# scychon/openmm_drudeNose

Hardware: AMD Instinct MI355X
Metric: integrator steps/sec at 1M Drude pairs (higher is better)
Workload: dtype f64; 1 GPU; SWM4-NDP water box, 1000000 molecules = 5000000 particle slots, 1000000 Drude pairs, 1 temperature group (+ molecular-COM and Drude thermostats), TGNH mode, mixed precision, numNHChains=1, hard wall 0.02 nm, harness force call-out inside the timed region (harness_force: lattice); harness_force=lattice, precision=mixed, variant=resident, hipgraph=False, parallelism=particle-sharded x1 (whole molecules), one KE all-reduce per step, slots_per_gpu=5000000

## Files before the change

### include/drude_tgnh.h

```cpp
#ifndef DRUDE_TGNH_H_
#define DRUDE_TGNH_H_

#include <stdint.h>

#ifdef __cplusplus
extern "C" {
#endif

#define TGNH_ABI_VERSION 1

typedef int tgnh_status;
enum {
    TGNH_OK = 0,
    TGNH_ERR_ARG = -1,
    TGNH_ERR_GROUP_MISMATCH = -2,
    TGNH_ERR_HARDWALL = -3,
    TGNH_ERR_UNSUPPORTED = -4,
    TGNH_ERR_HIP = -5,
    TGNH_ERR_STATE = -6
};

enum { TGNH_MODE_DUALNH = 0,
       TGNH_MODE_TGNH = 1 };

// ... 8 lines not shown
enum { TGNH_FLAG_TRUST_STATE_CHANGED = 16 };

enum { TGNH_FLAG_GATHER = 32 };

typedef struct tgnh_desc {
    uint32_t struct_size;
    int32_t mode;
    int32_t precision;
    int32_t flags;
    int32_t device;
    int32_t num_particles;
    int32_t padded_num_particles;
    int32_t num_pairs;
    int32_t num_groups;
    int32_t num_residues;
    int32_t num_constraints;
    int32_t has_cm_motion_remover;
    const double* mass;
    const int32_t* pair_drude;
    const int32_t* pair_parent;
    const int32_t* group;
    const int32_t* resid;
    const int32_t* constraint_i;
    const int32_t* constraint_j;
    double kB;
    double temperature, coupling_time;
    double drude_temperature, drude_coupling_time;
    double step_size;
    int32_t drude_steps_per_real_step;
    int32_t num_nh_chains;
    int32_t use_drude_nh_chains;
    int32_t use_com_temp_group;
    double max_drude_distance;
} tgnh_desc;

typedef struct tgnh_context* tgnh_handle;


typedef int (*tgnh_allreduce_fn)(void* buf, int count, void* stream, void* user);

const char* tgnh_last_error(void);
int tgnh_abi_version(void);

tgnh_status tgnh_create(const tgnh_desc* desc, tgnh_handle* out);
tgnh_status tgnh_destroy(tgnh_handle h);

tgnh_status tgnh_bind_buffers(tgnh_handle h, void* posq, void* posq_correction, void* velm,
                              const void* force, void* pos_delta);

tgnh_status tgnh_set_step_size(tgnh_handle h, double dt);
tgnh_status tgnh_set_drude_steps_per_real_step(tgnh_handle h, int n);
tgnh_status tgnh_set_max_drude_distance(tgnh_handle h, double d);

tgnh_status tgnh_get_local_dof_terms(tgnh_handle h, double* terms, int* count);
tgnh_status tgnh_set_global_dof_terms(tgnh_handle h, const double* terms, int count);
tgnh_status tgnh_set_allreduce(tgnh_handle h, tgnh_allreduce_fn fn, void* user);

#define TGNH_RCCL_ID_BYTES 128
tgnh_status tgnh_rccl_unique_id(void* id_out);
tgnh_status tgnh_rccl_init(tgnh_handle h, int world, int rank, const void* id);
tgnh_status tgnh_set_rccl_comm(tgnh_handle h, void* nccl_comm);
tgnh_status tgnh_rccl_shutdown(tgnh_handle h);
tgnh_status tgnh_set_resident_share(tgnh_handle h, int share);
tgnh_status tgnh_get_resident_work_groups(tgnh_handle h, int* per_compute_unit);
tgnh_status tgnh_get_step_path(tgnh_handle h, int* gather, const char** reason);
tgnh_status tgnh_get_resident_kernel(tgnh_handle h, int* which);

#define TGNH_XCHG_HANDLE_BYTES 64
tgnh_status tgnh_exchange_create(tgnh_handle h, int world, int rank, void* ipc_handle_out, void** mailbox_out);
tgnh_status tgnh_exchange_attach(tgnh_handle h, const void* ipc_handles);
tgnh_status tgnh_exchange_attach_pointers(tgnh_handle h, void* const* mailboxes);
tgnh_status tgnh_exchange_detach(tgnh_handle h);
tgnh_status tgnh_exchange_wait_stats(tgnh_handle h, void* stream, double* mean_us, double* max_us, int64_t* exchanges);

tgnh_status tgnh_step_begin(tgnh_handle h, void* stream);
tgnh_status tgnh_step_end(tgnh_handle h, void* stream);
tgnh_status tgnh_step_begin_kick(tgnh_handle h, void* stream);
tgnh_status tgnh_step_begin_move(tgnh_handle h, void* stream);
tgnh_status tgnh_step_end_kick(tgnh_handle h, void* stream);
tgnh_status tgnh_step_end_thermo(tgnh_handle h, void* stream);
tgnh_status tgnh_flush(tgnh_handle h, void* stream);
tgnh_status tgnh_note_replayed_steps(tgnh_handle h, int nsteps);
tgnh_status tgnh_get_pending_state(tgnh_handle h, uint32_t* bits);
tgnh_status tgnh_set_time(tgnh_handle h, double time, int64_t step_count);
tgnh_status tgnh_state_changed(tgnh_handle h);

tgnh_status tgnh_set_velocities_to_temperature(tgnh_handle h, double temperature, double drude_temperature,
                                               uint64_t seed, int64_t first_particle, void* stream);

typedef struct tgnh_momentum {
    uint32_t struct_size;
    int32_t  reserved;
    int64_t  massive;
    double   mass;
    double   momentum[3];
} tgnh_momentum;
tgnh_status tgnh_get_momentum(tgnh_handle h, void* stream, tgnh_momentum* out);
tgnh_status tgnh_shift_velocities(tgnh_handle h, const double dv[3], void* stream);
tgnh_status tgnh_remove_cm_motion(tgnh_handle h, void* stream);
tgnh_status tgnh_set_cm_motion_removal(tgnh_handle h, int every);

tgnh_status tgnh_set_molecules(tgnh_handle h, const int32_t* molecule );
tgnh_status tgnh_get_num_molecules(tgnh_handle h, int* count);
tgnh_status tgnh_get_molecules(tgnh_handle h, int32_t* molecule_out );
tgnh_status tgnh_scale_positions(tgnh_handle h, const double scale[3], int save, void* stream);
tgnh_status tgnh_restore_positions(tgnh_handle h, void* stream);

enum { TGNH_MIN_DRUDE_ONLY = 1 };
typedef struct tgnh_minimize_desc {
    double tolerance;
    double dt_start, dt_max;
    double max_step;
    double f_inc, f_dec, alpha_start, f_alpha;
    int32_t n_min;
    int32_t flags;
    const uint8_t* moving;
} tgnh_minimize_desc;
typedef struct tgnh_minimize_state {
    int64_t iterations, uphill, since_uphill, moving;
    int32_t converged;
    int32_t reserved;
    double dt, alpha, power, ff, vv, rms_force;
} tgnh_minimize_state;
tgnh_status tgnh_minimize_begin(tgnh_handle h, const tgnh_minimize_desc* desc, double* work , void* stream);
tgnh_status tgnh_minimize_iterate(tgnh_handle h, void* stream);
tgnh_status tgnh_get_minimize_state(tgnh_handle h, void* stream, tgnh_minimize_state* out);
tgnh_status tgnh_minimize_end(tgnh_handle h);
tgnh_status tgnh_run_harness_minimize(tgnh_handle h, const void* x0, double k_drude, double k_tether, int iterations, void* stream);

tgnh_status tgnh_set_periodic_box(tgnh_handle h, const double a[3], const double b[3], const double c[3]);
tgnh_status tgnh_get_periodic_box(tgnh_handle h, double a[3], double b[3], double c[3]);
tgnh_status tgnh_wrap_molecules(tgnh_handle h, void* stream);
enum { TGNH_FRAME_WRAP = 1, TGNH_FRAME_SKIP_DRUDE = 2, TGNH_FRAME_INTERLEAVED = 4 };
typedef struct tgnh_frame_desc {
    uint32_t struct_size;
    int32_t  flags;
    double   unit;
    int64_t  stride;
    int64_t  capacity;
} tgnh_frame_desc;
tgnh_status tgnh_get_frame_count(tgnh_handle h, int32_t flags, int64_t* count);
tgnh_status tgnh_write_frame(tgnh_handle h, const tgnh_frame_desc* desc, float* out , void* stream);

tgnh_status tgnh_scale_velocities(tgnh_handle h, const double* factors, int count, void* stream);
tgnh_status tgnh_rescale_to_temperature(tgnh_handle h, double temperature, double drude_temperature, void* stream);
tgnh_status tgnh_get_rescale_factors(tgnh_handle h, void* stream, double* factors);
tgnh_status tgnh_set_velocity_rescaling(tgnh_handle h, int every, double temperature, double drude_temperature);

tgnh_status tgnh_set_temperatures(tgnh_handle h, double temperature, double drude_temperature, void* stream);

tgnh_status tgnh_get_kinetic_energy(tgnh_handle h, int ke_sum_valid, void* stream, double* out);
tgnh_status tgnh_get_num_thermostats(tgnh_handle h, int* count);
tgnh_status tgnh_get_last_kinetic_energies(tgnh_handle h, void* stream, double* ke);
tgnh_status tgnh_get_last_scale_factors(tgnh_handle h, void* stream, double* scale);
tgnh_status tgnh_get_status_flags(tgnh_handle h, void* stream, uint32_t* flags);
tgnh_status tgnh_get_time(tgnh_handle h, double* time, int64_t* step_count);
tgnh_status tgnh_get_dof(tgnh_handle h, double* dof, double* nkt);

#define TGNH_DRUDE_HIST_BINS 32
typedef struct tgnh_drude_stats {
    uint32_t struct_size;
    int32_t  worst_particle;
    int64_t  pairs;
    int64_t  over;
    double   max_distance;
    double   sum_d2;
// ... 58 lines not shown
```

### openmm_drudenose_amd/_lib.py

```python
import ctypes as C
import os

HERE = os.path.dirname(os.path.abspath(__file__))
LIB_PATH = os.environ.get("TGNH_LIB") or os.path.join(HERE, "libdrudetgnh_hip.so")

TGNH_OK = 0
ERR_ARG, ERR_GROUP_MISMATCH, ERR_HARDWALL, ERR_UNSUPPORTED, ERR_HIP, ERR_STATE = -1, -2, -3, -4, -5, -6
MODE_DUALNH, MODE_TGNH = 0, 1
PREC_SINGLE, PREC_MIXED, PREC_DOUBLE = 0, 1, 2
FLAG_DEFER_SCALE, FLAG_RESIDENT_STEP, FLAG_WAVE_TILES, FLAG_TRUST_STATE_CHANGED, FLAG_GATHER = 2, 4, 8, 16, 32
KID_SKD, KID_KICK_KE, KID_SCALE, KID_KE, KID_CHAIN, KID_FORCE, KID_OTHER, KID_STEP = range(8)
KERNEL_NAMES = {KID_SKD: "scale+kick+drift", KID_KICK_KE: "kick+KE", KID_SCALE: "rescale", KID_KE: "KE",
                KID_CHAIN: "chain", KID_FORCE: "harness force", KID_OTHER: "other", KID_STEP: "resident step"}

c_i32p = C.POINTER(C.c_int32)
c_f64p = C.POINTER(C.c_double)


class TgnhDesc(C.Structure):
    _fields_ = [
        ("struct_size", C.c_uint32), ("mode", C.c_int32), ("precision", C.c_int32), ("flags", C.c_int32),
        ("device", C.c_int32), ("num_particles", C.c_int32), ("padded_num_particles", C.c_int32),
        ("num_pairs", C.c_int32), ("num_groups", C.c_int32), ("num_residues", C.c_int32),
        ("num_constraints", C.c_int32), ("has_cm_motion_remover", C.c_int32),
        ("mass", c_f64p), ("pair_drude", c_i32p), ("pair_parent", c_i32p), ("group", c_i32p), ("resid", c_i32p),
        ("constraint_i", c_i32p), ("constraint_j", c_i32p),
        ("kB", C.c_double), ("temperature", C.c_double), ("coupling_time", C.c_double),
        ("drude_temperature", C.c_double), ("drude_coupling_time", C.c_double), ("step_size", C.c_double),
        ("drude_steps_per_real_step", C.c_int32), ("num_nh_chains", C.c_int32),
        ("use_drude_nh_chains", C.c_int32), ("use_com_temp_group", C.c_int32),
        ("max_drude_distance", C.c_double),
    ]


DRUDE_HIST_BINS = 32


class TgnhDrudeStats(C.Structure):
    _fields_ = [
        ("struct_size", C.c_uint32), ("worst_particle", C.c_int32), ("pairs", C.c_int64), ("over", C.c_int64),
        ("max_distance", C.c_double), ("sum_d2", C.c_double), ("dipole", C.c_double * 3),
        ("hist", C.c_int64 * (DRUDE_HIST_BINS + 1)),
    ]


class TgnhMomentum(C.Structure):
    _fields_ = [
        ("struct_size", C.c_uint32), ("reserved", C.c_int32), ("massive", C.c_int64), ("mass", C.c_double),
        ("momentum", C.c_double * 3),
    ]


FRAME_WRAP, FRAME_SKIP_DRUDE, FRAME_INTERLEAVED = 1, 2, 4


class TgnhFrameDesc(C.Structure):
    _fields_ = [
        ("struct_size", C.c_uint32), ("flags", C.c_int32), ("unit", C.c_double), ("stride", C.c_int64), ("capacity", C.c_int64),
    ]


MIN_DRUDE_ONLY = 1
SITE_TWO_AVERAGE, SITE_THREE_AVERAGE, SITE_OUT_OF_PLANE, SITE_LOCAL_COORDINATES = range(4)
SITE_PARAMS = 12


class TgnhMinimizeDesc(C.Structure):
    _fields_ = [
        ("tolerance", C.c_double), ("dt_start", C.c_double), ("dt_max", C.c_double), ("max_step", C.c_double),
        ("f_inc", C.c_double), ("f_dec", C.c_double), ("alpha_start", C.c_double), ("f_alpha", C.c_double),
        ("n_min", C.c_int32), ("flags", C.c_int32), ("moving", C.c_void_p),
    ]


class TgnhMinimizeState(C.Structure):
    _fields_ = [
        ("iterations", C.c_int64), ("uphill", C.c_int64), ("since_uphill", C.c_int64), ("moving", C.c_int64),
        ("converged", C.c_int32), ("reserved", C.c_int32),
        ("dt", C.c_double), ("alpha", C.c_double), ("power", C.c_double), ("ff", C.c_double), ("vv", C.c_double),
        ("rms_force", C.c_double),
    ]


ALLREDUCE_FN = C.CFUNCTYPE(C.c_int, C.c_void_p, C.c_int, C.c_void_p, C.c_void_p)

SIGNATURES = {
    "tgnh_last_error": (C.c_char_p, []),
    "tgnh_abi_version": (C.c_int, []),
    "tgnh_create": (C.c_int, [C.POINTER(TgnhDesc), C.POINTER(C.c_void_p)]),
    "tgnh_destroy": (C.c_int, [C.c_void_p]),
    "tgnh_bind_buffers": (C.c_int, [C.c_void_p] * 6),
    "tgnh_set_step_size": (C.c_int, [C.c_void_p, C.c_double]),
    "tgnh_set_drude_steps_per_real_step": (C.c_int, [C.c_void_p, C.c_int]),
    "tgnh_set_max_drude_distance": (C.c_int, [C.c_void_p, C.c_double]),
    "tgnh_get_local_dof_terms": (C.c_int, [C.c_void_p, c_f64p, C.POINTER(C.c_int)]),
    "tgnh_set_global_dof_terms": (C.c_int, [C.c_void_p, c_f64p, C.c_int]),
    "tgnh_set_allreduce": (C.c_int, [C.c_void_p, ALLREDUCE_FN, C.c_void_p]),
    "tgnh_rccl_unique_id": (C.c_int, [C.c_void_p]),
    "tgnh_rccl_init": (C.c_int, [C.c_void_p, C.c_int, C.c_int, C.c_void_p]),
    "tgnh_set_rccl_comm": (C.c_int, [C.c_void_p, C.c_void_p]),
    "tgnh_rccl_shutdown": (C.c_int, [C.c_void_p]),
    "tgnh_exchange_wait_stats": (C.c_int, [C.c_void_p, C.c_void_p, c_f64p, c_f64p, C.POINTER(C.c_int64)]),
    "tgnh_get_pending_state": (C.c_int, [C.c_void_p, C.POINTER(C.c_uint32)]),
    "tgnh_set_resident_share": (C.c_int, [C.c_void_p, C.c_int]),
    "tgnh_get_resident_work_groups": (C.c_int, [C.c_void_p, C.POINTER(C.c_int)]),
    "tgnh_get_resident_kernel": (C.c_int, [C.c_void_p, C.POINTER(C.c_int)]),
    "tgnh_get_step_path": (C.c_int, [C.c_void_p, C.POINTER(C.c_int), C.POINTER(C.c_char_p)]),
    "tgnh_exchange_create": (C.c_int, [C.c_void_p, C.c_int, C.c_int, C.c_void_p, C.POINTER(C.c_void_p)]),
    "tgnh_exchange_attach": (C.c_int, [C.c_void_p, C.c_char_p]),
    "tgnh_exchange_attach_pointers": (C.c_int, [C.c_void_p, C.POINTER(C.c_void_p)]),
    "tgnh_exchange_detach": (C.c_int, [C.c_void_p]),
    "tgnh_step_begin": (C.c_int, [C.c_void_p, C.c_void_p]),
    "tgnh_step_end": (C.c_int, [C.c_void_p, C.c_void_p]),
    "tgnh_step_begin_kick": (C.c_int, [C.c_void_p, C.c_void_p]),
    "tgnh_step_begin_move": (C.c_int, [C.c_void_p, C.c_void_p]),
    "tgnh_step_end_kick": (C.c_int, [C.c_void_p, C.c_void_p]),
    "tgnh_step_end_thermo": (C.c_int, [C.c_void_p, C.c_void_p]),
    "tgnh_flush": (C.c_int, [C.c_void_p, C.c_void_p]),
    "tgnh_state_changed": (C.c_int, [C.c_void_p]),
    "tgnh_set_velocities_to_temperature": (C.c_int, [C.c_void_p, C.c_double, C.c_double, C.c_int64, C.c_int64, C.c_void_p]),
    "tgnh_get_momentum": (C.c_int, [C.c_void_p, C.c_void_p, C.c_void_p]),
    "tgnh_shift_velocities": (C.c_int, [C.c_void_p, c_f64p, C.c_void_p]),
    "tgnh_remove_cm_motion": (C.c_int, [C.c_void_p, C.c_void_p]),
    "tgnh_set_cm_motion_removal": (C.c_int, [C.c_void_p, C.c_int]),
    "tgnh_scale_velocities": (C.c_int, [C.c_void_p, c_f64p, C.c_int, C.c_void_p]),
    "tgnh_rescale_to_temperature": (C.c_int, [C.c_void_p, C.c_double, C.c_double, C.c_void_p]),
    "tgnh_get_rescale_factors": (C.c_int, [C.c_void_p, C.c_void_p, c_f64p]),
    "tgnh_set_velocity_rescaling": (C.c_int, [C.c_void_p, C.c_int, C.c_double, C.c_double]),
    "tgnh_set_molecules": (C.c_int, [C.c_void_p, c_i32p]),
    "tgnh_get_num_molecules": (C.c_int, [C.c_void_p, C.POINTER(C.c_int)]),
    "tgnh_get_molecules": (C.c_int, [C.c_void_p, c_i32p]),
    "tgnh_scale_positions": (C.c_int, [C.c_void_p, c_f64p, C.c_int, C.c_void_p]),
    "tgnh_restore_positions": (C.c_int, [C.c_void_p, C.c_void_p]),
    "tgnh_minimize_begin": (C.c_int, [C.c_void_p, C.c_void_p, C.c_void_p, C.c_void_p]),
    "tgnh_minimize_iterate": (C.c_int, [C.c_void_p, C.c_void_p]),
    "tgnh_get_minimize_state": (C.c_int, [C.c_void_p, C.c_void_p, C.c_void_p]),
    "tgnh_minimize_end": (C.c_int, [C.c_void_p]),
    "tgnh_run_harness_minimize": (C.c_int, [C.c_void_p, C.c_void_p, C.c_double, C.c_double, C.c_int, C.c_void_p]),
    "tgnh_set_periodic_box": (C.c_int, [C.c_void_p, c_f64p, c_f64p, c_f64p]),
    "tgnh_get_periodic_box": (C.c_int, [C.c_void_p, c_f64p, c_f64p, c_f64p]),
    "tgnh_wrap_molecules": (C.c_int, [C.c_void_p, C.c_void_p]),
    "tgnh_get_frame_count": (C.c_int, [C.c_void_p, C.c_int32, C.POINTER(C.c_int64)]),
    "tgnh_write_frame": (C.c_int, [C.c_void_p, C.c_void_p, C.c_void_p, C.c_void_p]),
    "tgnh_set_temperatures": (C.c_int, [C.c_void_p, C.c_double, C.c_double, C.c_void_p]),
    "tgnh_note_replayed_steps": (C.c_int, [C.c_void_p, C.c_int]),
    "tgnh_set_time": (C.c_int, [C.c_void_p, C.c_double, C.c_int64]),
    "tgnh_get_kinetic_energy": (C.c_int, [C.c_void_p, C.c_int, C.c_void_p, c_f64p]),
    "tgnh_get_num_thermostats": (C.c_int, [C.c_void_p, C.POINTER(C.c_int)]),
    "tgnh_get_last_kinetic_energies": (C.c_int, [C.c_void_p, C.c_void_p, c_f64p]),
    "tgnh_get_last_scale_factors": (C.c_int, [C.c_void_p, C.c_void_p, c_f64p]),
    "tgnh_get_status_flags": (C.c_int, [C.c_void_p, C.c_void_p, C.POINTER(C.c_uint32)]),
    "tgnh_get_time": (C.c_int, [C.c_void_p, c_f64p, C.POINTER(C.c_int64)]),
    "tgnh_get_dof": (C.c_int, [C.c_void_p, c_f64p, c_f64p]),
    "tgnh_get_drude_statistics": (C.c_int, [C.c_void_p, C.c_double, C.c_double, C.c_void_p, C.c_void_p]),
    "tgnh_get_thermostat_len": (C.c_int, [C.c_void_p, C.c_int, C.POINTER(C.c_int)]),
    "tgnh_get_thermostat_state": (C.c_int, [C.c_void_p, C.c_int, C.c_void_p, c_f64p]),
    "tgnh_set_thermostat_state": (C.c_int, [C.c_void_p, C.c_int, C.c_void_p, c_f64p]),
    "tgnh_get_topology_len": (C.c_int, [C.c_void_p, C.c_int, C.POINTER(C.c_int)]),
    "tgnh_get_topology": (C.c_int, [C.c_void_p, C.c_int, c_i32p]),
    "tgnh_get_launch_bounds": (C.c_int, [C.c_void_p, c_i32p]),
    "tgnh_compute_kinetic_energies": (C.c_int, [C.c_void_p, C.c_void_p]),
    "tgnh_half_kick": (C.c_int, [C.c_void_p, C.c_void_p]),
    "tgnh_harness_force": (C.c_int, [C.c_void_p, C.c_void_p, C.c_double, C.c_double, C.c_void_p, C.c_void_p]),
    "tgnh_harness_pack_sites": (C.c_int, [C.c_void_p, C.c_void_p]),
    "tgnh_harness_lattice_hint": (C.c_int, [C.c_void_p, C.c_int, C.c_int, C.c_double, c_f64p, C.c_int]),
    "tgnh_harness_sites_kind": (C.c_int, [C.c_void_p, C.POINTER(C.c_int)]),
    "tgnh_run_harness": (C.c_int, [C.c_void_p, C.c_void_p, C.c_double, C.c_double, C.c_int, C.c_void_p]),
    "tgnh_run_steps": (C.c_int, [C.c_void_p, C.c_int, C.c_void_p]),
    "tgnh_harness_set_clusters": (C.c_int, [C.c_void_p, C.c_int, c_i32p, c_f64p]),
    "tgnh_harness_shake_positions": (C.c_int, [C.c_void_p, C.c_double, C.c_void_p]),
    "tgnh_harness_shake_velocities": (C.c_int, [C.c_void_p, C.c_double, C.c_void_p]),
    "tgnh_harness_set_virtual_sites": (C.c_int, [C.c_void_p, C.c_int, c_i32p, c_f64p]),
    "tgnh_harness_virtual_sites": (C.c_int, [C.c_void_p, C.c_void_p]),
    "tgnh_run_harness_constrained": (C.c_int, [C.c_void_p, C.c_void_p, C.c_double, C.c_double, C.c_double, C.c_int, C.c_void_p]),
    "tgnh_set_constraint_clusters": (C.c_int, [C.c_void_p, C.c_int, c_i32p, c_f64p]),
    "tgnh_get_num_constraint_clusters": (C.c_int, [C.c_void_p, C.POINTER(C.c_int)]),
    "tgnh_apply_constraints": (C.c_int, [C.c_void_p, C.c_double, C.c_void_p]),
    "tgnh_apply_velocity_constraints": (C.c_int, [C.c_void_p, C.c_double, C.c_void_p]),
    "tgnh_set_virtual_sites": (C.c_int, [C.c_void_p, C.c_int, c_i32p, c_i32p, c_f64p]),
    "tgnh_get_num_virtual_sites": (C.c_int, [C.c_void_p, C.POINTER(C.c_int)]),
    "tgnh_compute_virtual_sites": (C.c_int, [C.c_void_p, C.c_void_p]),
    "tgnh_distribute_virtual_site_forces": (C.c_int, [C.c_void_p, C.c_void_p, C.c_void_p]),
    "tgnh_harness_water_force": (C.c_int, [C.c_void_p, C.c_double, C.c_double, C.c_void_p, C.c_void_p]),
    "tgnh_harness_remove_cm_motion": (C.c_int, [C.c_void_p, C.c_void_p]),
    "tgnh_timing_enable": (C.c_int, [C.c_void_p, C.c_int]),
    "tgnh_timing_read": (C.c_int, [C.c_void_p, C.c_int, c_f64p, C.POINTER(C.c_int64)]),
# ... 28 lines not shown
```

### openmm_drudenose_amd/build.py

```python
import os
import subprocess
import sys

HERE = os.path.dirname(os.path.abspath(__file__))
CSRC = os.path.join(HERE, "csrc")
LIB = os.path.join(HERE, "libdrudetgnh_hip.so")
SOURCES = ["tgnh_topology.cpp", "tgnh_lifecycle.cpp", "tgnh_exchange.cpp", "tgnh_step.cpp", "tgnh_velocities.cpp", "tgnh_queries.cpp", "tgnh_harness_host.cpp", "tgnh_positions.cpp",
           "tgnh_frames.cpp", "tgnh_minimize.cpp", "tgnh_constraints.cpp", "tgnh_virtual_sites.cpp",
           "tgnh_kernels.hip", "tgnh_gather.hip", "tgnh_harness.hip", "tgnh_velinit.hip", "tgnh_drude_stats.hip", "tgnh_cm_motion.hip",
           "tgnh_rescale.hip", "tgnh_scale_positions.hip", "tgnh_wrap.hip", "tgnh_minimize.hip", "tgnh_constraints.hip",
           "tgnh_virtual_sites.hip"]
HEADERS = sorted(n for n in os.listdir(CSRC) if n.endswith(".h")) + [os.path.join("..", "..", "include", "drude_tgnh.h")]
ARCH = "gfx950"


def source_sha():
    import hashlib
    h = hashlib.sha1()
    for name in sorted(os.listdir(CSRC)):
        path = os.path.join(CSRC, name)
        if os.path.isfile(path) and name.endswith((".cpp", ".hip", ".h")):
            h.update(name.encode())
            h.update(open(path, "rb").read())
    h.update(open(os.path.join(HERE, "..", "include", "drude_tgnh.h"), "rb").read())
    return h.hexdigest()[:16]


def _stale():
    if not os.path.exists(LIB):
        return True
    t = os.path.getmtime(LIB)
    deps = [os.path.join(CSRC, s) for s in SOURCES + HEADERS] + [os.path.abspath(__file__)]
    return any(os.path.getmtime(d) > t for d in deps)


def _object_key(src, flags):
    import hashlib
    h = hashlib.sha1(" ".join(flags).encode())
    for path in [os.path.join(CSRC, src)] + [os.path.join(CSRC, x) for x in HEADERS]:
        h.update(open(path, "rb").read())
    return h.hexdigest()[:16]


def build(force=False, verbose=False):
    if not force and not _stale():
        return LIB
    from concurrent.futures import ThreadPoolExecutor
    hipcc = os.environ.get("HIPCC", "/opt/rocm/bin/hipcc")
    flags = [hipcc, "--offload-arch=" + ARCH, "-O3", "-std=c++17", "-fPIC", "-Wall", "-Wno-unused-function", "-x", "hip"]
    objdir = os.path.join(HERE, "build")
    os.makedirs(objdir, exist_ok=True)

    def compile_one(src):
        obj = os.path.join(objdir, f"{os.path.splitext(src)[0]}.{_object_key(src, flags)}.o")
        if force or not os.path.exists(obj):
            cmd = flags + ["-c", os.path.join(CSRC, src), "-o", obj + ".tmp"]
            if verbose:
                print(" ".join(cmd), file=sys.stderr)
            subprocess.run(cmd, check=True)
            os.replace(obj + ".tmp", obj)
        return obj

    with ThreadPoolExecutor(len(SOURCES)) as pool:
        objs = list(pool.map(compile_one, SOURCES))
    for name in os.listdir(objdir):
        if name.endswith(".o") and os.path.join(objdir, name) not in objs:
            os.remove(os.path.join(objdir, name))
    cmd = [hipcc, "--offload-arch=" + ARCH, "-shared", "-fPIC"] + objs + ["-ldl", "-o", LIB]
    if verbose:
        print(" ".join(cmd), file=sys.stderr)
    subprocess.run(cmd, check=True)
    return LIB


if __name__ == "__main__":
    print(build(force="--force" in sys.argv, verbose=True))
```

### openmm_drudenose_amd/csrc/tgnh_constraints.cpp

```cpp
#include <numeric>

#include "tgnh_host.h"
#include "tgnh_constraints.h"

static const int CN_PA[6] = {0, 0, 0, 1, 1, 2}, CN_PB[6] = {1, 2, 3, 2, 3, 3};

static tgnh_status clusters_check(const tgnh_context* c, int n, const int32_t* atoms, const double* dist) {
    const int N = c->d.num_particles;
    std::vector<int> owner((size_t)N, -1);
    for (int k = 0; k < n; k++) {
        const int32_t* at = atoms + 4 * (size_t)k;
        const double* d = dist + 6 * (size_t)k;
        const std::string who = "tgnh_set_constraint_clusters: cluster " + std::to_string(k);
        for (int m = 0; m < 4; m++) {
            if (at[m] < -1 || at[m] >= N) return fail(TGNH_ERR_ARG, who + ": atom index " + std::to_string(at[m]) + " out of range");
            if (at[m] < 0) continue;
            if (owner[at[m]] == k) return fail(TGNH_ERR_ARG, who + " lists atom " + std::to_string(at[m]) + " twice");
            if (owner[at[m]] >= 0)
                return fail(TGNH_ERR_ARG, who + " and cluster " + std::to_string(owner[at[m]]) + " share atom " + std::to_string(at[m]) + ": two lanes would write one slot");
            owner[at[m]] = k;
        }
        int K = 0;
        for (int p = 0; p < 6; p++) {
            if (!std::isfinite(d[p]) || d[p] < 0.0) return fail(TGNH_ERR_ARG, who + ": a distance is negative or not finite");
// ... 21 lines not shown
    return TGNH_OK;
}

extern "C" tgnh_status tgnh_set_constraint_clusters(tgnh_handle h, int n, const int32_t* atoms, const double* dist) {
    CHECK_H(h);
    if (n < 0 || (n > 0 && (!atoms || !dist))) return fail(TGNH_ERR_ARG, "tgnh_set_constraint_clusters: bad cluster arrays");
    tgnh_status rc = clusters_check(h, n, atoms, dist); if (rc) return rc;
    if (h->host_only) { h->cons.count = n; return TGNH_OK; }
    HIP_OK(hipSetDevice(h->device));
    h->cons.drop();
    if (n == 0) return TGNH_OK;
    std::vector<int> order((size_t)n), first((size_t)n);
    for (int k = 0; k < n; k++) {
        int lo = h->d.num_particles;
        for (int m = 0; m < 4; m++) if (atoms[4 * (size_t)k + m] >= 0) lo = std::min(lo, (int)atoms[4 * (size_t)k + m]);
        first[k] = lo;
    }
    std::iota(order.begin(), order.end(), 0);
    std::stable_sort(order.begin(), order.end(), [&](int x, int y) { return first[x] < first[y]; });
    std::vector<int4> r_atoms((size_t)n);
    std::vector<double4> r_w((size_t)n);
    std::vector<double> r_d2(3 * (size_t)n, 0.0);
    std::vector<uint32_t> r_pairs((size_t)n);
    for (int row = 0; row < n; row++) {
        const int32_t* at = atoms + 4 * (size_t)order[row];
        const double* d = dist + 6 * (size_t)order[row];
        r_atoms[row] = make_int4(at[0], at[1], at[2], at[3]);
        double w[4];
        for (int m = 0; m < 4; m++) w[m] = at[m] >= 0 && h->topo.mass[at[m]] != 0.0 ? 1.0 / h->topo.mass[at[m]] : 0.0;
        r_w[row] = make_double4(w[0], w[1], w[2], w[3]);
        uint32_t pairs = 0, K = 0;
        for (int p = 0; p < 6; p++) {
            if (d[p] == 0.0) continue;
            r_d2[K * (size_t)n + row] = d[p] * d[p];
            pairs |= ((uint32_t)CN_PA[p] | (uint32_t)CN_PB[p] << 2) << (4 * K);
            K++;
        }
        r_pairs[row] = pairs | K << 12;
    }
    HIP_OK(h->cons.d_atoms.upload(r_atoms));
    HIP_OK(h->cons.d_invmass.upload(r_w));
    HIP_OK(h->cons.d_d2.upload(r_d2));
    HIP_OK(h->cons.d_pairs.upload(r_pairs));
    h->cons.count = n;
    return TGNH_OK;
}

extern "C" tgnh_status tgnh_get_num_constraint_clusters(tgnh_handle h, int* count) {
    CHECK_H(h);
    if (!count) return fail(TGNH_ERR_ARG, "null count");
    *count = h->cons.count;
    return TGNH_OK;
}

static tgnh_status constraints_ready(tgnh_handle h, const char* what) {
    CHECK_H(h);
    if (h->host_only) return fail(TGNH_ERR_STATE, std::string(what) + ": host-only handle (device -1): no GPU work can be launched on it");
    if (!h->bound.velm) return fail(TGNH_ERR_STATE, std::string(what) + ": tgnh_bind_buffers has not been called");
    return TGNH_OK;
}

static ConstraintArgs constraint_args(tgnh_handle h, double tol) {
    ConstraintArgs a{};
    a.atoms = h->cons.d_atoms; a.invmass = h->cons.d_invmass; a.d2 = h->cons.d_d2; a.pairs = h->cons.d_pairs; a.n = h->cons.count;
    a.posq = h->bound.posq; a.posq_corr = h->bound.posq_corr; a.velm = h->bound.velm; a.pos_delta = h->bound.pos_delta;
    a.tol = tol; a.status = h->status.d_word;
    return a;
}

extern "C" tgnh_status tgnh_apply_constraints(tgnh_handle h, double tol, void* stream) {
    tgnh_status rc = constraints_ready(h, "tgnh_apply_constraints"); if (rc) return rc;
    if (!h->bound.pos_delta) return fail(TGNH_ERR_STATE, "tgnh_apply_constraints: posDelta buffer not bound");
    if (h->cons.count == 0) return TGNH_OK;
    HIP_OK(hipSetDevice(h->device));
    HIP_OK(launch_constrain_positions(h->d.precision, constraint_args(h, tol), (hipStream_t)stream));
    return TGNH_OK;
}

extern "C" tgnh_status tgnh_apply_velocity_constraints(tgnh_handle h, double tol, void* stream) {
    tgnh_status rc = constraints_ready(h, "tgnh_apply_velocity_constraints"); if (rc) return rc;
    h->owed.ke_carry = false;
    if (h->cons.count == 0) return TGNH_OK;
    HIP_OK(hipSetDevice(h->device));
    HIP_OK(launch_constrain_velocities(h->d.precision, constraint_args(h, tol), (hipStream_t)stream));
    return TGNH_OK;
}
```

### openmm_drudenose_amd/csrc/tgnh_context.h

```cpp
#ifndef TGNH_CONTEXT_H_
#define TGNH_CONTEXT_H_

#include <map>
#include <string>
#include <vector>

#include "tgnh_internal.h"
#include "tgnh_by_index.h"
#include "tgnh_minimize.h"

void tgnh_set_error(const std::string& msg);

namespace tgnh {
template <typename T> class DeviceBuf {
    T* p_ = nullptr;
    bool pinned_ = false;
public:
    DeviceBuf() = default;
    DeviceBuf(DeviceBuf&& o) noexcept : p_(o.p_), pinned_(o.pinned_) { o.p_ = nullptr; }
    ~DeviceBuf() { reset(); }
    void reset() { if (p_) (void)(pinned_ ? hipHostFree(p_) : hipFree(p_)); p_ = nullptr; }
    hipError_t alloc(size_t n, bool zero = false, unsigned ext_flags = 0) {
        reset(); pinned_ = false;
        void* p = nullptr;
        hipError_t e = ext_flags ? hipExtMallocWithFlags(&p, sizeof(T) * n, ext_flags) : hipMalloc(&p, sizeof(T) * n);
        if (e != hipSuccess) return e;
        p_ = static_cast<T*>(p);
        return zero ? hipMemset(p_, 0, sizeof(T) * n) : hipSuccess;
    }
    hipError_t alloc_pinned(size_t n) { reset(); pinned_ = true; return hipHostMalloc(reinterpret_cast<void**>(&p_), sizeof(T) * n, hipHostMallocDefault); }
    hipError_t upload(const T* src, size_t n) {
        hipError_t e = alloc(n ? n : 1);
        return e != hipSuccess || !n ? e : hipMemcpy(p_, src, sizeof(T) * n, hipMemcpyHostToDevice);
    }
    hipError_t upload(const std::vector<T>& v) { return upload(v.data(), v.size()); }
    T* get() const { return p_; }
    operator T*() const { return p_; }
};
typedef DeviceBuf<unsigned char> DeviceBytes;

template <typename Row> struct __attribute__((visibility("hidden"))) RowScratch {
    DeviceBuf<Row> d_rows;
    int rows_allocated = 0;
    Row h_row{};
    tgnh_status ensure(int grid, bool zero, const char* too_small);
};
}

struct tgnh_context {
    tgnh_desc d;
    int device = 0;
    bool host_only = false;
    struct Topology {
        std::vector<double> mass;
        std::vector<int> pair_drude, pair_parent, group, resid, normal;
        std::vector<int> res_count, res_first;
        std::vector<int> tile_start, tile_res;
        std::vector<int2> res_entries;
        std::vector<int> big_first, big_count;
        int num_big = 0, num_tiles = 0;
        std::vector<uint32_t> meta;
        std::vector<int2> wave_tile;
        std::vector<uint32_t> wmeta;
        std::vector<uint32_t> tile_pat, wtile_pat;
        std::vector<uint32_t> pattern, wpattern;
        int num_wtiles = 0;
        tgnh::DeviceBuf<uint32_t> d_meta, d_wmeta, d_tile_pat, d_pattern, d_wpattern;
        tgnh::DeviceBuf<int> d_tile_start, d_tile_res;
        tgnh::DeviceBuf<int2> d_res_table, d_wave_tile, d_big_table;
        tgnh::DeviceBytes d_big_com;
    } topo;
    struct Gather {
        bool generic = false;
        bool chain = false;
        std::string reason;
        std::vector<int2> res_table;
        std::vector<int> resid, partner;
        int com_lanes = 64;
        tgnh::DeviceBuf<int> d_group, d_resid, d_partner;
        tgnh::DeviceBuf<int2> d_res_table;
        tgnh::DeviceBytes d_com;
        tgnh::DeviceBuf<double> d_scratch;
    } gather;
    struct ByIndex {
        tgnh::DeviceBuf<int> d_partner;
    } by_index;
    tgnh::RowScratch<tgnh::DrudeStatsRow> dstats;
    struct CmMotion : tgnh::RowScratch<tgnh::CmRow> {
        int every = 0;
    } cmm;
    struct Rescale {
        tgnh::DeviceBuf<double> d_buf;
        bool applied = false;
        int every = 0;
        double temperature = 0, drude_temperature = 0;
    } resc;
    struct Molecules {
        struct Table {
            std::vector<int> mol_of;
            int count = 0;
            std::vector<int> mem_start, members;
            bool spans = false;
            std::vector<int> span_first;
            std::vector<unsigned long long> span_heads;
            std::vector<int> span_out;
            std::vector<unsigned long long> span_drude;
        } t;
        bool set = false;
        bool on_device = false;
        tgnh::DeviceBuf<int> d_span_first, d_mol_of, d_mem_start, d_members;
        tgnh::DeviceBuf<unsigned long long> d_span_heads;
        tgnh::DeviceBuf<int> d_span_out;
        tgnh::DeviceBuf<unsigned long long> d_span_drude;
        tgnh::DeviceBuf<double> d_shift;
        void drop_device() { on_device = false; d_span_first.reset(); d_mol_of.reset(); d_mem_start.reset(); d_members.reset(); d_span_heads.reset(); d_shift.reset(); d_span_out.reset(); d_span_drude.reset(); }
    } mol;
    struct PeriodicBox {
        bool set = false;
        double a[3] = {0, 0, 0}, b[3] = {0, 0, 0}, c[3] = {0, 0, 0};
    } box;
    struct Frames {
        std::vector<int> out_index;
        int kept = -1;
        tgnh::DeviceBuf<int> d_out_index;
    } frames;
    struct PositionSnapshot {
        tgnh::DeviceBytes d_posq, d_corr;
        bool taken = false;
        bool valid = false;
        const void *of_posq = nullptr, *of_corr = nullptr;
    } snap;
    struct Minimize {
        bool active = false;
        double* work = nullptr;
        int64_t moving = 0;
        tgnh::DeviceBuf<unsigned char> d_mask;
        tgnh::DeviceBuf<double> d_rows;
        tgnh::DeviceBuf<tgnh::MinState> d_state;
        tgnh::MinState h_state{};
        void drop() { active = false; work = nullptr; moving = 0; d_mask.reset(); d_rows.reset(); d_state.reset(); }
    } minim;
    struct Constraints {
        int count = 0;
        tgnh::DeviceBuf<int4> d_atoms;
        tgnh::DeviceBuf<double4> d_invmass;
        tgnh::DeviceBuf<double> d_d2;
        tgnh::DeviceBuf<uint32_t> d_pairs;
        void drop() { count = 0; d_atoms.reset(); d_invmass.reset(); d_d2.reset(); d_pairs.reset(); }
    } cons;
    struct VirtualSites {
        int count = 0;
        int receivers = 0;
        tgnh::DeviceBuf<int4> d_atoms;
        tgnh::DeviceBuf<int> d_kind;
        tgnh::DeviceBuf<double> d_params;
        tgnh::DeviceBuf<int> d_recv_slot, d_recv_start, d_recv_row;
        tgnh::DeviceBuf<unsigned char> d_recv_role;
        void drop() { count = receivers = 0; d_atoms.reset(); d_kind.reset(); d_params.reset(); d_recv_slot.reset(); d_recv_start.reset(); d_recv_row.reset(); d_recv_role.reset(); }
    } vsites;
    struct Thermostat {
        std::vector<double> h_state;
        std::vector<double> local_terms, global_terms;
        std::vector<double> dof, nkbt;
        double realkbT = 0, drudekbT = 0;
        tgnh::ChainLayout L{};
        tgnh::DeviceBuf<double> d_partials;
        tgnh::DeviceBuf<double> d_state;
        tgnh::DeviceBuf<double> d_stage;
        tgnh::DeviceBuf<double> d_scalar;
    } thermo;
    struct LaunchConfig {
        int grid = 0, gb = 1;
        int num_cus = 256, grid_override = 0;
        std::map<int, int> grid_cache;
        bool alternate_sweeps = true;
        int inline_sum_rows = tgnh::CHAIN_INLINE_SUM_ROWS;
        bool inline_sum_all = false;
        bool carry_ok = false;
        bool inline_chain = false;
        bool wave_ke = false;
        int resident_grid[5][2] = {{0, 0}, {0, 0}, {0, 0}, {0, 0}, {0, 0}};
        int resident_share = 1;
        int wresident_per_cu = 0, wresident_grid = 0;
        int resident_per_cu = 0;
    } cfg;
    struct Owed {
        bool end_pending = false;
        bool scale_pending = false;
        bool kick_pending = false;
        bool first_half_done = false;
        bool chain_pending = false;
        bool sum_pending = false;
        bool xwait_pending = false;
        bool stage_pending = false;
        bool ke_carry = false;
        bool chain_pending_twice = false;
        bool carry_pending = false;
        bool tail_summed = false;
        bool end_folded = false;
        bool g_com_fresh = false;
        enum : uint32_t { BIT_SWEEP_REVERSE = 1u << 8 };
        uint32_t bits() const {
            return end_pending | scale_pending << 1 | kick_pending << 2 | first_half_done << 3 | chain_pending << 4 | sum_pending << 5 |
                   xwait_pending << 6 | stage_pending << 7 | ke_carry << 9;
        }
        void chain_owed(bool twice) { chain_pending = true; chain_pending_twice = twice; }
        void chain_ran() { chain_pending = sum_pending = xwait_pending = carry_pending = false; }
        void velocities_current() { scale_pending = kick_pending = false; }
        void end_half_deferred(bool kick) { scale_pending = first_half_done = true; kick_pending = kick; }
        void resident_settled() { end_pending = first_half_done = false; velocities_current(); chain_pending = sum_pending = xwait_pending = false; }
        void thermostat_reset() { end_pending = first_half_done = false; velocities_current(); chain_pending = stage_pending = carry_pending = ke_carry = false; }
    } owed;
    struct Run {
        double time = 0;
        int64_t step_count = 0;
        int sweep_reverse = 0;
        int ke_parts = 0;
    } run;
    struct Bound {
        void *posq = nullptr, *posq_corr = nullptr, *velm = nullptr, *pos_delta = nullptr;
        const void* force = nullptr;
    } bound;
    struct Status {
        tgnh::DeviceBuf<uint32_t> d_word;
        tgnh::DeviceBuf<uint32_t> h_seen;
        int failed_code = 0;
        std::string failed;
    } status;
    struct Meeting {
        tgnh::DeviceBuf<unsigned int> d_sync;
        tgnh::DeviceBuf<unsigned long long> d_rows;
        tgnh::DeviceBuf<unsigned long long> self_box;
        tgnh::DeviceBuf<unsigned long long> d_self_misc;
        tgnh::XchgArgs self_x{};
    } meet;
    struct Exchange {
        tgnh_allreduce_fn allreduce = nullptr;
        void* allreduce_user = nullptr;
        void* rccl_comm = nullptr;
        bool rccl_owned = false;
        tgnh::XchgArgs args{};
        bool on = false;
        int world = 0, rank = 0;
        tgnh::DeviceBuf<unsigned long long> mailbox;
        tgnh::DeviceBuf<unsigned long long*> d_peers;
        std::vector<void*> opened;
        tgnh::DeviceBuf<unsigned long long> d_seq;
        tgnh::DeviceBuf<unsigned int> d_dead;
        tgnh::DeviceBuf<unsigned long long> d_stat;
        void close_peers() { for (void* p : opened) (void)hipIpcCloseMemHandle(p); opened.clear(); }
        ~Exchange() { close_peers(); }
    } xchg;
    struct Harness {
        tgnh::DeviceBuf<int4> d_cl_atoms, d_vs_atoms;
        tgnh::DeviceBuf<double> d_cl_dist, d_vs_w;
        int num_clusters = 0, num_sites = 0;
        tgnh::DeviceBuf<uint8_t> d_sflag;
        tgnh::DeviceBuf<uint32_t> d_sbase;
        tgnh::DeviceBytes d_sites;
        int lat_k = 0, lat_side = 0, lat_mol0 = 0;
        double lat_spacing = 0;
        std::vector<double> lat_geom;
        bool lat_on = false;
        tgnh::DeviceBuf<unsigned char> d_lat_tab;
        tgnh::DeviceBytes d_g_x0;
    } harness;
    struct Timing {
        bool on = false;
        int only = -1;
        struct Ev { hipEvent_t a, b; int kid; };
        std::vector<Ev> ev_pool;
        size_t ev_used = 0;
        double t_total[tgnh::KID_COUNT] = {0};
        int64_t t_count[tgnh::KID_COUNT] = {0};
        ~Timing() { for (auto& e : ev_pool) { (void)hipEventDestroy(e.a); (void)hipEventDestroy(e.b); } }
    } timing;
};

#endif
```

### openmm_drudenose_amd/csrc/tgnh_harness.hip

```cpp
#include "tgnh_context.h"
#include "tgnh_device_math.h"

namespace tgnh {

template <int PREC>
__global__ __launch_bounds__(BLOCK) void force_kernel(const ForceArgs a) {
    typedef typename Prec<PREC>::real4 real4;
    typedef typename Prec<PREC>::mixed mixed;
    const real4* __restrict__ posq = reinterpret_cast<const real4*>(a.posq);
    const float4* __restrict__ pcorr = reinterpret_cast<const float4*>(a.posq_corr);
    const real4* __restrict__ x0 = reinterpret_cast<const real4*>(a.x0);
    const mixed kd = (mixed)a.k_drude, kt = (mixed)a.k_tether;
    const int lane = threadIdx.x & 63;
    const int nround = (a.n + gridDim.x * BLOCK - 1) / (gridDim.x * BLOCK);
    for (int rr = 0; rr < nround; rr++) {
        const int r = a.reverse ? nround - 1 - rr : rr;
        const int blk = a.reverse ? (int)gridDim.x - 1 - (int)blockIdx.x : (int)blockIdx.x;
        const int i = (r * gridDim.x + blk) * BLOCK + threadIdx.x;
        const bool in = i < a.n;
        uint32_t m = 0;
        mixed x = 0, y = 0, z = 0;
        if (in) {
            m = a.meta[i];
            const real4 p = posq[i];
// ... 347 lines not shown
    const int ma = blockIdx.x;
    double xa[5][3], f[5][3];
#pragma unroll
    for (int i = 0; i < 5; i++) { site(5 * ma + i, xa[i]); f[i][0] = f[i][1] = f[i][2] = 0.0; }
    for (int mb = threadIdx.x; mb < a.n_mol; mb += BLOCK) {
        if (mb == ma) continue;
#pragma unroll
        for (int j = 0; j < 5; j++) {
            double xb[3];
            site(5 * mb + j, xb);
#pragma unroll
            for (int i = 0; i < 5; i++) {
                double d[3];
#pragma unroll
                for (int k = 0; k < 3; k++) { d[k] = xa[i][k] - xb[k]; d[k] -= a.box * floor(d[k] * inv_box + 0.5); }
                const double r2 = d[0] * d[0] + d[1] * d[1] + d[2] * d[2];
                if (r2 >= c2) continue;
                const double r = sqrt(r2), inv_r = 1.0 / r;
                double dEdr = ONE_4PI_EPS0 * Q[i] * Q[j] * (-inv_r * inv_r + 2.0 * krf * r);
                if (i == 0 && j == 0) {
                    const double s2 = sigma * sigma / r2, s6 = s2 * s2 * s2;
                    dEdr += 4.0 * eps * (-12.0 * s6 * s6 + 6.0 * s6) * inv_r;
                }
                const double c = -dEdr * inv_r;
                f[i][0] += c * d[0]; f[i][1] += c * d[1]; f[i][2] += c * d[2];
            }
        }
    }
    const int lane = threadIdx.x & 63, wv = threadIdx.x >> 6;
#pragma unroll
    for (int i = 0; i < 5; i++)
#pragma unroll
        for (int k = 0; k < 3; k++) {
            const double t = h_wave_sum(f[i][k]);
            if (lane == 0) sred[wv][3 * i + k] = t;
        }
    __syncthreads();
    if (threadIdx.x < 3) {
        const int k = threadIdx.x;
        double fs[5];
#pragma unroll
        for (int i = 0; i < 5; i++) { fs[i] = 0.0; for (int w = 0; w < BLOCK / 64; w++) fs[i] += sred[w][3 * i + k]; }
        const double sp = kd * (xa[1][k] - xa[0][k]);
        fs[1] -= sp; fs[0] += sp;
        fs[0] += W[0] * fs[4]; fs[2] += W[1] * fs[4]; fs[3] += W[2] * fs[4]; fs[4] = 0.0;
#pragma unroll
        for (int i = 0; i < 5; i++) a.force[(size_t)k * a.padded + 5 * ma + i] = (long long)(fs[i] * 4294967296.0);
    }
}

template <int PREC>
__global__ __launch_bounds__(BLOCK) void cmm_kernel(void* velm_, int n) {
    typedef typename Prec<PREC>::mixed mixed;
    typedef typename Prec<PREC>::mixed4 mixed4;
    mixed4* __restrict__ velm = reinterpret_cast<mixed4*>(velm_);
    __shared__ double sred[BLOCK / 64][4];
    __shared__ double vcm[3];
    double px = 0, py = 0, pz = 0, pm = 0;
    for (int i = threadIdx.x; i < n; i += BLOCK) {
        const mixed4 v = velm[i];
        if (v.w != 0) { const double m = 1.0 / (double)v.w; px += m * v.x; py += m * v.y; pz += m * v.z; pm += m; }
    }
    px = h_wave_sum(px); py = h_wave_sum(py); pz = h_wave_sum(pz); pm = h_wave_sum(pm);
    if ((threadIdx.x & 63) == 0) { double* r = sred[threadIdx.x >> 6]; r[0] = px; r[1] = py; r[2] = pz; r[3] = pm; }
    __syncthreads();
    if (threadIdx.x == 0) {
        double t[4] = {0, 0, 0, 0};
        for (int w = 0; w < BLOCK / 64; w++) for (int k = 0; k < 4; k++) t[k] += sred[w][k];
        for (int k = 0; k < 3; k++) vcm[k] = t[k] / t[3];
    }
    __syncthreads();
    for (int i = threadIdx.x; i < n; i += BLOCK) {
        mixed4 v = velm[i];
        if (v.w != 0) { v.x -= (mixed)vcm[0]; v.y -= (mixed)vcm[1]; v.z -= (mixed)vcm[2]; velm[i] = v; }
    }
}

}
using namespace tgnh;

#define H_FAIL(code, msg) do { tgnh_set_error(msg); return code; } while (0)
#define H_HIP(expr) do { hipError_t e_ = (expr); if (e_ != hipSuccess) { tgnh_set_error(std::string(#expr) + ": " + hipGetErrorString(e_)); return TGNH_ERR_HIP; } } while (0)

static tgnh_status harness_ready(tgnh_handle h) {
    if (!h) H_FAIL(TGNH_ERR_ARG, "null handle");
    if (h->host_only) H_FAIL(TGNH_ERR_STATE, "host-only handle (device -1): no GPU work can be launched on it");
    if (!h->bound.velm) H_FAIL(TGNH_ERR_STATE, "tgnh_bind_buffers has not been called");
    return TGNH_OK;
}

extern "C" tgnh_status tgnh_harness_set_clusters(tgnh_handle h, int n, const int32_t* atoms, const double* dist) {
    if (!h) H_FAIL(TGNH_ERR_ARG, "null handle");
    if (h->host_only) H_FAIL(TGNH_ERR_STATE, "host-only handle");
    if (n < 0 || (n > 0 && (!atoms || !dist))) H_FAIL(TGNH_ERR_ARG, "bad cluster arrays");
    for (long long i = 0; i < 4LL * n; i++)
        if (atoms[i] < -1 || atoms[i] >= h->d.num_particles) H_FAIL(TGNH_ERR_ARG, "cluster atom index out of range");
    H_HIP(hipSetDevice(h->device));
    h->harness.d_cl_atoms.reset(); h->harness.d_cl_dist.reset();
    h->harness.num_clusters = n;
    if (n == 0) return TGNH_OK;
    H_HIP(h->harness.d_cl_atoms.upload(reinterpret_cast<const int4*>(atoms), n));
    H_HIP(h->harness.d_cl_dist.upload(dist, 6 * (size_t)n));
    return TGNH_OK;
}

static ClusterArgs cluster_args(tgnh_handle h, double tol) {
    ClusterArgs a{};
    a.atoms = h->harness.d_cl_atoms; a.dist = h->harness.d_cl_dist; a.n = h->harness.num_clusters;
    a.posq = h->bound.posq; a.posq_corr = h->bound.posq_corr; a.velm = h->bound.velm; a.pos_delta = h->bound.pos_delta;
    a.tol = tol; a.status = h->status.d_word;
    return a;
}

extern "C" tgnh_status tgnh_harness_shake_positions(tgnh_handle h, double tol, void* stream) {
    tgnh_status rc = harness_ready(h); if (rc) return rc;
    if (!h->bound.pos_delta) H_FAIL(TGNH_ERR_STATE, "posDelta buffer not bound");
    if (h->harness.num_clusters == 0) return TGNH_OK;
    H_HIP(hipSetDevice(h->device));
    H_HIP(launch_shake<false>(h->d.precision, cluster_args(h, tol), (hipStream_t)stream));
    return TGNH_OK;
}

extern "C" tgnh_status tgnh_harness_shake_velocities(tgnh_handle h, double tol, void* stream) {
    tgnh_status rc = harness_ready(h); if (rc) return rc;
    h->owed.ke_carry = false;
    if (h->harness.num_clusters == 0) return TGNH_OK;
    H_HIP(hipSetDevice(h->device));
    H_HIP(launch_shake<true>(h->d.precision, cluster_args(h, tol), (hipStream_t)stream));
    return TGNH_OK;
}

extern "C" tgnh_status tgnh_harness_set_virtual_sites(tgnh_handle h, int n, const int32_t* atoms, const double* weights) {
    if (!h) H_FAIL(TGNH_ERR_ARG, "null handle");
    if (h->host_only) H_FAIL(TGNH_ERR_STATE, "host-only handle");
    if (n < 0 || (n > 0 && (!atoms || !weights))) H_FAIL(TGNH_ERR_ARG, "bad virtual-site arrays");
    for (long long i = 0; i < 4LL * n; i++)
        if (atoms[i] < 0 || atoms[i] >= h->d.num_particles) H_FAIL(TGNH_ERR_ARG, "virtual-site atom index out of range");
    H_HIP(hipSetDevice(h->device));
    h->harness.d_vs_atoms.reset(); h->harness.d_vs_w.reset();
    h->harness.num_sites = n;
    if (n == 0) return TGNH_OK;
    H_HIP(h->harness.d_vs_atoms.upload(reinterpret_cast<const int4*>(atoms), n));
    H_HIP(h->harness.d_vs_w.upload(weights, 3 * (size_t)n));
    return TGNH_OK;
}

extern "C" tgnh_status tgnh_harness_virtual_sites(tgnh_handle h, void* stream) {
    tgnh_status rc = harness_ready(h); if (rc) return rc;
    if (h->harness.num_sites == 0) return TGNH_OK;
    H_HIP(hipSetDevice(h->device));
    SiteArgs a{};
    a.atoms = h->harness.d_vs_atoms; a.w = h->harness.d_vs_w; a.n = h->harness.num_sites; a.posq = h->bound.posq; a.posq_corr = h->bound.posq_corr;
    H_HIP(launch_sites(h->d.precision, a, (hipStream_t)stream));
    return TGNH_OK;
}

extern "C" tgnh_status tgnh_run_harness_constrained(tgnh_handle h, const void* x0, double k_drude, double k_tether,
                                                    double tol, int nsteps, void* stream) {
    tgnh_status rc = harness_ready(h); if (rc) return rc;
    for (int i = 0; i < nsteps; i++) {
        rc = tgnh_step_begin_kick(h, stream); if (rc) return rc;
        rc = tgnh_harness_shake_positions(h, tol, stream); if (rc) return rc;
        rc = tgnh_apply_constraints(h, tol, stream); if (rc) return rc;
        rc = tgnh_step_begin_move(h, stream); if (rc) return rc;
        rc = tgnh_harness_virtual_sites(h, stream); if (rc) return rc;
        rc = tgnh_compute_virtual_sites(h, stream); if (rc) return rc;
        rc = tgnh_harness_force(h, x0, k_drude, k_tether, const_cast<void*>(h->bound.force), stream); if (rc) return rc;
        rc = tgnh_step_end_kick(h, stream); if (rc) return rc;
        if (h->d.mode == TGNH_MODE_TGNH) {
            rc = tgnh_harness_shake_velocities(h, tol, stream); if (rc) return rc;
            rc = tgnh_apply_velocity_constraints(h, tol, stream); if (rc) return rc;
        }
        rc = tgnh_step_end_thermo(h, stream); if (rc) return rc;
    }
    return TGNH_OK;
}

extern "C" tgnh_status tgnh_harness_water_force(tgnh_handle h, double box, double cutoff, void* force_out, void* stream) {
    tgnh_status rc = harness_ready(h); if (rc) return rc;
    if (!force_out || !(box > 0) || !(cutoff > 0)) H_FAIL(TGNH_ERR_ARG, "bad box / cutoff / force buffer");
    if (h->d.num_particles % 5) H_FAIL(TGNH_ERR_ARG, "the testWater force field needs O, D, H1, H2, M per molecule");
    H_HIP(hipSetDevice(h->device));
    WaterArgs a{};
    a.posq = h->bound.posq; a.posq_corr = h->bound.posq_corr; a.force = reinterpret_cast<long long*>(force_out);
    a.n_mol = h->d.num_particles / 5; a.padded = h->d.padded_num_particles; a.box = box; a.cutoff = cutoff;
    hipStream_t s = (hipStream_t)stream;
    auto fn = with_precision(h->d.precision, [](auto P) { return &water_force_kernel<decltype(P)::value>; });
    if (!fn) H_FAIL(TGNH_ERR_ARG, "unknown precision");
    TGNH_LAUNCH(fn, dim3(a.n_mol), dim3(BLOCK), 0, s, a);
    H_HIP(hipGetLastError());
    return TGNH_OK;
}

extern "C" tgnh_status tgnh_harness_remove_cm_motion(tgnh_handle h, void* stream) {
    tgnh_status rc = harness_ready(h); if (rc) return rc;
    h->owed.ke_carry = false;
    H_HIP(hipSetDevice(h->device));
    hipStream_t s = (hipStream_t)stream;
    auto fn = with_precision(h->d.precision, [](auto P) { return &cmm_kernel<decltype(P)::value>; });
    if (!fn) H_FAIL(TGNH_ERR_ARG, "unknown precision");
    TGNH_LAUNCH(fn, dim3(1), dim3(BLOCK), 0, s, h->bound.velm, h->d.num_particles);
    H_HIP(hipGetLastError());
    return TGNH_OK;
}
```

### openmm_drudenose_amd/csrc/tgnh_host.h

```cpp
#ifndef TGNH_HOST_H_
#define TGNH_HOST_H_

#include <algorithm>
#include <cmath>
#include <cstdio>
#include <cstdlib>
#include <cstring>

#include "tgnh_context.h"
#include "tgnh_minimize.h"
#include "tgnh_rescale.h"
#include "tgnh_scale_positions.h"

using namespace tgnh;

#pragma GCC visibility push(hidden)
inline tgnh_status fail(tgnh_status code, const std::string& msg) {
    tgnh_set_error(msg);
    return code;
}
#define HIP_OK(expr) do { hipError_t e_ = (expr); if (e_ != hipSuccess) return fail(TGNH_ERR_HIP, std::string(#expr) + ": " + hipGetErrorString(e_)); } while (0)
#define CHECK_H(h) do { if (!(h)) return fail(TGNH_ERR_ARG, "null handle"); } while (0)

inline bool com_thermostat_on(const tgnh_desc& d) { return d.mode == TGNH_MODE_TGNH && d.use_com_temp_group; }
inline int pass_kind(const tgnh_desc& d) { return (d.flags & TGNH_FLAG_DEFER_SCALE) ? 0 : 1; }
void make_layout(tgnh_context* c);
tgnh_status build_topology(tgnh_context* c, const tgnh_desc* d);
void local_dof_terms(tgnh_context* c);
tgnh_status check_temperatures(double temperature, double drude_temperature);
void set_bath_temperatures(tgnh_context* c, double temperature, double drude_temperature);
std::vector<double> thermostat_nkt(const tgnh_context* c, double realkbT, double drudekbT);
void thermostat_targets(tgnh_context* c, std::vector<double>& st);
tgnh_status finalize_thermostat(tgnh_context* c);
std::vector<int> partner_table(const tgnh_context* c);
tgnh_status device_partner_table(tgnh_context* c, const int** out);
tgnh_status deferred_guard(tgnh_handle h, const char* what);
void note_status(tgnh_handle h, uint32_t flags);
tgnh_status entry(tgnh_handle h, bool need_bufs);
bool stream_capturing(hipStream_t s);
tgnh_status finish_query(tgnh_handle h, hipStream_t s);
tgnh_status allreduce_doubles(tgnh_handle h, double* device_ptr, int count, hipStream_t s);
bool resident_now(tgnh_handle h);
tgnh_status allreduce_hook(tgnh_handle h, hipStream_t s);
bool big_com_on(tgnh_handle h);
tgnh_status run_big_com(tgnh_handle h, bool kick, hipStream_t s);
tgnh_status run_tile(tgnh_handle h, int ops, int kid, hipStream_t s, const double* scale = nullptr);
GatherArgs gather_args(tgnh_handle h, const double* scale);
ChainArgs chain_args(tgnh_handle h);
tgnh_status run_chain_gather(tgnh_handle h, hipStream_t s, bool sum_only);
tgnh_status materialize_chain(tgnh_handle h, hipStream_t s);
tgnh_status settle_kick(tgnh_handle h, hipStream_t s);
tgnh_status settle_end(tgnh_handle h, hipStream_t s);
tgnh_status flush_impl(tgnh_handle h, hipStream_t s);
tgnh_status ke_query_launches(tgnh_handle h, hipStream_t s);
tgnh_status cm_removal_due(tgnh_handle h, hipStream_t s);
tgnh_status rescale_due(tgnh_handle h, hipStream_t s);
tgnh_status molecules_ensure(tgnh_context* c, const char* what);
tgnh_status molecules_launch_bounds(const tgnh_context* c);
tgnh_status molecules_device(tgnh_context* c, hipStream_t s);

struct Timed {
    tgnh_context* c; hipStream_t s; int kid; tgnh_context::Timing::Ev* ev = nullptr;
    Timed(tgnh_context* c_, hipStream_t s_, int kid_) : c(c_), s(s_), kid(kid_) {
        if (!c->timing.on) return;
        if (c->timing.only >= 0 && kid != c->timing.only) return;
        if (c->timing.ev_used == c->timing.ev_pool.size()) {
            tgnh_context::Timing::Ev e; e.kid = kid;
            if (hipEventCreate(&e.a) != hipSuccess || hipEventCreate(&e.b) != hipSuccess) return;
            c->timing.ev_pool.push_back(e);
        }
        ev = &c->timing.ev_pool[c->timing.ev_used++];
        ev->kid = kid;
        (void)hipEventRecord(ev->a, s);
    }
    ~Timed() { if (ev) (void)hipEventRecord(ev->b, s); }
};
template <typename Row> tgnh_status tgnh::RowScratch<Row>::ensure(int grid, bool zero, const char* too_small) {
    if (!d_rows) {
        HIP_OK(d_rows.alloc((size_t)grid + 1, zero));
        rows_allocated = grid + 1;
    }
    if (grid < 1 || grid > INDEX_GRID_CAP || grid + 1 > rows_allocated) return fail(TGNH_ERR_STATE, too_small);
    return TGNH_OK;
}
#pragma GCC visibility pop

#endif
```

### openmm_drudenose_amd/csrc/tgnh_internal.h

```cpp
#ifndef TGNH_INTERNAL_H_
#define TGNH_INTERNAL_H_

#include <hip/hip_runtime.h>
#include <stdint.h>
#include <type_traits>

#include "../../include/drude_tgnh.h"

namespace tgnh {

#ifndef TGNH_SPT
#define TGNH_SPT 2
#endif
#ifndef TGNH_TBLOCK
#define TGNH_TBLOCK 256
#endif
constexpr int BLOCK = 256;
constexpr int TBLOCK = TGNH_TBLOCK;
constexpr int SPT = TGNH_SPT;
constexpr int TILE_SLOTS = TBLOCK * SPT;
constexpr int TILE_RES = TILE_SLOTS / 2;
constexpr int GRID_CAP = 2048;
constexpr int MAX_GROUPS = 32;

// ... 54 lines not shown
constexpr size_t XCHG_REPLICA_U64 =
    ((sizeof(unsigned long long) * 2 * (size_t)XCHG_MAX_WORLD * XCHG_NT_PAD * XCHG_CELL_U64 + 4095) / 4096 * 4096 + 256) / sizeof(unsigned long long);
constexpr size_t XCHG_MAILBOX_BYTES(int ) { return sizeof(unsigned long long) * XCHG_REPLICA_U64 * XCHG_REPLICAS; }

struct XchgArgs {
    int on;
    int world, rank;
    unsigned long long* const* peers;
    unsigned long long* mine;
    unsigned long long* seq;
    unsigned int* dead;
    unsigned int* status;
    unsigned long long* stat;
};

constexpr int CHAIN_INLINE_SUM_NT = 10;
constexpr int CHAIN_INLINE_SUM_ROWS = 256;

struct ChainArgs {
    ChainLayout L;
    XchgArgs x;
    int x_send, x_wait;
    double* st;
    uint32_t* status;
    const double* partials;
    int nparts;
    int nbig;
    const double* stage;
    int commit;
    int do_sum;
    int do_chain;
    int chain_twice;
    int lanes;
    int ke_carry;
    double dt;
    int S;
    double dtc, inv_dtc;
    double realkbT, drudekbT;
};

struct TileArgs {
    void* posq;
    void* posq_corr;
    void* velm;
    const long long* force;
    void* pos_delta;
    const uint32_t* meta;
    const int* tile_start;
    const int* tile_res;
    const int2* res_table;
    const void* big_com;
    const double* scale;
    double* partials;
    uint32_t* status;
    unsigned int* sync;
    int census;
    unsigned long long* rows;
    const int2* wave_tile;
    const uint32_t* wmeta;
    const uint32_t* tile_pat;
    const uint32_t* pattern;
    const uint32_t* wpattern;
    int num_wtiles;
    int tail_sum;
    double* ke_red;
    int num_tiles;
    int reverse;
    int padded;
    int num_groups;
    int use_com;
    int hardwall;
    double dt;
    double max_dist;
    double hw_scale;
    int chain_on;
    int sum_rows;
    int commit_len, commit_skip, commit_skip_n;
    const double* commit_src;
    double* commit_dst;
    int x_wait;
    const double* st_in;
    double* st_out;
    ChainArgs chain;
};

struct BigComArgs {
    const int2* table;
    int n;
    const void* velm;
    const long long* force;
    int padded;
    int kick;
    double dt;
    void* big_com;
    double* partials;
    int NT, G;
};

struct ForceArgs {
    const void* posq;
    const void* posq_corr;
    const void* x0;
    const uint32_t* meta;
    long long* force;
    int n, padded;
    int reverse;
    double k_drude, k_tether;
    const uint8_t* sflag;
    const uint32_t* sbase;
    const void* sites;
    int lat_k, lat_side, lat_mol0;
    double lat_spacing, lat_inv_k, lat_inv_side, lat_inv_side2;
    const unsigned char* lat_tab;
};
constexpr size_t LAT_TAB_BYTES = 64 + 64 * 3 * sizeof(double);

constexpr int GATHER_KE_ROWS = 1024;
constexpr int GATHER_MAX_NT = 2048;
struct GatherArgs {
    void* posq; void* posq_corr; void* velm; const long long* force; void* pos_delta;
    const int* group;
    const int* resid;
    const int2* res_table;
    const int* partner;
    void* com;
    const double* scale;
    double* partials;
    uint32_t* status;
    int n, padded, n_res, G, NT, use_com, hardwall, ops, kick_com;
    int com_lanes;
    double dt, max_dist, hw_scale;
};

#define TGNH_LAUNCH(...) do { (void)hipGetLastError(); hipLaunchKernelGGL(__VA_ARGS__); } while (0)

template <typename F>
auto with_precision(const int precision, F&& f) -> decltype(f(std::integral_constant<int, TGNH_PREC_SINGLE>{})) {
    switch (precision) {
        case TGNH_PREC_SINGLE: return f(std::integral_constant<int, TGNH_PREC_SINGLE>{});
        case TGNH_PREC_MIXED: return f(std::integral_constant<int, TGNH_PREC_MIXED>{});
        case TGNH_PREC_DOUBLE: return f(std::integral_constant<int, TGNH_PREC_DOUBLE>{});
        default: return {};
    }
}
#define TGNH_LAUNCH_PREC(kernel, precision, grid, block, lds, s, ...) do {                                        \
        auto fn_ = tgnh::with_precision(precision, [](auto P) { return &kernel<decltype(P)::value>; });           \
        if (!fn_) return hipErrorInvalidValue;                                                                     \
        TGNH_LAUNCH(fn_, grid, block, lds, s, __VA_ARGS__);                                                        \
    } while (0)
template <typename FN> int blocks_per_cu(FN fn, const int threads, const size_t lds) {
    int n = 0;
    if (!fn || hipOccupancyMaxActiveBlocksPerMultiprocessor(&n, reinterpret_cast<const void*>(fn), threads, lds) != hipSuccess) return 0;
    return n;
}

typedef void (*tile_fn_t)(const TileArgs);
hipError_t launch_tile(int precision, int ops, int gb, const TileArgs& a, int grid, size_t lds, hipStream_t s);
int tile_blocks_per_cu(int precision, int ops, int gb, size_t lds, bool multi = false);
hipError_t launch_step(int precision, int gb, int kind, const TileArgs& a, int grid, size_t lds, hipStream_t s);
int step_blocks_per_cu(int precision, int gb, int kind, size_t lds);
int step_kind_ops2(int kind);
hipError_t launch_wstep(int precision, int gb, bool multi, const TileArgs& a, int grid, hipStream_t s);
int wstep_blocks_per_cu(int precision, int gb, bool multi);
hipError_t launch_wke(int precision, int ops, int gb, const TileArgs& a, int grid, hipStream_t s);
int wke_blocks_per_cu(int precision, int ops, int gb);
hipError_t launch_chain(const ChainArgs& a, hipStream_t s);
hipError_t launch_big_com(int precision, const BigComArgs& a, hipStream_t s);
hipError_t launch_force(int precision, const ForceArgs& a, hipStream_t s);
hipError_t launch_gather_com(int precision, const GatherArgs& a, hipStream_t s);
int gather_ke_grid(const GatherArgs& a);
hipError_t launch_gather_ke(int precision, const GatherArgs& a, int grid, hipStream_t s);
hipError_t launch_gather_rowsum(const double* partials, int nrows, int NT, double* ke_red, hipStream_t s);
hipError_t launch_gather_chain(const ChainArgs& a, double* scratch, hipStream_t s);
hipError_t launch_gather_update(int precision, const GatherArgs& a, hipStream_t s);
hipError_t launch_gather_force(int precision, const GatherArgs& a, const void* x0, long long* force, double k_drude, double k_tether, hipStream_t s);
constexpr int PLAIN_KE_PARTS = 2048;
hipError_t launch_plain_ke(int precision, const void* velm, const long long* force, int n, int padded,
                           double time_shift, double* out , hipStream_t s);
size_t tile_lds_bytes(int precision, int ops, bool hardwall, bool use_com);

}

#endif
```

### openmm_drudenose_amd/csrc/tgnh_lifecycle.cpp

```cpp
#include <memory>

#include "tgnh_host.h"
#ifndef TGNH_MEETING_MEM
#define TGNH_MEETING_MEM hipDeviceMallocFinegrained
#endif

static thread_local std::string g_err;
extern "C" const char* tgnh_last_error(void) { return g_err.c_str(); }
extern "C" int tgnh_abi_version(void) { return TGNH_ABI_VERSION; }

void tgnh_set_error(const std::string& msg) { g_err = msg; }

static tgnh_status validate_desc(const tgnh_desc* d, bool* long_chain) {
    if (d->struct_size != sizeof(tgnh_desc)) return fail(TGNH_ERR_ARG, "tgnh_desc size mismatch (ABI)");
    if (d->mode != TGNH_MODE_DUALNH && d->mode != TGNH_MODE_TGNH) return fail(TGNH_ERR_ARG, "bad mode");
    if (d->precision < TGNH_PREC_SINGLE || d->precision > TGNH_PREC_DOUBLE) return fail(TGNH_ERR_ARG, "bad precision");
    if (d->num_particles < 1 || d->num_pairs < 0 || !d->mass || (d->num_pairs && (!d->pair_drude || !d->pair_parent)))
        return fail(TGNH_ERR_ARG, "bad particle / pair arrays");
    if (d->padded_num_particles < d->num_particles) return fail(TGNH_ERR_ARG, "padded_num_particles < num_particles");
    if (d->num_constraints < 0) return fail(TGNH_ERR_ARG, "negative num_constraints");
    if (3LL * d->padded_num_particles > 2147483647LL)
        return fail(TGNH_ERR_UNSUPPORTED, "more than 715 827 882 padded particle slots: the index into the third force plane leaves 32 bits");
    if (d->num_nh_chains < 1 || d->drude_steps_per_real_step < 1) return fail(TGNH_ERR_ARG, "numNHChains and drudeStepsPerRealStep must be >= 1");
    if (d->mode == TGNH_MODE_TGNH && (d->num_groups < 1 || d->num_residues < 1 || !d->group || !d->resid))
// ... 45 lines not shown
    if (const char* e = getenv("TGNH_GRID")) { int g = atoi(e); if (g >= 1) c->cfg.grid_override = std::min(g, GRID_CAP); }
#endif
    {
        bool want = true;
        c->cfg.inline_sum_all = d->num_particles < 2000000;
#ifdef TGNH_TUNING
        if (const char* e = getenv("TGNH_INLINE_CHAIN")) want = e[0] != '0';
        if (const char* e4 = getenv("TGNH_INLINE_SUM_ROWS")) c->cfg.inline_sum_rows = atoi(e4);
        if (const char* e5 = getenv("TGNH_INLINE_SUM_ALL")) c->cfg.inline_sum_all = e5[0] != '0';
        if (const char* e3 = getenv("TGNH_ALTERNATE_SWEEPS")) c->cfg.alternate_sweeps = e3[0] != '0';
#endif
        int inline_multi_max = 2500000;
#ifdef TGNH_TUNING
        if (const char* e6 = getenv("TGNH_INLINE_MULTI_MAX")) inline_multi_max = atoi(e6);
#endif
        c->cfg.inline_chain = want && !c->gather.generic && (c->thermo.L.C == 1 || (c->thermo.L.C <= 4 && d->num_particles < inline_multi_max));
        if (c->thermo.L.total > 256 && c->thermo.L.C > 1) c->cfg.inline_chain = c->cfg.inline_chain && false;
    }
    return TGNH_OK;
}

static tgnh_status allocate(tgnh_context* c) {
    const size_t NT = c->thermo.L.NT;
    HIP_OK(c->thermo.d_partials.alloc((size_t)(c->cfg.grid + c->topo.num_big) * NT, true));
    HIP_OK(c->thermo.d_state.alloc(c->thermo.L.total));
    HIP_OK(c->thermo.d_stage.alloc(c->thermo.L.total));
    HIP_OK(c->status.d_word.alloc(1, true));
    HIP_OK(c->status.h_seen.alloc_pinned(1));
    *c->status.h_seen = 0;
    if (c->gather.chain && c->thermo.L.C > 4) HIP_OK(c->gather.d_scratch.alloc(NT * (4 * c->thermo.L.C + 1)));
    HIP_OK(c->thermo.d_scalar.alloc(1 + PLAIN_KE_PARTS));
    HIP_OK(c->meet.d_sync.alloc(4, true));
    const bool resident = (c->d.flags & TGNH_FLAG_RESIDENT_STEP) != 0;
    if (c->cfg.wave_ke || resident)
        HIP_OK(c->meet.d_rows.alloc(2 * (size_t)GRID_CAP * CHAIN_INLINE_SUM_NT, true, TGNH_MEETING_MEM));
    if (!resident) return TGNH_OK;
    HIP_OK(c->meet.self_box.alloc(XCHG_MAILBOX_BYTES(1) / sizeof(unsigned long long), true, TGNH_MEETING_MEM));
    HIP_OK(c->meet.d_self_misc.alloc(4, true));
    unsigned long long* const box = c->meet.self_box;
    HIP_OK(hipMemcpy(c->meet.d_self_misc + 2, &box, sizeof(box), hipMemcpyHostToDevice));
    c->meet.self_x = XchgArgs{};
    c->meet.self_x.on = 1; c->meet.self_x.world = 1; c->meet.self_x.rank = 0;
    c->meet.self_x.peers = reinterpret_cast<unsigned long long* const*>(c->meet.d_self_misc + 2);
    c->meet.self_x.mine = c->meet.self_box;
    c->meet.self_x.seq = c->meet.d_self_misc;
    c->meet.self_x.dead = reinterpret_cast<unsigned int*>(c->meet.d_self_misc + 1);
    c->meet.self_x.status = c->status.d_word;
    return TGNH_OK;
}

template <typename Launch> static tgnh_status census(tgnh_context* c, int per_cu_max, Launch&& launch, int* found) {
    for (int per_cu = std::min(per_cu_max, 8); per_cu >= 1 && !*found; per_cu--) {
        TileArgs a{};
        a.census = 1; a.sync = c->meet.d_sync;
        HIP_OK(hipMemset(c->meet.d_sync + 2, 0, 2 * sizeof(unsigned int)));
        const int grid = std::min(per_cu * c->cfg.num_cus, GRID_CAP);
        HIP_OK(launch(a, grid));
        unsigned int res[2] = {0, 1};
        HIP_OK(hipMemcpy(res, c->meet.d_sync + 2, sizeof(res), hipMemcpyDeviceToHost));
        if (res[0] == (unsigned)grid && res[1] == 0) *found = per_cu;
    }
    return TGNH_OK;
}

static tgnh_status resident_census(tgnh_context* c) {
    if (!(c->d.flags & TGNH_FLAG_RESIDENT_STEP) || c->cfg.gb == 0 || !c->cfg.inline_chain || c->thermo.L.NT > CHAIN_INLINE_SUM_NT) return TGNH_OK;
    const int kind = pass_kind(c->d);
    const size_t lds = tile_lds_bytes(c->d.precision, step_kind_ops2(kind), true, true);
    tgnh_status rc = census(c, c->thermo.L.C == 1 ? step_blocks_per_cu(c->d.precision, c->cfg.gb, kind, lds) : 0,
                            [&](const TileArgs& a, int grid) { return launch_step(c->d.precision, c->cfg.gb, kind, a, grid, lds, (hipStream_t)0); },
                            &c->cfg.resident_per_cu);
    if (rc) return rc;
    const bool multi = c->thermo.L.C > 1;
    bool want_w = c->cfg.wave_ke && (c->d.flags & TGNH_FLAG_DEFER_SCALE) && (c->cfg.resident_per_cu > 0 || multi);
    if (c->d.mode == TGNH_MODE_DUALNH && !c->thermo.L.use_drude_chains && multi) want_w = false;
#ifdef TGNH_TUNING
    if (const char* e = getenv("TGNH_WSTEP")) want_w = want_w && e[0] != '0';
#endif
    return census(c, want_w ? wstep_blocks_per_cu(c->d.precision, c->cfg.gb, multi) : 0,
                  [&](const TileArgs& a, int grid) { return launch_wstep(c->d.precision, c->cfg.gb, multi, a, grid, (hipStream_t)0); },
                  &c->cfg.wresident_per_cu);
}

extern "C" tgnh_status tgnh_create(const tgnh_desc* d, tgnh_handle* out) {
    if (!d || !out) return fail(TGNH_ERR_ARG, "null argument");
    bool long_chain = false;
    tgnh_status rc = validate_desc(d, &long_chain); if (rc) return rc;
    const bool host_only = d->device == -1;
    if (!host_only) {
        int ndev = 0;
        HIP_OK(hipGetDeviceCount(&ndev));
        if (d->device < 0 || d->device >= ndev) return fail(TGNH_ERR_HIP, "no such HIP device (the HIP path needs an MI355X; there is no CPU fallback)");
        HIP_OK(hipSetDevice(d->device));
    }

    std::unique_ptr<tgnh_context> owner(new tgnh_context());
    tgnh_context* c = owner.get();
    c->host_only = host_only;
    c->d = *d;
    c->device = d->device;
    set_bath_temperatures(c, d->temperature, d->drude_temperature);
    make_layout(c);
    c->cfg.gb = c->thermo.L.G <= 1 ? 1 : (c->thermo.L.G <= 4 ? 4 : (c->thermo.L.G <= 8 ? 8 : 0));
    if (long_chain) { c->gather.generic = true; c->gather.reason = "a chain too long for the LDS-resident form"; }
    else if (d->flags & TGNH_FLAG_GATHER) { c->gather.generic = true; c->gather.reason = "asked for (TGNH_FLAG_GATHER)"; }
    if (!host_only) {
        hipDeviceProp_t prop;
        if (hipGetDeviceProperties(&prop, d->device) == hipSuccess && prop.multiProcessorCount > 0) c->cfg.num_cus = prop.multiProcessorCount;
    }
    rc = build_topology(c, d); if (rc) return rc;
    rc = decide_policy(c, d, long_chain); if (rc) return rc;
    local_dof_terms(c);
    c->thermo.global_terms = c->thermo.local_terms;
    c->d.mass = nullptr; c->d.pair_drude = c->d.pair_parent = c->d.group = c->d.resid = nullptr;
    c->d.constraint_i = c->d.constraint_j = nullptr;

    if (!host_only) {
        rc = allocate(c); if (rc) return rc;
        rc = resident_census(c); if (rc) return rc;
    }
    rc = finalize_thermostat(c); if (rc) return rc;
    *out = owner.release();
    return TGNH_OK;
}

extern "C" tgnh_status tgnh_destroy(tgnh_handle h) {
    CHECK_H(h);
    if (h->xchg.rccl_comm) (void)tgnh_rccl_shutdown(h);
    if (!h->host_only) (void)hipSetDevice(h->device);
    delete h;
    return TGNH_OK;
}

extern "C" tgnh_status tgnh_bind_buffers(tgnh_handle h, void* posq, void* posq_correction, void* velm,
                                         const void* force, void* pos_delta) {
    CHECK_H(h);
    if (h->host_only) return fail(TGNH_ERR_STATE, "host-only handle (device -1): no GPU work can be launched on it");
    if (!posq || !velm || !force) return fail(TGNH_ERR_ARG, "posq, velm and force are required");
    if (h->d.precision == TGNH_PREC_MIXED && !posq_correction) return fail(TGNH_ERR_ARG, "mixed precision needs posqCorrection");
    if ((h->owed.kick_pending || h->owed.end_pending) && (velm != h->bound.velm || force != h->bound.force))
        return fail(TGNH_ERR_STATE, "tgnh_bind_buffers: velm / force may not be rebound while a deferred half kick is pending (tgnh_flush first)");
    if (posq == h->bound.posq && posq_correction == h->bound.posq_corr && velm == h->bound.velm && force == h->bound.force && pos_delta == h->bound.pos_delta)
        return TGNH_OK;
    {
        HIP_OK(hipSetDevice(h->device));
        const size_t N = (size_t)h->d.num_particles, P = (size_t)h->d.padded_num_particles;
        const size_t r4 = h->d.precision == TGNH_PREC_DOUBLE ? 32 : 16, m4 = h->d.precision == TGNH_PREC_SINGLE ? 16 : 32;
        struct { const void* p; size_t need; const char* name; } bufs[] = {
            {posq, N * r4, "posq"}, {posq_correction, N * 16, "posqCorrection"}, {velm, N * m4, "velm"},
            {force, 3 * P * sizeof(long long), "force"}, {pos_delta, N * m4, "posDelta"}};
        for (const auto& b : bufs) {
            if (!b.p) continue;
            hipDeviceptr_t base = nullptr; size_t size = 0;
            if (hipMemGetAddressRange(&base, &size, const_cast<void*>(b.p)) != hipSuccess) { (void)hipGetLastError(); continue; }
            const size_t left = size - (size_t)(static_cast<const char*>(b.p) - static_cast<const char*>(base));
            if (left < b.need)
                return fail(TGNH_ERR_ARG, std::string("tgnh_bind_buffers: ") + b.name + " has " + std::to_string(left) + " bytes behind the pointer, the launches touch " + std::to_string(b.need));
        }
    }
    h->owed.ke_carry = false;
    if (posq != h->bound.posq || posq_correction != h->bound.posq_corr) h->snap.valid = false;
    h->bound.posq = posq; h->bound.posq_corr = posq_correction; h->bound.velm = velm; h->bound.force = force; h->bound.pos_delta = pos_delta;
    return TGNH_OK;
}

tgnh_status deferred_guard(tgnh_handle h, const char* what) {
    if (h->owed.first_half_done || h->owed.end_pending)
        return fail(TGNH_ERR_STATE, std::string(what) + ": not allowed between steps with TGNH_FLAG_DEFER_SCALE (the next thermostat half step has already run)");
    return TGNH_OK;
}

extern "C" tgnh_status tgnh_set_step_size(tgnh_handle h, double dt) {
    CHECK_H(h);
    if (!(dt > 0) || !std::isfinite(dt)) return fail(TGNH_ERR_ARG, "step size must be positive");
    if (dt != h->d.step_size) { tgnh_status rc = deferred_guard(h, "tgnh_set_step_size"); if (rc) return rc; }
    h->d.step_size = dt;
    return TGNH_OK;
}
extern "C" tgnh_status tgnh_set_drude_steps_per_real_step(tgnh_handle h, int n) {
    CHECK_H(h);
    if (n < 1) return fail(TGNH_ERR_ARG, "drudeStepsPerRealStep must be >= 1");
    if (n != h->d.drude_steps_per_real_step) { tgnh_status rc = deferred_guard(h, "tgnh_set_drude_steps_per_real_step"); if (rc) return rc; }
    h->d.drude_steps_per_real_step = n;
    return TGNH_OK;
}
extern "C" tgnh_status tgnh_set_max_drude_distance(tgnh_handle h, double dist) {
    CHECK_H(h);
    if (!(dist >= 0)) return fail(TGNH_ERR_ARG, "setMaxDrudeDistance: Distance cannot be negative");
    h->d.max_drude_distance = dist;
    return TGNH_OK;
}

extern "C" tgnh_status tgnh_set_temperatures(tgnh_handle h, double temperature, double drude_temperature, void* stream) {
    CHECK_H(h);
    tgnh_status rc = check_temperatures(temperature, drude_temperature); if (rc) return rc;
    rc = deferred_guard(h, "tgnh_set_temperatures"); if (rc) return rc;
    const ChainLayout& L = h->thermo.L;
    hipStream_t s = (hipStream_t)stream;
    rc = entry(h, false); if (rc) return rc;
    if (!h->host_only) { rc = materialize_chain(h, s); if (rc) return rc; }
    h->owed.ke_carry = false;
    set_bath_temperatures(h, temperature, drude_temperature);
    std::vector<double> st(L.total, 0.0);
    thermostat_targets(h, st);
    const int sections[2][2] = {{L.off_etaMass, L.len_etaMass}, {L.off_nkbt, L.NT}};
    for (const auto& sec : sections) std::copy(st.begin() + sec[0], st.begin() + sec[0] + sec[1], h->thermo.h_state.begin() + sec[0]);
    if (h->host_only) return TGNH_OK;
    for (const auto& sec : sections) {
        HIP_OK(hipMemcpyAsync(h->thermo.d_state + sec[0], st.data() + sec[0], sizeof(double) * sec[1], hipMemcpyHostToDevice, s));
        HIP_OK(hipMemcpyAsync(h->thermo.d_stage + sec[0], st.data() + sec[0], sizeof(double) * sec[1], hipMemcpyHostToDevice, s));
    }
    HIP_OK(hipStreamSynchronize(s));
    return TGNH_OK;
}

extern "C" tgnh_status tgnh_get_local_dof_terms(tgnh_handle h, double* terms, int* count) {
    CHECK_H(h);
    if (count) *count = h->thermo.L.NT;
    if (terms) std::copy(h->thermo.local_terms.begin(), h->thermo.local_terms.end(), terms);
    return TGNH_OK;
}
extern "C" tgnh_status tgnh_set_global_dof_terms(tgnh_handle h, const double* terms, int count) {
    CHECK_H(h);
    if (!terms || count != h->thermo.L.NT) return fail(TGNH_ERR_ARG, "dof term count mismatch");
    if (h->run.step_count != 0) return fail(TGNH_ERR_STATE, "global dof must be set before the first step");
    if (!h->host_only) HIP_OK(hipSetDevice(h->device));
    h->thermo.global_terms.assign(terms, terms + count);
    return finalize_thermostat(h);
}
```

### openmm_drudenose_amd/csrc/tgnh_queries.cpp

```cpp
#include "tgnh_host.h"

static tgnh_status read_state(tgnh_handle h, int off, int n, hipStream_t s, double* out) {
    if (!out) return fail(TGNH_ERR_ARG, "null out");
    if (h->host_only) { std::copy(h->thermo.h_state.begin() + off, h->thermo.h_state.begin() + off + n, out); return TGNH_OK; }
    { tgnh_status rc = entry(h, false); if (rc) return rc; }
    { tgnh_status rc = materialize_chain(h, s); if (rc) return rc; }
    HIP_OK(hipMemcpyAsync(out, h->thermo.d_state + off, sizeof(double) * n, hipMemcpyDeviceToHost, s));
    return finish_query(h, s);
}

extern "C" tgnh_status tgnh_get_kinetic_energy(tgnh_handle h, int ke_sum_valid, void* stream, double* out) {
    CHECK_H(h);
    if (!out) return fail(TGNH_ERR_ARG, "null out");
    hipStream_t s = (hipStream_t)stream;
    if (h->d.mode == TGNH_MODE_TGNH && ke_sum_valid)
        return read_state(h, h->thermo.L.off_kesum, 1, s, out);
    tgnh_status rc = entry(h, true); if (rc) return rc;
    rc = flush_impl(h, s); if (rc) return rc;
    const double ts = h->d.mode == TGNH_MODE_DUALNH ? 0.5 * h->d.step_size : 0.0;
    HIP_OK(launch_plain_ke(h->d.precision, h->bound.velm, reinterpret_cast<const long long*>(h->bound.force), h->d.num_particles,
                           h->d.padded_num_particles, ts, h->thermo.d_scalar, s));
    HIP_OK(hipMemcpyAsync(out, h->thermo.d_scalar, sizeof(double), hipMemcpyDeviceToHost, s));
    HIP_OK(hipStreamSynchronize(s));
    return TGNH_OK;
// ... 151 lines not shown
    if (!(threshold >= 0.0) || !std::isfinite(threshold)) return fail(TGNH_ERR_ARG, "tgnh_get_drude_statistics: threshold is negative or not finite");
    if (!(hist_max >= 0.0) || !std::isfinite(hist_max)) return fail(TGNH_ERR_ARG, "tgnh_get_drude_statistics: hist_max is negative or not finite");
    tgnh_status rc = entry(h, true); if (rc) return rc;
    hipStream_t s = (hipStream_t)stream;
    DrudeStatsRow& r = h->dstats.h_row;
    r = DrudeStatsRow{};
    r.worst = 0x7fffffff;
    if (h->d.num_pairs > 0) {
        const int grid = index_grid(h->d.num_particles);
        rc = h->dstats.ensure(grid, true, "internal: the Drude statistics' grid exceeds its rows"); if (rc) return rc;
        if (h->d.precision == TGNH_PREC_MIXED && !h->bound.posq_corr) return fail(TGNH_ERR_STATE, "internal: mixed precision without a position correction");
        const int* partner = nullptr;
        rc = device_partner_table(h, &partner); if (rc) return rc;
        {
            Timed t(h, s, KID_OTHER);
            HIP_OK(launch_drude_stats(h->d.precision, h->bound.posq, h->bound.posq_corr, partner, h->d.num_particles, threshold, hist_max,
                                      h->dstats.d_rows, grid, s));
        }
        HIP_OK(hipMemcpyAsync(&r, h->dstats.d_rows + grid, sizeof(r), hipMemcpyDeviceToHost, s));
    }
    rc = finish_query(h, s); if (rc) return rc;
    double max_d2;
    std::memcpy(&max_d2, &r.max_key, sizeof(max_d2));
    out->worst_particle = r.worst == 0x7fffffff ? -1 : r.worst;
    out->pairs = r.pairs; out->over = r.over;
    out->max_distance = r.worst == 0x7fffffff ? 0.0 : std::sqrt(max_d2);
    out->sum_d2 = r.sum_d2;
    std::copy(r.dipole, r.dipole + 3, out->dipole);
    std::copy(r.hist, r.hist + TGNH_DRUDE_HIST_BINS + 1, out->hist);
    return TGNH_OK;
}

static void drain_events(tgnh_handle h) {
    for (size_t i = 0; i < h->timing.ev_used; i++) {
        auto& e = h->timing.ev_pool[i];
        if (hipEventSynchronize(e.b) != hipSuccess) continue;
        float ms = 0;
        if (hipEventElapsedTime(&ms, e.a, e.b) == hipSuccess) { h->timing.t_total[e.kid] += ms; h->timing.t_count[e.kid] += 1; }
    }
    h->timing.ev_used = 0;
}
extern "C" tgnh_status tgnh_timing_enable(tgnh_handle h, int on) {
    CHECK_H(h);
    if (h->host_only) return fail(TGNH_ERR_STATE, "host-only handle");
    HIP_OK(hipSetDevice(h->device));
    if (!on) drain_events(h);
    else {
        for (int k = 0; k < KID_COUNT; k++) { h->timing.t_total[k] = 0; h->timing.t_count[k] = 0; }
        h->timing.ev_used = 0;
        while (h->timing.ev_pool.size() < 2048) {
            tgnh_context::Timing::Ev e; e.kid = 0;
            if (hipEventCreate(&e.a) != hipSuccess) break;
            if (hipEventCreate(&e.b) != hipSuccess) { (void)hipEventDestroy(e.a); break; }
            h->timing.ev_pool.push_back(e);
        }
    }
    h->timing.on = on != 0;
    h->timing.only = on >= 2 ? on - 2 : -1;
    return TGNH_OK;
}
extern "C" tgnh_status tgnh_timing_read(tgnh_handle h, int kernel, double* total_ms, int64_t* launches) {
    CHECK_H(h);
    if (kernel < 0 || kernel >= KID_COUNT) return fail(TGNH_ERR_ARG, "bad kernel id");
    if (!h->host_only) { HIP_OK(hipSetDevice(h->device)); drain_events(h); }
    if (total_ms) *total_ms = h->timing.t_total[kernel];
    if (launches) *launches = h->timing.t_count[kernel];
    return TGNH_OK;
}
extern "C" tgnh_status tgnh_algorithmic_bytes(tgnh_handle h, int kernel, double* bytes) {
    CHECK_H(h);
    if (!bytes) return fail(TGNH_ERR_ARG, "null out");
    const double N = h->d.num_particles;
    const double V = h->d.precision == TGNH_PREC_SINGLE ? 16 : 32;
    const double F = 24;
    const double X = h->d.precision == TGNH_PREC_SINGLE ? 16 : 32;
    double b = 0;
    switch (kernel) {
        case KID_SKD: b = N * (2 * V + F + 2 * X); break;
        case KID_KICK_KE: b = N * (V + F); break;
        case KID_SCALE: b = N * (2 * V + (h->owed.end_folded ? F : 0)); break;
        case KID_KE: b = N * V; break;
        case KID_FORCE: b = N * (X + F); break;
        case KID_STEP:
            b = (h->d.flags & TGNH_FLAG_DEFER_SCALE) ? N * (3 * V + 2 * F + 2 * X) : N * (6 * V + 3 * F + 2 * X) / 2; break;
        default: b = 0;
    }
    *bytes = b;
    return TGNH_OK;
}
```

### openmm_drudenose_amd/csrc/tgnh_step.cpp

```cpp
#include "tgnh_host.h"

constexpr int64_t STATUS_POLL_EVERY = 64;

void note_status(tgnh_handle h, uint32_t flags) {
    if (h->status.failed_code) return;
    if (flags & 8u) {
        h->status.failed_code = TGNH_ERR_STATE;
        h->status.failed = "resident step (noticed at step " + std::to_string((long long)h->run.step_count) + "): the launch's work-groups did "
                    "not all become resident within the time limit (TGNH_FLAG_RESIDENT_STEP needs the device to itself)";
        if (flags & 4u) h->status.failed += "; the waiting work-groups timed out in turn (status bits 2 and 3)";
    } else if (flags & 16u) {
        h->status.failed_code = TGNH_ERR_STATE;
        h->status.failed = "kinetic-energy pass (noticed at step " + std::to_string((long long)h->run.step_count) + "): work-group 0 did not "
                    "receive every work-group's row of sums within the time limit (the sums were left as NaN: nothing integrated "
                    "on with a partial sum); the device is shared with something that keeps this launch's work-groups from running "
                    "-- or a chain was handed a NaN kinetic energy: with an all-reduce attached, the rank on which that happened";
    } else if (flags & 4u) {
        h->status.failed_code = TGNH_ERR_STATE;
        h->status.failed = "mailbox exchange timed out (noticed at step " + std::to_string((long long)h->run.step_count) +
                    "): a peer did not send its kinetic-energy sums; the run cannot continue";
    } else if ((flags & 1u) && h->d.mode == TGNH_MODE_DUALNH) {
        h->status.failed_code = TGNH_ERR_HARDWALL;
        h->status.failed = "Drude particle moved too far beyond hard wall constraint";
    }
// ... 238 lines not shown
    ChainArgs a{};
    a.L = h->thermo.L; a.st = h->thermo.d_state; a.partials = h->thermo.d_partials; a.nparts = h->run.ke_parts;
    a.nbig = h->topo.num_big;
    a.dt = h->d.step_size; a.S = h->d.drude_steps_per_real_step;
    a.dtc = a.dt / a.S; a.inv_dtc = 1.0 / a.dtc;
    a.realkbT = h->thermo.realkbT; a.drudekbT = h->thermo.drudekbT;
#ifdef TGNH_TUNING
    if (const char* e = getenv("TGNH_CHAIN_LANES")) a.lanes = e[0] != '0';
#endif
    a.stage = h->thermo.d_stage;
    a.status = h->status.d_word;
    if (h->xchg.on) a.x = h->xchg.args;
    a.commit = h->owed.stage_pending ? 1 : 0;
    h->owed.stage_pending = false;
    return a;
}

static tgnh_status commit_stage(tgnh_handle h, hipStream_t s) {
    if (!h->owed.stage_pending) return TGNH_OK;
    ChainArgs a = chain_args(h);
    a.do_sum = 0; a.do_chain = 0;
    HIP_OK(launch_chain(a, s));
    return TGNH_OK;
}

static tgnh_status run_chain(tgnh_handle h, hipStream_t s, bool twice) {
    if (h->gather.chain) return run_chain_gather(h, s, false);
    const bool sum_next = rescale_sums_rows(h, h->run.ke_parts), sum_now = !sum_next && !h->owed.tail_summed;
    const bool mailbox = h->xchg.on, hook = !mailbox && h->xchg.allreduce;
    const bool chain_next = h->cfg.inline_chain;
    const bool chain_with_sum = !chain_next && !hook, chain_alone = !chain_next && hook;
    h->owed.tail_summed = false;
    tgnh_status rc;
    ChainArgs a = chain_args(h);
    a.chain_twice = twice ? 1 : 0;
    if (sum_now || chain_with_sum) {
        a.do_sum = sum_now ? 1 : 0; a.x_send = mailbox ? 1 : 0;
        a.do_chain = chain_with_sum ? 1 : 0; a.x_wait = mailbox && chain_with_sum ? 1 : 0;
        rc = timed_chain(h, a, s); if (rc) return rc;
    }
    if (hook) { rc = allreduce_hook(h, s); if (rc) return rc; }
    if (chain_alone) {
        a.do_sum = 0; a.do_chain = 1; a.commit = 0;
        rc = timed_chain(h, a, s); if (rc) return rc;
    }
    if (chain_next) { h->owed.chain_owed(twice); h->owed.sum_pending |= sum_next; h->owed.xwait_pending |= mailbox; }
    return TGNH_OK;
}

tgnh_status materialize_chain(tgnh_handle h, hipStream_t s) {
    { tgnh_status rc = settle_end(h, s); if (rc) return rc; }
    if (!h->owed.chain_pending) return commit_stage(h, s);
    ChainArgs a = chain_args(h);
    a.do_sum = h->owed.sum_pending ? 1 : 0; a.do_chain = 1; a.chain_twice = h->owed.chain_pending_twice ? 1 : 0;
    a.x_wait = h->owed.xwait_pending ? 1 : 0;
    a.ke_carry = h->owed.carry_pending ? 1 : 0;
    { tgnh_status rc = timed_chain(h, a, s); if (rc) return rc; }
    h->owed.chain_ran();
    return TGNH_OK;
}

static int resident_kernel(tgnh_handle h, int kind) {
    if (!((h->d.flags & TGNH_FLAG_RESIDENT_STEP) && h->cfg.inline_chain && h->cfg.gb != 0 && h->thermo.L.NT <= CHAIN_INLINE_SUM_NT &&
          (h->xchg.on || !h->xchg.allreduce))) return 0;
    if (kind == 0 && h->cfg.wresident_per_cu > 0) return 2;
    return h->cfg.resident_per_cu > 0 && h->thermo.L.C == 1 ? 1 : 0;
}
bool resident_now(tgnh_handle h) { return resident_kernel(h, pass_kind(h->d)) != 0; }

extern "C" tgnh_status tgnh_get_step_path(tgnh_handle h, int* gather, const char** reason) {
    CHECK_H(h);
    if (gather) *gather = h->gather.generic ? (h->gather.chain ? 2 : 1) : 0;
    if (reason) *reason = h->gather.reason.c_str();
    return TGNH_OK;
}

extern "C" tgnh_status tgnh_get_resident_kernel(tgnh_handle h, int* which) {
    CHECK_H(h);
    if (!which) return fail(TGNH_ERR_ARG, "null out");
    *which = resident_kernel(h, pass_kind(h->d));
    return TGNH_OK;
}

static tgnh_status run_resident(tgnh_handle h, hipStream_t s, int kind) {
    if (h->owed.stage_pending) { tgnh_status rc = commit_stage(h, s); if (rc) return rc; }
    TileArgs a = tile_args(h, nullptr);
    const int ops2 = step_kind_ops2(kind);
    if ((ops2 & OP_POSDELTA) && !h->bound.pos_delta) return fail(TGNH_ERR_STATE, "posDelta buffer not bound");
    const bool hw = a.hardwall != 0 && (ops2 & (OP_DRIFT | OP_MOVE));
    const size_t lds = tile_lds_bytes(h->d.precision, ops2, hw, a.use_com != 0);
    const bool wstep = resident_kernel(h, kind) == 2;
    int& grid = h->cfg.resident_grid[kind][hw ? 1 : 0];
    if (grid == 0 && !wstep) {
        int per_cu = std::min(h->cfg.resident_per_cu, step_blocks_per_cu(h->d.precision, h->cfg.gb, kind, lds));
        if (per_cu < 1) return fail(TGNH_ERR_HIP, "step_kernel: occupancy query failed");
        grid = std::max(1, std::min(std::min(h->topo.num_tiles, per_cu * h->cfg.num_cus / h->cfg.resident_share), GRID_CAP));
    }
    a.chain_on = 1;
    a.chain = chain_args(h);
    a.chain.chain_twice = kind == 0 ? 1 : 0;
    a.x_wait = 1;
    if (!h->xchg.on) a.chain.x = h->meet.self_x;
    a.st_in = h->thermo.d_state; a.st_out = h->thermo.d_state;
    a.sync = h->meet.d_sync; a.rows = h->meet.d_rows;
    if (big_com_on(h)) { tgnh_status rc = run_big_com(h, kind == 0 || kind == 2, s); if (rc) return rc; }
    if (wstep && h->cfg.wresident_grid == 0) {
        const int need = (h->topo.num_wtiles + WBLOCK / 64 - 1) / (WBLOCK / 64);
        h->cfg.wresident_grid = std::max(1, std::min(std::min(need, h->cfg.wresident_per_cu * h->cfg.num_cus / h->cfg.resident_share), GRID_CAP));
    }
    const int g = wstep ? h->cfg.wresident_grid : grid;
    a.chain.nparts = g;
    h->run.ke_parts = g;
    { tgnh_status rc = check_launch(h, a, g, wstep ? WBLOCK : TBLOCK, wstep, true); if (rc) return rc; }
    {
        Timed t(h, s, KID_STEP);
        if (wstep) HIP_OK(launch_wstep(h->d.precision, h->cfg.gb, h->thermo.L.C > 1, a, g, s));
        else HIP_OK(launch_step(h->d.precision, h->cfg.gb, kind, a, g, lds, s));
    }
    h->owed.resident_settled();
    return TGNH_OK;
}

static tgnh_status first_half(tgnh_handle h, hipStream_t s) {
    if (h->owed.first_half_done) return TGNH_OK;
    if (h->owed.ke_carry) {
        h->owed.ke_carry = false;
        if (big_com_on(h)) { tgnh_status rc = run_big_com(h, false, s); if (rc) return rc; }
        if (h->cfg.inline_chain) {
            h->owed.chain_owed(false); h->owed.sum_pending = false; h->owed.carry_pending = true;
            return TGNH_OK;
        }
        ChainArgs a = chain_args(h);
        a.do_sum = 0; a.do_chain = 1; a.ke_carry = 1;
        return timed_chain(h, a, s);
    }
    tgnh_status rc = run_tile(h, OP_KE, KID_KE, s); if (rc) return rc;
    return run_chain(h, s, false);
}

tgnh_status entry(tgnh_handle h, bool need_bufs) {
    if (!h) return fail(TGNH_ERR_ARG, "null handle");
    h->owed.g_com_fresh = false;
    if (need_bufs) { tgnh_status rc = need_buffers(h); if (rc) return rc; }
    if (!h->host_only) {
        HIP_OK(hipSetDevice(h->device));
        if (h->status.h_seen) note_status(h, *h->status.h_seen);
    }
    if (h->status.failed_code) return fail(h->status.failed_code, h->status.failed);
    return TGNH_OK;
}

static tgnh_status poll_status_async(tgnh_handle h, hipStream_t s) {
    if (!h->status.h_seen || h->run.step_count % STATUS_POLL_EVERY != 0) return TGNH_OK;
    if (stream_capturing(s)) return TGNH_OK;
    HIP_OK(hipMemcpyAsync(h->status.h_seen, h->status.d_word, sizeof(uint32_t), hipMemcpyDeviceToHost, s));
    return TGNH_OK;
}

static void start_of_step(tgnh_handle h) {
    if (h->cfg.alternate_sweeps) h->run.sweep_reverse = (int)(h->run.step_count & 1);
}
static tgnh_status advance_clock(tgnh_handle h, hipStream_t s) {
    h->run.time += h->d.step_size; h->run.step_count += 1;
    return poll_status_async(h, s);
}

extern "C" tgnh_status tgnh_step_begin(tgnh_handle h, void* stream) {
    tgnh_status rc = entry(h, true); if (rc) return rc;
    hipStream_t s = (hipStream_t)stream;
    rc = cm_removal_due(h, s); if (rc) return rc;
    rc = rescale_due(h, s); if (rc) return rc;
    start_of_step(h);
    if (h->owed.end_pending) {
        if (resident_now(h)) return run_resident(h, s, 0);
        rc = settle_end(h, s); if (rc) return rc;
    }
    if (!(h->d.flags & TGNH_FLAG_DEFER_SCALE) && resident_now(h) && !h->owed.ke_carry)
        return run_resident(h, s, 1);
    rc = first_half(h, s); if (rc) return rc;
    rc = run_tile(h, (h->owed.kick_pending ? OP_PREKICK : 0) | OP_SCALE | OP_KICK | OP_DRIFT, KID_SKD, s); if (rc) return rc;
    h->owed.velocities_current(); h->owed.first_half_done = false;
    return TGNH_OK;
}

static tgnh_status second_half(tgnh_handle h, hipStream_t s, int kick_ops) {
    tgnh_status rc;
    const bool defer = (h->d.flags & TGNH_FLAG_DEFER_SCALE) != 0;
    h->owed.ke_carry = false;
    if (h->owed.scale_pending || h->owed.kick_pending || h->owed.end_pending) { rc = flush_impl(h, s); if (rc) return rc; }
    if (!defer && resident_now(h)) {
        rc = run_resident(h, s, kick_ops ? 2 : 4); if (rc) return rc;
        h->owed.ke_carry = ke_carries(h);
    } else if (kick_ops && resident_now(h)) {
        h->owed.end_pending = true;
    } else {
        const bool fold = !defer && kick_ops != 0 && !h->gather.generic;
        const int nostore = kick_ops && !h->gather.generic ? OP_NOSTORE : 0;
        h->owed.end_folded = fold;
        rc = run_tile(h, kick_ops | OP_KE | nostore, kick_ops ? KID_KICK_KE : KID_KE, s); if (rc) return rc;
        rc = run_chain(h, s, defer); if (rc) return rc;
        if (defer) h->owed.end_half_deferred(nostore != 0);
        else {
            rc = run_tile(h, (fold ? OP_PREKICK : 0) | OP_SCALE, KID_SCALE, s); if (rc) return rc;
            h->owed.ke_carry = ke_carries(h);
        }
    }
    return advance_clock(h, s);
}

extern "C" tgnh_status tgnh_step_end(tgnh_handle h, void* stream) {
    tgnh_status rc = entry(h, true); if (rc) return rc;
    return second_half(h, (hipStream_t)stream, OP_KICK);
}

tgnh_status settle_kick(tgnh_handle h, hipStream_t s) {
    return (h->owed.kick_pending || h->owed.end_pending) ? flush_impl(h, s) : TGNH_OK;
}

tgnh_status settle_end(tgnh_handle h, hipStream_t s) {
    if (!h->owed.end_pending) return TGNH_OK;
    h->owed.end_pending = false;
    tgnh_status rc = run_tile(h, OP_KICK | OP_KE | OP_NOSTORE, KID_KICK_KE, s); if (rc) return rc;
    rc = run_chain(h, s, true); if (rc) return rc;
    h->owed.end_half_deferred(true);
    return TGNH_OK;
}

static tgnh_status split_entry(tgnh_handle h, hipStream_t s, bool fresh_ke) {
    tgnh_status rc = entry(h, true); if (rc) return rc;
    if (fresh_ke) h->owed.ke_carry = false;
    return settle_kick(h, s);
}

extern "C" tgnh_status tgnh_step_begin_kick(tgnh_handle h, void* stream) {
    hipStream_t s = (hipStream_t)stream;
    tgnh_status rc = split_entry(h, s, false); if (rc) return rc;
    rc = cm_removal_due(h, s); if (rc) return rc;
    rc = rescale_due(h, s); if (rc) return rc;
    start_of_step(h);
    if (!(h->d.flags & TGNH_FLAG_DEFER_SCALE) && resident_now(h) && !h->owed.ke_carry) return run_resident(h, s, 3);
    rc = first_half(h, s); if (rc) return rc;
    rc = run_tile(h, OP_SCALE | OP_KICK | OP_POSDELTA, KID_OTHER, s); if (rc) return rc;
    h->owed.scale_pending = false; h->owed.first_half_done = false;
    return TGNH_OK;
}
extern "C" tgnh_status tgnh_step_begin_move(tgnh_handle h, void* stream) {
    tgnh_status rc = split_entry(h, (hipStream_t)stream, true); if (rc) return rc;
    return run_tile(h, OP_MOVE, KID_OTHER, (hipStream_t)stream);
}
extern "C" tgnh_status tgnh_step_end_kick(tgnh_handle h, void* stream) {
    tgnh_status rc = split_entry(h, (hipStream_t)stream, true); if (rc) return rc;
    return run_tile(h, OP_KICK, KID_OTHER, (hipStream_t)stream);
}
extern "C" tgnh_status tgnh_step_end_thermo(tgnh_handle h, void* stream) {
    tgnh_status rc = entry(h, true); if (rc) return rc;
    return second_half(h, (hipStream_t)stream, 0);
}
extern "C" tgnh_status tgnh_half_kick(tgnh_handle h, void* stream) { return tgnh_step_end_kick(h, stream); }

tgnh_status flush_impl(tgnh_handle h, hipStream_t s) {
    tgnh_status rc = settle_end(h, s); if (rc) return rc;
    if (!h->owed.scale_pending && !h->owed.kick_pending) return TGNH_OK;
    rc = materialize_chain(h, s); if (rc) return rc;
    if (h->owed.scale_pending) {
        rc = run_tile(h, (h->owed.kick_pending ? OP_PREKICK : 0) | OP_SCALE, KID_SCALE, s, h->thermo.d_state + h->thermo.L.off_scale_a); if (rc) return rc;
        HIP_OK(hipMemcpyAsync(h->thermo.d_state + h->thermo.L.off_scale, h->thermo.d_state + h->thermo.L.off_scale_b, sizeof(double) * h->thermo.L.NT,
                              hipMemcpyDeviceToDevice, s));
    } else {
        rc = run_tile(h, OP_KICK, KID_OTHER, s); if (rc) return rc;
    }
    if (big_com_on(h)) { rc = run_big_com(h, false, s); if (rc) return rc; }
    h->owed.velocities_current();
    return TGNH_OK;
}

extern "C" tgnh_status tgnh_flush(tgnh_handle h, void* stream) {
    CHECK_H(h);
    if (!h->owed.scale_pending && !h->owed.kick_pending && !h->owed.end_pending) return TGNH_OK;
    tgnh_status rc = entry(h, true); if (rc) return rc;
    return flush_impl(h, (hipStream_t)stream);
}

extern "C" tgnh_status tgnh_note_replayed_steps(tgnh_handle h, int nsteps) {
    CHECK_H(h);
    if (nsteps < 0) return fail(TGNH_ERR_ARG, "negative step count");
    h->run.time += h->d.step_size * nsteps;
    h->run.step_count += nsteps;
    return TGNH_OK;
}

extern "C" tgnh_status tgnh_set_time(tgnh_handle h, double time, int64_t step_count) {
    CHECK_H(h);
    if (step_count < 0) return fail(TGNH_ERR_ARG, "negative step count");
    h->run.time = time;
    h->run.step_count = step_count;
    return TGNH_OK;
}

extern "C" tgnh_status tgnh_get_pending_state(tgnh_handle h, uint32_t* bits) {
    CHECK_H(h);
    if (!bits) return fail(TGNH_ERR_ARG, "null out");
    *bits = h->owed.bits() | (h->run.sweep_reverse ? (uint32_t)tgnh_context::Owed::BIT_SWEEP_REVERSE : 0u);
    return TGNH_OK;
}

extern "C" tgnh_status tgnh_state_changed(tgnh_handle h) {
    CHECK_H(h);
    tgnh_status rc = deferred_guard(h, "tgnh_state_changed");
    if (rc) return rc;
    h->owed.ke_carry = false;
    return TGNH_OK;
}
```

### openmm_drudenose_amd/csrc/tgnh_topology.cpp

```cpp
#include <map>

#include "tgnh_host.h"

std::vector<int> partner_table(const tgnh_context* c) {
    std::vector<int> t(c->d.num_particles, -1);
    for (size_t k = 0; k < c->topo.pair_drude.size(); k++) {
        const int p = c->topo.pair_drude[k], p1 = c->topo.pair_parent[k];
        t[p] = (int)((unsigned)p1 | 0x80000000u); t[p1] = p;
    }
    return t;
}
tgnh_status device_partner_table(tgnh_context* c, const int** out) {
    if (!c->gather.d_partner && !c->by_index.d_partner) HIP_OK(c->by_index.d_partner.upload(partner_table(c)));
    *out = c->gather.d_partner ? c->gather.d_partner : c->by_index.d_partner;
    return TGNH_OK;
}

static tgnh_status build_gather_topology(tgnh_context* c, const std::vector<int>& res_order) {
    const tgnh_desc& d = c->d;
    const int N = d.num_particles;
    const bool com = com_thermostat_on(d);
    c->topo.tile_start.assign(1, N); c->topo.tile_res.assign(1, 0); c->topo.num_tiles = 0;
    c->topo.res_entries.assign(1, make_int2(0, 0));
    c->topo.meta.clear(); c->topo.wave_tile.clear(); c->topo.wmeta.clear(); c->topo.num_wtiles = 0;
// ... 154 lines not shown
    while (start < N && !c->gather.generic) {
        int end = std::min(start + cap, N);
        auto ok = [&](int e) {
            if (e < N && forbid[e] > 0) return false;
            if (com && entries_in(start, e) > TILE_RES) return false;
            return true;
        };
        while (end > start && !ok(end)) end--;
        if (end == start) {
            c->gather.generic = true;
            c->gather.reason = "a Drude pair (or a chain of overlapping pairs) spans more than one 512-slot tile";
            break;
        }
        end = mol_cut(start, end, cap, ok);
        if (align > 1 && end < N) {
            for (int e = end; e > start && e > end - 64; e--)
                if (e % align == 0 && ok(e)) { end = e; break; }
        }
        c->topo.tile_start.push_back(start);
        start = end;
    }
    c->topo.tile_start.push_back(N);
    c->topo.num_tiles = (int)c->topo.tile_start.size() - 1;
    if (c->gather.generic) return build_gather_topology(c, res_order);

    std::vector<int2> entries;
    c->topo.tile_res.assign(c->topo.num_tiles + 1, 0);
    c->topo.meta.assign(N, 0);
    for (int t = 0; t < c->topo.num_tiles; t++) {
        c->topo.tile_res[t] = (int)entries.size();
        int prev_res = -1, local = -1;
        for (int i = c->topo.tile_start[t]; i < c->topo.tile_start[t + 1]; i++) {
            if (com && c->topo.resid[i] != prev_res) {
                prev_res = c->topo.resid[i];
                local++;
                entries.push_back(is_big[prev_res] ? make_int2(-(big_index[prev_res] + 1), 0)
                                                   : make_int2(c->topo.res_count[prev_res], c->topo.res_first[prev_res]));
            }
            int off = 0;
            if (partner[i] >= 0) {
                off = partner[i] - i;
                if (partner[i] < c->topo.tile_start[t] || partner[i] >= c->topo.tile_start[t + 1] || off < -1024 || off > 1023)
                    return fail(TGNH_ERR_STATE, "internal: Drude partner outside its tile");
            }
            c->topo.meta[i] = pack_meta((uint32_t)role[i], (uint32_t)c->topo.group[i], off, (uint32_t)(com ? local : 0));
        }
        if (com && local + 1 > TILE_RES) return fail(TGNH_ERR_STATE, "internal: too many molecules in a tile");
    }
    c->topo.tile_res[c->topo.num_tiles] = (int)entries.size();
    if (entries.empty()) entries.push_back(make_int2(0, 0));
    c->topo.res_entries = entries;
    c->topo.num_big = (int)c->topo.big_first.size();

    c->topo.wave_tile.clear(); c->topo.wmeta.clear(); c->topo.num_wtiles = 0;
    if (c->topo.num_big == 0) {
        std::vector<int2> wt;
        bool fits = true;
        for (int st = 0; st < N && fits;) {
            int end = std::min(st + WAVE_SLOTS, N);
            while (end > st && end < N && forbid[end] > 0) end--;
            if (end == st) { fits = false; break; }
            end = mol_cut(st, end, WAVE_SLOTS, [&](int e) { return forbid[e] == 0; });
            int maxn = 1;
            if (com) for (int i = st; i < end; i++) maxn = std::max(maxn, c->topo.res_count[c->topo.resid[i]]);
            wt.push_back(make_int2(st, maxn));
            st = end;
        }
        if (fits) {
            c->topo.num_wtiles = (int)wt.size();
            wt.push_back(make_int2(N, 0));
            c->topo.wmeta.assign(N, 0);
            for (int i = 0; i < N; i++) {
                int pos = 0, n = 1;
                if (com) { const int r = c->topo.resid[i]; pos = i - c->topo.res_first[r]; n = c->topo.res_count[r]; }
                const int off = partner[i] >= 0 ? partner[i] - i : 0;
                c->topo.wmeta[i] = pack_wmeta((uint32_t)role[i], (uint32_t)c->topo.group[i], off, (uint32_t)pos, (uint32_t)(n - 1));
            }
            c->topo.wave_tile = wt;
        }
    }
    {
        std::map<std::vector<uint32_t>, uint32_t> ids, wids;
        auto intern = [&](std::map<std::vector<uint32_t>, uint32_t>& m, std::vector<uint32_t>& store, const uint32_t* w, int P,
                          uint32_t limit, uint32_t* id) {
            std::vector<uint32_t> key(w, w + P);
            auto it = m.find(key);
            if (it == m.end()) {
                if (m.size() >= limit) return false;
                it = m.emplace(key, (uint32_t)m.size()).first;
                key.resize(PATTERN_WORDS, 0u);
                store.insert(store.end(), key.begin(), key.end());
            }
            *id = it->second;
            return true;
        };
        c->topo.tile_pat.assign(std::max(c->topo.num_tiles, 1), 0u); c->topo.pattern.clear();
        for (int t = 0; t < c->topo.num_tiles; t++) {
            const int ts = c->topo.tile_start[t], n = c->topo.tile_start[t + 1] - ts;
            for (int P = 1; P <= PATTERN_WORDS && P < n; P++) {
                const uint32_t mols = com ? (c->topo.meta[ts + P] >> 21) - (c->topo.meta[ts] >> 21) : 0u;
                if (mols > 255u) break;
                bool same = true;
                for (int k = 0; k < n && same; k++)
                    same = c->topo.meta[ts + k] == c->topo.meta[ts + k % P] + (((uint32_t)(k / P) * mols) << 21);
                if (!same) continue;
                uint32_t id;
                if (intern(ids, c->topo.pattern, c->topo.meta.data() + ts, P, 1u << 16, &id))
                    c->topo.tile_pat[t] = (uint32_t)P | (mols << 8) | (id << 16);
                break;
            }
        }
        c->topo.wtile_pat.assign(std::max(c->topo.num_wtiles, 1), 0u); c->topo.wpattern.clear();
        for (int t = 0; t < c->topo.num_wtiles; t++) {
            const int ws = c->topo.wave_tile[t].x, n = c->topo.wave_tile[t + 1].x - ws;
            for (int P = 1; P <= PATTERN_WORDS && P < n; P++) {
                bool same = true;
                for (int k = 0; k < n && same; k++) same = c->topo.wmeta[ws + k] == c->topo.wmeta[ws + k % P];
                if (!same) continue;
                uint32_t id;
                if (intern(wids, c->topo.wpattern, c->topo.wmeta.data() + ws, P, 1u << 16, &id))
                    c->topo.wtile_pat[t] = (uint32_t)P | (id << 8);
                break;
            }
        }
        if (c->topo.pattern.empty()) c->topo.pattern.assign(PATTERN_WORDS, 0u);
        if (c->topo.wpattern.empty()) c->topo.wpattern.assign(PATTERN_WORDS, 0u);
    }
    if (c->host_only) return TGNH_OK;
    HIP_OK(c->topo.d_tile_pat.upload(c->topo.tile_pat));
    HIP_OK(c->topo.d_pattern.upload(c->topo.pattern));
    HIP_OK(c->topo.d_wpattern.upload(c->topo.wpattern));
    HIP_OK(c->topo.d_meta.upload(c->topo.meta));
    HIP_OK(c->topo.d_tile_start.upload(c->topo.tile_start));
    HIP_OK(c->topo.d_tile_res.upload(c->topo.tile_res));
    HIP_OK(c->topo.d_res_table.upload(c->topo.res_entries));
    if (!c->topo.wave_tile.empty()) {
        std::vector<int2> packed = c->topo.wave_tile;
        for (int t = 0; t < c->topo.num_wtiles; t++) packed[t].y |= (int)(c->topo.wtile_pat[t] << 8);
        HIP_OK(c->topo.d_wave_tile.upload(packed));
        HIP_OK(c->topo.d_wmeta.upload(c->topo.wmeta));
    }
    if (c->topo.num_big) {
        std::vector<int2> bt(c->topo.num_big);
        for (int k = 0; k < c->topo.num_big; k++) bt[k] = make_int2(c->topo.big_count[k], c->topo.big_first[k]);
        HIP_OK(c->topo.d_big_table.upload(bt));
        HIP_OK(c->topo.d_big_com.alloc(32 * (size_t)c->topo.num_big, true));
    }
    return TGNH_OK;
}

void local_dof_terms(tgnh_context* c) {
    const tgnh_desc& d = c->d;
    const int N = d.num_particles, P = d.num_pairs;
    const int NT = c->thermo.L.NT;
    c->thermo.local_terms.assign(NT, 0.0);
    if (d.mode == TGNH_MODE_DUALNH) {
        double real = 0;
        for (int i = 0; i < N; i++) real += (c->topo.mass[i] == 0.0 ? 0 : 3);
        real -= 3.0 * P;
        real -= d.num_constraints;
        c->thermo.local_terms[0] = real;
        c->thermo.local_terms[2] = 3.0 * P;
        return;
    }
    const int G = d.num_groups, R = d.num_residues;
    std::vector<double> resInv(R, 0.0);
    {
        std::vector<double> rm(R, 0.0);
        for (int i = 0; i < N; i++) rm[c->topo.resid[i]] += c->topo.mass[i];
        for (int r = 0; r < R; r++) resInv[r] = 1.0 / rm[r];
    }
    std::vector<double> dof(G, 0.0), red(G, 0.0);
    for (int i = 0; i < N; i++) {
        if (c->topo.mass[i] != 0.0) {
            dof[c->topo.group[i]] += 3;
            if (d.use_com_temp_group) red[c->topo.group[i]] += 3 * c->topo.mass[i] * resInv[c->topo.resid[i]];
        }
    }
    for (int i = 0; i < P; i++) dof[c->topo.group[c->topo.pair_drude[i]]] -= 3;
    for (int i = 0; i < d.num_constraints; i++) {
        if (d.constraint_i) dof[c->topo.group[d.constraint_i[i]]] -= 1; else dof[0] -= 1;
    }
    for (int g = 0; g < G; g++) c->thermo.local_terms[g] = dof[g] - red[g];
    c->thermo.local_terms[G] = d.use_com_temp_group ? 3.0 * R : 0.0;
    c->thermo.local_terms[G + 1] = 3.0 * P;
}

tgnh_status check_temperatures(double temperature, double drude_temperature) {
    if (!(temperature >= 0) || !std::isfinite(temperature) || !(drude_temperature >= 0) || !std::isfinite(drude_temperature))
        return fail(TGNH_ERR_ARG, "a temperature must be finite and not negative");
    return TGNH_OK;
}
void set_bath_temperatures(tgnh_context* c, double temperature, double drude_temperature) {
    c->d.temperature = temperature; c->d.drude_temperature = drude_temperature;
    c->thermo.realkbT = c->d.kB * temperature;
    c->thermo.drudekbT = c->d.kB * drude_temperature;
}

std::vector<double> thermostat_nkt(const tgnh_context* c, double realkbT, double drudekbT) {
    const ChainLayout& L = c->thermo.L;
    std::vector<double> nkbt(L.NT, 0.0);
    if (c->d.mode == TGNH_MODE_DUALNH) {
        nkbt[0] = c->thermo.dof[0] * realkbT; nkbt[2] = c->thermo.dof[2] * drudekbT;
    } else {
        for (int i = 0; i < L.G + 1; i++) nkbt[i] = c->thermo.dof[i] * realkbT;
        nkbt[L.G + 1] = c->thermo.dof[L.G + 1] * drudekbT;
// ... 115 lines not shown
```

### openmm_drudenose_amd/csrc/tgnh_wave_device.h

```cpp
#ifndef TGNH_WAVE_DEVICE_H_
#define TGNH_WAVE_DEVICE_H_
#include "tgnh_tile_device.h"

namespace tgnh {

struct PatternWord {
    uint32_t pat = 0u, word = 0u;
    __device__ __forceinline__ bool of(const TileArgs& a, const uint32_t p, const int lane) {
        if ((p & 255u) == 0u) return false;
        if (p != pat) {
            const int period = (int)(p & 255u);
            const int q = (int)(((float)lane + 0.5f) * __builtin_amdgcn_rcpf((float)period));
            word = a.wpattern[(p >> 8) * PATTERN_WORDS + (uint32_t)(lane - q * period)];
            pat = p;
        }
        return true;
    }
};

template <int PREC> struct WaveIn {
    typename Prec<PREC>::mixed4 v;
    uint32_t meta;
    long long fx, fy, fz;
};

template <int PREC, int OPS>
__device__ __forceinline__ void wave_load(const TileArgs& a, const int ws, const int n, const bool patterned, const uint32_t pword, const int lane, WaveIn<PREC>& in) {
    typedef typename Prec<PREC>::mixed mixed;
    typedef typename Prec<PREC>::mixed4 mixed4;
    const mixed4* __restrict__ velm = reinterpret_cast<const mixed4*>(a.velm);
    const int idx = ws + lane;
    mixed4 v = mk4((mixed)0, (mixed)0, (mixed)0, (mixed)0);
    uint32_t meta = 64u << 10;
    long long fx = 0, fy = 0, fz = 0;
    if (lane < n) {
        v = velm[idx];
        if (!patterned) meta = a.wmeta[idx];
        if (OPS & OP_KICK) {
            fx = a.force[idx];
            fy = a.force[idx + a.padded];
            fz = a.force[idx + 2 * a.padded];
        }
    }
    if (patterned && lane < n) meta = pword;
    in.v = v; in.meta = meta; in.fx = fx; in.fy = fy; in.fz = fz;
}

template <int PREC> struct WStepIn {
    typename Prec<PREC>::mixed4 v;
    uint32_t meta;
    long long fx, fy, fz;
    typename Prec<PREC>::real4 p;
    float4 c;
    typename Prec<PREC>::mixed mass, cx, cy, cz;
};

struct WaveBounds { int ws, y, n; };

template <int PREC, int GB> struct WaveStep {
    typedef typename Prec<PREC>::real real;
    typedef typename Prec<PREC>::mixed mixed;
    typedef typename Prec<PREC>::real4 real4;
    typedef typename Prec<PREC>::mixed4 mixed4;
    const TileArgs& a;
    TileEnv<PREC, GB>* e;
    const double* s_scale;
    mixed *ix, *iy, *iz, *im, *jx, *jy, *jz;
    mixed4* __restrict__ velm; real4* __restrict__ posq; float4* __restrict__ pcorr;
    int lane, G, nw;
    bool use_com, hardwall;
    mixed dt, fscale;
    PatternWord pw;
    __device__ __forceinline__ WaveStep(const TileArgs& a_, TileEnv<PREC, GB>* e_, const double* s_scale_, mixed* img, const int lane_)
        : a(a_), e(e_), s_scale(s_scale_), ix(img), iy(img + WAVE_SLOTS), iz(img + 2 * WAVE_SLOTS), im(img + 3 * WAVE_SLOTS),
          jx(img + 4 * WAVE_SLOTS), jy(img + 5 * WAVE_SLOTS), jz(img + 6 * WAVE_SLOTS),
          velm(reinterpret_cast<mixed4*>(a_.velm)), posq(reinterpret_cast<real4*>(a_.posq)), pcorr(reinterpret_cast<float4*>(a_.posq_corr)),
          lane(lane_), G(a_.num_groups), nw(a_.num_wtiles), use_com(a_.use_com != 0), hardwall(a_.hardwall != 0),
          dt((mixed)a_.dt), fscale((mixed)(0.5 * a_.dt / 4294967296.0)) {}
    __device__ __forceinline__ static void wfence() {
        __builtin_amdgcn_fence(__ATOMIC_RELEASE, "wavefront");
        __builtin_amdgcn_wave_barrier();
        __builtin_amdgcn_fence(__ATOMIC_ACQUIRE, "wavefront");
    }
    __device__ __forceinline__ void bounds(const int ww, WaveBounds& b) const {
        const int2* t = a.wave_tile + (a.reverse ? nw - 1 - ww : ww);
        b.ws = t[0].x; b.y = t[0].y; b.n = t[1].x - b.ws;
    }
    __device__ __forceinline__ void load_vf(const WaveBounds& b, WStepIn<PREC>& in) {
        const int idx = b.ws + lane;
        const bool patterned = pw.of(a, (uint32_t)b.y >> 8, lane);
        mixed4 v = mk4((mixed)0, (mixed)0, (mixed)0, (mixed)0);
        uint32_t meta = 64u << 10;
        long long fx = 0, fy = 0, fz = 0;
        if (lane < b.n) {
            v = reinterpret_cast<const mixed4*>(a.velm)[idx];
            if (!patterned) meta = a.wmeta[idx];
            fx = a.force[idx]; fy = a.force[idx + a.padded]; fz = a.force[idx + 2 * a.padded];
        }
        if (patterned && lane < b.n) meta = pw.word;
        in.v = v; in.meta = meta; in.fx = fx; in.fy = fy; in.fz = fz;
    }
    __device__ __forceinline__ void load_x(const WaveBounds& b, WStepIn<PREC>& in) const {
        const int idx = b.ws + lane;
        if (lane < b.n) {
            in.p = reinterpret_cast<const real4*>(a.posq)[idx];
            if (PREC == TGNH_PREC_MIXED) in.c = reinterpret_cast<const float4*>(a.posq_corr)[idx];
        }
    }
    template <bool KICK = true>
    __device__ __forceinline__ void prepare(WStepIn<PREC>& t, const WaveBounds& bd, const bool ke) {
        mixed4& v = t.v;
        const uint32_t m = t.meta;
        t.mass = v.w != 0 ? rcp_(v.w) : (mixed)0;
        if (KICK) {
            const mixed c = fscale * v.w;
            v.x += c * force_as(t.fx, (mixed)0);
            v.y += c * force_as(t.fy, (mixed)0);
            v.z += c * force_as(t.fz, (mixed)0);
        }
        ix[lane] = v.x; iy[lane] = v.y; iz[lane] = v.z; im[lane] = t.mass;
        wfence();
        mixed cx = 0, cy = 0, cz = 0;
        if (use_com) {
            const int j = (int)((m >> 17) & 63u), n1 = (int)((m >> 23) & 63u);
            const int first = lane - j;
            mixed px = 0, py = 0, pz = 0, pm = 0;
            for (int k = 0; k < (bd.y & 255); k++) {
                if (k <= n1) {
                    const mixed um = im[first + k];
                    px += ix[first + k] * um; py += iy[first + k] * um; pz += iz[first + k] * um; pm += um;
                }
            }
            const mixed wq = rcp_(pm);
            cx = px * wq; cy = py * wq; cz = pz * wq;
            if (ke && j == 0 && lane < bd.n)
                e->ke_com += ((double)cx * cx + (double)cy * cy + (double)cz * cz) * (double)pm;
        }
        t.cx = cx; t.cy = cy; t.cz = cz;
        if (ke) {
            const uint32_t role = m & 3u, g = (m >> 2) & 255u;
            const double rx = v.x - cx, ry = v.y - cy, rz = v.z - cz;
            double val = v.w != 0 ? (rx * rx + ry * ry + rz * rz) * (double)t.mass : 0.0;
            if (role == ROLE_DRUDE) {
                const int pl = lane + (int)((m >> 10) & 127u) - 64;
                const double dx = ix[pl] - v.x, dy = iy[pl] - v.y, dz = iz[pl] - v.z;
                const double mass1 = t.mass, mass2 = im[pl];
                const double mu = mass1 * mass2 * rcp_(mass1 + mass2);
                const double d = (dx * dx + dy * dy + dz * dz) * mu;
                e->ke_drude += d;
                val -= d;
            }
#pragma unroll
            for (int b = 0; b < GB; b++) e->ke_g[b] += (g == (uint32_t)b) ? val : 0.0;
        }
    }
    __device__ __forceinline__ void finish(WStepIn<PREC>& t, const WaveBounds& bd) {
        mixed4 v = t.v;
        const uint32_t m = t.meta;
        const uint32_t role = m & 3u, g = (m >> 2) & 255u;
        const int pl = lane + (int)((m >> 10) & 127u) - 64;
        const mixed mass = t.mass, cx = t.cx, cy = t.cy, cz = t.cz;
        const mixed s_com = (mixed)s_scale[G], s_drude = (mixed)s_scale[G + 1], s_g = (mixed)s_scale[g];
        mixed px = t.p.x, py = t.p.y, pz = t.p.z;
        const real pq = t.p.w;
        if (PREC == TGNH_PREC_MIXED) { px += (mixed)t.c.x; py += (mixed)t.c.y; pz += (mixed)t.c.z; }
        if (role == ROLE_NORMAL) {
            if (v.w != 0) {
                const mixed rx = v.x - cx, ry = v.y - cy, rz = v.z - cz;
                v.x = s_g * rx + s_com * (v.x - rx);
                v.y = s_g * ry + s_com * (v.y - ry);
                v.z = s_g * rz + s_com * (v.z - rz);
            }
        } else {
            const mixed ux = ix[pl], uy = iy[pl], uz = iz[pl], um = im[pl];
            const mixed rsx = v.x - cx, rsy = v.y - cy, rsz = v.z - cz;
            const mixed rpx = ux - cx, rpy = uy - cy, rpz = uz - cz;
            const mixed invTot = rcp_(mass + um);
            const mixed msf = invTot * mass, mpf = invTot * um;
            const mixed sdp = s_drude * mpf;
            v.x = s_g * (rsx * msf + rpx * mpf) + sdp * (rsx - rpx) + s_com * (v.x - rsx);
            v.y = s_g * (rsy * msf + rpy * mpf) + sdp * (rsy - rpy) + s_com * (v.y - rsy);
            v.z = s_g * (rsz * msf + rpz * mpf) + sdp * (rsz - rpz) + s_com * (v.z - rsz);
        }
        if (v.w != 0) {
            const mixed c = fscale * v.w;
            v.x += c * force_as(t.fx, (mixed)0);
            v.y += c * force_as(t.fy, (mixed)0);
            v.z += c * force_as(t.fz, (mixed)0);
            px += dt * v.x; py += dt * v.y; pz += dt * v.z;
        }
        if (hardwall) {
            wfence();
            ix[lane] = v.x; iy[lane] = v.y; iz[lane] = v.z;
            jx[lane] = px; jy[lane] = py; jz[lane] = pz;
            wfence();
            if (role != ROLE_NORMAL) {
                const mixed maxd = (mixed)a.max_dist, hws = (mixed)a.hw_scale;
                const mixed sxd = px - jx[pl], syd = py - jy[pl], szd = pz - jz[pl];
                const mixed d2 = sxd * sxd + syd * syd + szd * szd;
                if (d2 > maxd * maxd) {
                    const mixed4 uv = mk4(ix[pl], iy[pl], iz[pl], im[pl]);
                    const bool is_d = role == ROLE_DRUDE;
                    const mixed4 vel1 = is_d ? v : uv, vel2 = is_d ? uv : v;
                    const mixed dx = is_d ? sxd : -sxd, dy = is_d ? syd : -syd, dz = is_d ? szd : -szd;
                    const mixed r = sqrt_(d2);
                    const mixed rInv = rcp_(r);
                    if (rInv * maxd < (mixed)0.5) atomicOr(a.status, 1u);
                    const mixed bx = dx * rInv, by = dy * rInv, bz = dz * rInv;
                    const mixed mass1 = is_d ? mass : uv.w, mass2 = is_d ? uv.w : mass;
                    const mixed deltaR = r - maxd;
                    mixed deltaT = dt;
                    mixed dotvr1 = vel1.x * bx + vel1.y * by + vel1.z * bz;
                    const mixed vp1x = vel1.x - bx * dotvr1, vp1y = vel1.y - by * dotvr1, vp1z = vel1.z - bz * dotvr1;
                    const mixed invTot = rcp_(mass1 + mass2);
                    mixed dotvr2 = vel2.x * bx + vel2.y * by + vel2.z * bz;
                    const mixed vp2x = vel2.x - bx * dotvr2, vp2y = vel2.y - by * dotvr2, vp2z = vel2.z - bz * dotvr2;
                    const mixed vbCMass = (mass1 * dotvr1 + mass2 * dotvr2) * invTot;
                    dotvr1 -= vbCMass;
                    dotvr2 -= vbCMass;
                    if (dotvr1 != dotvr2) deltaT = deltaR / abs_(dotvr1 - dotvr2);
                    if (deltaT > dt) deltaT = dt;
                    const mixed vBond = hws / sqrt_(mass1);
                    dotvr1 = -dotvr1 * vBond * mass2 * invTot / abs_(dotvr1);
                    dotvr2 = -dotvr2 * vBond * mass1 * invTot / abs_(dotvr2);
                    const mixed dr1 = -deltaR * mass2 * invTot + deltaT * dotvr1;
                    const mixed dr2 = deltaR * mass1 * invTot + deltaT * dotvr2;
                    dotvr1 += vbCMass;
                    dotvr2 += vbCMass;
                    if (is_d) {
                        px += bx * dr1; py += by * dr1; pz += bz * dr1;
                        v.x = vp1x + bx * dotvr1; v.y = vp1y + by * dotvr1; v.z = vp1z + bz * dotvr1;
                    } else {
                        px += bx * dr2; py += by * dr2; pz += bz * dr2;
                        v.x = vp2x + bx * dotvr2; v.y = vp2y + by * dotvr2; v.z = vp2z + bz * dotvr2;
                    }
                }
            }
        }
        wfence();
        if (lane < bd.n) {
            const int idx = bd.ws + lane;
            velm[idx] = v;
            store_position<PREC>(posq, pcorr, idx, px, py, pz, pq);
        }
    }
};

}
#endif
```

### openmm_drudenose_amd/csrc/tgnh_wave_kernels.h

```cpp
#ifndef TGNH_WAVE_KERNELS_H_
#define TGNH_WAVE_KERNELS_H_
#include "tgnh_wave_device.h"
#include "tgnh_meet_device.h"

namespace tgnh {

template <int PREC, int OPS, int GB>
__global__ __launch_bounds__(TBLOCK, TGNH_MINWAVES) void wke_kernel(const TileArgs a) {
    typedef typename Prec<PREC>::mixed mixed;
    typedef typename Prec<PREC>::mixed4 mixed4;
    constexpr bool DO_KICK = (OPS & OP_KICK) != 0, STORE = DO_KICK && !(OPS & OP_NOSTORE);
    static_assert(GB > 0, "register bins only");
    __shared__ double sred[TBLOCK / 64][GB + 2];
    __shared__ mixed s_img[TBLOCK / 64][4][WAVE_SLOTS];
    const int tid = threadIdx.x, lane = tid & 63;
    const int wv = __builtin_amdgcn_readfirstlane(tid >> 6);
    mixed* const ix = s_img[wv][0]; mixed* const iy = s_img[wv][1]; mixed* const iz = s_img[wv][2]; mixed* const im = s_img[wv][3];
    const int G = a.num_groups;
    const bool use_com = a.use_com != 0;
    const mixed fscale = (mixed)(0.5 * a.dt / 4294967296.0);
    mixed4* __restrict__ velm = reinterpret_cast<mixed4*>(a.velm);
    commit_staged(a, tid, TBLOCK);
    double ke_g[GB], ke_com = 0.0, ke_drude = 0.0;
#pragma unroll
// ... 45 lines not shown
            const double d = (dx * dx + dy * dy + dz * dz) * mu;
            ke_drude += d;
            val -= d;
        }
#pragma unroll
        for (int b = 0; b < GB; b++) ke_g[b] += (g == (uint32_t)b) ? val : 0.0;
        __builtin_amdgcn_fence(__ATOMIC_RELEASE, "wavefront");
        __builtin_amdgcn_wave_barrier();
        __builtin_amdgcn_fence(__ATOMIC_ACQUIRE, "wavefront");
    };

    int w = __builtin_amdgcn_readfirstlane((int)blockIdx.x * (TBLOCK / 64) + wv);
    Bounds b0{}, b1{}, b2{};
    WaveIn<PREC> A, B;
    PatternWord pw;
    auto load = [&](const Bounds& b, WaveIn<PREC>& in) {
        const bool patterned = pw.of(a, (uint32_t)b.y >> 8, lane);
        wave_load<PREC, OPS>(a, b.ws, b.n, patterned, pw.word, lane, in);
    };
    if (w < nw) { bounds(w, b0); load(b0, A); }
    if (w + stride < nw) bounds(w + stride, b1);
    while (w < nw) {
        if (w + 2 * stride < nw) bounds(w + 2 * stride, b2);
        if (w + stride < nw) load(b1, B);
        work(A, b0);
        w += stride;
        if (w >= nw) break;
        if (w + 2 * stride < nw) bounds(w + 2 * stride, b0);
        if (w + stride < nw) load(b2, A);
        work(B, b1);
        w += stride;
        b1 = b0; b0 = b2;
    }
#pragma unroll
    for (int b = 0; b < GB; b++) ke_g[b] = wave_sum(ke_g[b]);
    ke_com = wave_sum(ke_com);
    ke_drude = wave_sum(ke_drude);
    if (lane == 0) {
#pragma unroll
        for (int b = 0; b < GB; b++) sred[wv][b] = ke_g[b];
        sred[wv][GB] = ke_com;
        sred[wv][GB + 1] = ke_drude;
    }
    __syncthreads();
    if (tid < GB + 2) {
        double t = 0.0;
#pragma unroll
        for (int k = 0; k < TBLOCK / 64; k++) t += sred[k][tid];
        const int b = tid < GB ? tid : G + (tid - GB);
        if (tid >= GB || tid < G) {
            if (a.tail_sum) {
                unsigned long long* cell = a.rows + row_word((int)blockIdx.x, 2 * b);
                store_tagged(cell, cell + 64, (unsigned long long)(gen0 + 1u) << 32, t);
            } else a.partials[(size_t)blockIdx.x * (G + 2) + b] = t;
        }
    }
    if (a.tail_sum && blockIdx.x == 0) {
        __shared__ double s_tail[TBLOCK / 64][GB + 2];
        const int NT = G + 2;
        double acc[GB + 2];
#pragma unroll
        for (int b = 0; b < GB + 2; b++) acc[b] = 0.0;
        const bool ok = collect_rows<GB, false, TBLOCK>(a, tid, (int)gridDim.x, NT, (unsigned long long)(gen0 + 1u), acc);
        if (!ok) atomicOr(a.status, 16u);
#pragma unroll
        for (int b = 0; b < GB + 2; b++) {
            if (b < NT) {
                const double t = wave_sum(acc[b]);
                if (lane == 0) s_tail[wv][b] = t;
            }
        }
        const bool all_ok = __syncthreads_and(ok ? 1 : 0) != 0;
        if (tid < NT) {
            double t = 0.0;
#pragma unroll
            for (int k = 0; k < TBLOCK / 64; k++) t += s_tail[k][tid];
            a.ke_red[tid] = all_ok ? t : __longlong_as_double(0x7ff8000000000000ll);
        }
        if (tid == 0) a.sync[1] = gen0 + 1u;
    }
}


template <int PREC, int GB, bool MULTI = false>
__global__ __launch_bounds__(WBLOCK) void wstep_kernel(const TileArgs a) {
    typedef typename Prec<PREC>::mixed mixed;
    static_assert(GB > 0, "register bins only");
    __shared__ double s_scale[MAX_GROUPS + 2];
    __shared__ double s_part[WBLOCK / 64][CHAIN_INLINE_SUM_NT];
    __shared__ double s_x[64 + XCHG_MAX_WORLD * CHAIN_INLINE_SUM_NT];
    __shared__ int s_go;
    __shared__ unsigned s_gen;
    __shared__ unsigned long long s_seq1;
    __shared__ mixed s_img[WBLOCK / 64][7][WAVE_SLOTS];
    __shared__ double s_block[256];
    const int tid = threadIdx.x, lane = tid & 63, G = a.num_groups, NT = G + 2;
    const int wv = __builtin_amdgcn_readfirstlane(tid >> 6);
    const bool chain_wave = tid < 64;
    const int itg = tid & 63;
    if (a.census) { census(a); return; }
    TileEnv<PREC, GB> e;
    e.tid = tid; e.G = G; e.smem = nullptr; e.wbins0 = nullptr; e.s_scale = s_scale;
    e.clear_ke();
    WaveStep<PREC, GB> ws(a, &e, s_scale, &s_img[wv][0][0], lane);
    typedef WaveBounds Bounds;
    auto bounds = [&](const int ww, Bounds& b) { ws.bounds(ww, b); };
    auto load_vf = [&](const Bounds& b, WStepIn<PREC>& in) { ws.load_vf(b, in); };
    auto load_x = [&](const Bounds& b, WStepIn<PREC>& in) { ws.load_x(b, in); };
    auto prepare = [&](WStepIn<PREC>& t, const Bounds& bd, const bool ke) { ws.template prepare<true>(t, bd, ke); };
    auto finish = [&](WStepIn<PREC>& t, const Bounds& bd) { ws.finish(t, bd); };
    auto wfence = [] { WaveStep<PREC, GB>::wfence(); };

    unsigned gen0 = 0;
    unsigned long long seq0 = 0;
    Chain1Regs creg{};
    if (chain_wave) {
        gen0 = __hip_atomic_load(&a.sync[1], __ATOMIC_RELAXED, __HIP_MEMORY_SCOPE_AGENT);
        seq0 = __hip_atomic_load(a.chain.x.seq, __ATOMIC_RELAXED, __HIP_MEMORY_SCOPE_AGENT);
        if (itg < NT && !(MULTI && a.chain.L.C > 1)) creg = chain1_load(a.chain, a.st_in, itg);
    }
    if (MULTI && a.chain.L.C > 1 && tid < a.chain.L.total) s_block[tid] = a.st_in[tid];

    const int nw = a.num_wtiles, stride = (int)gridDim.x * (WBLOCK / 64);

    TRACE(0);
    const int w0 = __builtin_amdgcn_readfirstlane((int)blockIdx.x * (WBLOCK / 64) + wv);
    const bool have = w0 < nw;
    int w = w0;
    Bounds b0{}, b1{};
    WStepIn<PREC> cur;
    if (have) {
        bounds(w, b0);
        if (w + stride < nw) bounds(w + stride, b1);
        load_vf(b0, cur);
    }
    while (have) {
#ifdef TGNH_TRACE
        if (w == w0) { asm volatile("s_waitcnt vmcnt(0)" ::: "memory"); TRACE(3); }
#endif
        prepare(cur, b0, true);
#ifdef TGNH_TRACE
        if (w == w0) TRACE(4);
#endif
        if (w + stride >= nw) break;
        wfence();
        w += stride;
        b0 = b1;
        if (w + stride < nw) bounds(w + stride, b1);
        load_vf(b0, cur);
    }
    const int w_last = w;
    TRACE(1);
    MeetShared sh{s_scale, s_part, s_x, &s_go, &s_gen, &s_seq1, s_block};
    if (!step_meet<PREC, GB, true, WBLOCK, MULTI>(a, e, gen0, seq0, creg, sh, [&] {
            if (have) {
                load_x(b0, cur);
                if (w_last - stride >= 0) bounds(w_last - stride, b1);
            }
        })) return;

    TRACE(9);
    if (have) {
        w = w_last;
        finish(cur, b0);
        TRACE(5);
        while (w - stride >= 0) {
            w -= stride;
            b0 = b1;
            if (w - stride >= 0) bounds(w - stride, b1);
            load_vf(b0, cur); load_x(b0, cur);
            prepare(cur, b0, false);
            finish(cur, b0);
        }
    }
    TRACE(15);
}

template <int PREC, int OPS> static tile_fn_t wke_fn_gb(int gb) {
    if (gb <= 1) return wke_kernel<PREC, OPS, 1>;
    if (gb <= 4) return wke_kernel<PREC, OPS, 4>;
    return wke_kernel<PREC, OPS, 8>;
}
template <int PREC> static tile_fn_t wke_fn_ops(int ops, int gb) {
    switch (ops) {
        case OP_KE: return wke_fn_gb<PREC, OP_KE>(gb);
        case OP_KICK | OP_KE: return wke_fn_gb<PREC, OP_KICK | OP_KE>(gb);
        case OP_KICK | OP_KE | OP_NOSTORE: return wke_fn_gb<PREC, OP_KICK | OP_KE | OP_NOSTORE>(gb);
        default: return nullptr;
    }
}
static tile_fn_t wke_fn(int precision, int ops, int gb) {
    if (gb == 0) return nullptr;
    return with_precision(precision, [&](auto P) -> tile_fn_t { return wke_fn_ops<decltype(P)::value>(ops, gb); });
}
hipError_t launch_wke(int precision, int ops, int gb, const TileArgs& a, int grid, hipStream_t s) {
    tile_fn_t fn = wke_fn(precision, ops, gb);
    if (!fn) return hipErrorInvalidValue;
    TGNH_LAUNCH(fn, dim3(grid), dim3(TBLOCK), 0, s, a);
    return hipGetLastError();
}
int wke_blocks_per_cu(int precision, int ops, int gb) { return blocks_per_cu(wke_fn(precision, ops, gb), TBLOCK, 0); }

template <int PREC, bool MULTI> static tile_fn_t wstep_fn_gb(int gb) {
    return gb <= 1 ? wstep_kernel<PREC, 1, MULTI> : gb <= 4 ? wstep_kernel<PREC, 4, MULTI> : wstep_kernel<PREC, 8, MULTI>;
}
static tile_fn_t wstep_fn(int precision, int gb, bool multi) {
    if (gb == 0) return nullptr;
    return with_precision(precision, [&](auto P) -> tile_fn_t {
        return multi ? wstep_fn_gb<decltype(P)::value, true>(gb) : wstep_fn_gb<decltype(P)::value, false>(gb);
    });
}
hipError_t launch_wstep(int precision, int gb, bool multi, const TileArgs& a, int grid, hipStream_t s) {
    tile_fn_t fn = wstep_fn(precision, gb, multi);
    if (!fn) return hipErrorInvalidValue;
    TGNH_LAUNCH(fn, dim3(grid), dim3(WBLOCK), 0, s, a);
    return hipGetLastError();
}
int wstep_blocks_per_cu(int precision, int gb, bool multi) { return blocks_per_cu(wstep_fn(precision, gb, multi), WBLOCK, 0); }

}
#endif
```

### openmm_drudenose_amd/drudetgnhplugin.py

```python
import ctypes as C

import numpy as np

from . import _lib
from ._lib import (MODE_DUALNH, MODE_TGNH, PREC_SINGLE, PREC_MIXED, PREC_DOUBLE,
                   FLAG_DEFER_SCALE, FLAG_RESIDENT_STEP, FLAG_WAVE_TILES, FLAG_TRUST_STATE_CHANGED, FLAG_GATHER)
from .synth import KB

_PREC = {"single": PREC_SINGLE, "mixed": PREC_MIXED, "double": PREC_DOUBLE}
_MODE = {"dualNH": MODE_DUALNH, "TGNH": MODE_TGNH}


class TgnhError(RuntimeError):

    def __init__(self, status, message):
        super().__init__(message)
        self.status = status


def _check(rc):
    if rc != _lib.TGNH_OK:
        raise TgnhError(rc, _lib.load().tgnh_last_error().decode())


# ... 888 lines not shown
        self.force.view(3, self.padded)[:, :self.n] = (t * 4294967296.0).to(self.torch.int64).t()

    def compute_forces(self):
        if self.force_fn is not None:
            self.force_fn(self)
        else:
            _check(self.lib.tgnh_harness_force(self.h, self._x0_arg(), self.k_drude, self.k_tether,
                                               self.force.data_ptr(), self._stream()))
        if self.site_forces:
            self.distribute_site_forces()

    def step_begin(self):
        _check(self.lib.tgnh_step_begin(self.h, self._stream()))

    def step_end(self):
        _check(self.lib.tgnh_step_end(self.h, self._stream()))
        self.ke_sum_valid = True

    def step(self, steps):
        if self.force_fn is None and self.constrained:
            _check(self.lib.tgnh_run_harness_constrained(self.h, self._x0_arg(), self.k_drude, self.k_tether,
                                                         self.integrator.getConstraintTolerance(), int(steps), self._stream()))
            if steps > 0:
                self.ke_sum_valid = True
            return
        if self.force_fn is None:
            _check(self.lib.tgnh_run_harness(self.h, self._x0_arg(), self.k_drude, self.k_tether, int(steps), self._stream()))
            if steps > 0:
                self.ke_sum_valid = True
            return
        lib, h = self.lib, self.h
        for _ in range(steps):
            if self.state_hook is not None:
                self.state_hook(self)
            if not self.constrained:
                self.step_begin()
                self.compute_forces()
                self.step_end()
                continue
            tol = self.integrator.getConstraintTolerance()
            _check(lib.tgnh_step_begin_kick(h, self._stream()))
            _check(lib.tgnh_harness_shake_positions(h, tol, self._stream()))
            _check(lib.tgnh_apply_constraints(h, tol, self._stream()))
            _check(lib.tgnh_step_begin_move(h, self._stream()))
            self._place_sites()
            self.compute_forces()
            _check(lib.tgnh_step_end_kick(h, self._stream()))
            if self.mode == MODE_TGNH:
                _check(lib.tgnh_harness_shake_velocities(h, tol, self._stream()))
                _check(lib.tgnh_apply_velocity_constraints(h, tol, self._stream()))
            _check(lib.tgnh_step_end_thermo(h, self._stream()))
            self.ke_sum_valid = True

    def step_without_forces(self, steps):
        if self.constrained:
            raise TgnhError(_lib.ERR_STATE, "step_without_forces: unconstrained systems only")
        _check(self.lib.tgnh_run_steps(self.h, int(steps), self._stream()))
        if steps > 0:
            self.ke_sum_valid = True

    def capture_steps(self, steps, forces=True):
        torch = self.torch
        if self.force_fn is not None:
            raise TgnhError(_lib.ERR_STATE, "capture_steps supports the harness force call-out only")
        for what, every in (("centre-of-mass removal", self.cm_motion_removal), ("velocity rescaling", self.velocity_rescaling)):
            if every > 0 and (self.time()[1] % every or int(steps) % every):
                raise TgnhError(_lib.ERR_STATE, f"capture_steps: with {what} every {every} steps, the step count at the "
                                f"capture ({self.time()[1]}) and the steps captured ({int(steps)}) must both be multiples of it")
        torch.cuda.synchronize(self.dev)
        def record():
            g = torch.cuda.CUDAGraph()
            with torch.cuda.graph(g):
                if self.constrained and not forces:
                    raise TgnhError(_lib.ERR_STATE, "capture_steps(forces=False): unconstrained systems only")
                if self.constrained:
                    _check(self.lib.tgnh_run_harness_constrained(self.h, self._x0_arg(), self.k_drude, self.k_tether,
                                                                 self.integrator.getConstraintTolerance(), int(steps), self._stream()))
                elif not forces:
                    _check(self.lib.tgnh_run_steps(self.h, int(steps), self._stream()))
                else:
                    _check(self.lib.tgnh_run_harness(self.h, self._x0_arg(), self.k_drude, self.k_tether, int(steps), self._stream()))
            return g
        for _ in range(4):
            owed_before = self.pending_state() & 0x2ff
            first = record()
            if self.pending_state() & 0x2ff == owed_before:
                break
            first.replay()
            torch.cuda.synchronize(self.dev)
            self.ke_sum_valid = True
        else:
            raise TgnhError(_lib.ERR_STATE, "capture_steps: the handle does not reach a steady state of its step sequence")
        clock = self.time()
        graphs = [first, record()]
        if self.pending_state() & 0x2ff != owed_before:
            raise TgnhError(_lib.ERR_STATE, "capture_steps: the step sequence is not periodic")
        self.set_time(*clock)
        self._captured_not_run = int(steps)
        turn = [0]
        baths = self._bath_epoch

        def replay():
            if self._bath_epoch != baths:
                raise TgnhError(_lib.ERR_STATE, "capture_steps: the temperatures were changed after these steps were recorded "
                                "(their launches hold the old kT): capture them again")
            graphs[turn[0] & 1].replay()
            turn[0] += 1
            if self._captured_not_run:
                self._captured_not_run = 0
            else:
                _check(self.lib.tgnh_note_replayed_steps(self.h, int(steps)))
            self.ke_sum_valid = True
        replay.graph = graphs[0]
        replay.graphs = graphs
        return replay

    def pending_state(self):
        bits = C.c_uint32()
        _check(self.lib.tgnh_get_pending_state(self.h, C.byref(bits)))
        return bits.value

    def status_flags(self):
        flags = C.c_uint32()
        self.lib.tgnh_get_status_flags(self.h, self._stream(), C.byref(flags))
        return flags.value

    def check(self):
        flags = C.c_uint32()
        _check(self.lib.tgnh_get_status_flags(self.h, self._stream(), C.byref(flags)))
        return flags.value

    def _vec(self, fn, n):
        out = np.zeros(n)
        _check(fn(self.h, self._stream(), out.ctypes.data_as(_lib.c_f64p)))
        return out

    def last_kinetic_energies(self):
        return self._vec(self.lib.tgnh_get_last_kinetic_energies, self.num_thermostats())

    def last_scale_factors(self):
        return self._vec(self.lib.tgnh_get_last_scale_factors, self.num_thermostats())

    def compute_kinetic_energies(self):
        _check(self.lib.tgnh_compute_kinetic_energies(self.h, self._stream()))
        return self.last_kinetic_energies()

    def half_kick(self):
        _check(self.lib.tgnh_half_kick(self.h, self._stream()))

    def kinetic_energy(self):
        out = C.c_double()
        _check(self.lib.tgnh_get_kinetic_energy(self.h, int(self.ke_sum_valid), self._stream(), C.byref(out)))
        return out.value

    def drude_statistics(self, threshold=None, hist_max=0.0):
        if threshold is None:
            threshold = self.integrator.getMaxDrudeDistance()
        st = _lib.TgnhDrudeStats()
        st.struct_size = C.sizeof(st)
        _check(self.lib.tgnh_get_drude_statistics(self.h, float(threshold), float(hist_max), self._stream(), C.byref(st)))
        return DrudeStatistics(st, float(threshold), float(hist_max))

    def time(self):
        t, k = C.c_double(), C.c_int64()
        _check(self.lib.tgnh_get_time(self.h, C.byref(t), C.byref(k)))
        return t.value, k.value

    def set_time(self, time, step_count):
        _check(self.lib.tgnh_set_time(self.h, float(time), int(step_count)))

    def timing(self, on):
        _check(self.lib.tgnh_timing_enable(self.h, int(on)))

    def timing_read(self, kid):
        ms, n = C.c_double(), C.c_int64()
        _check(self.lib.tgnh_timing_read(self.h, kid, C.byref(ms), C.byref(n)))
        return ms.value, n.value

    def algorithmic_bytes(self, kid):
        b = C.c_double()
        _check(self.lib.tgnh_algorithmic_bytes(self.h, kid, C.byref(b)))
        return b.value
```

Baseline: 4158 steps/s.

## Keep velocities in SoA planes with per-pattern inverse mass during resident steps

While the resident wave-step kernel runs back-to-back steps, velocities move out of the interleaved velm (x,y,z,invmass) array into three planar arrays, and inverse mass is taken from a per-pattern table. This cuts velocity traffic to three words per particle instead of four. Entry happens after a streak of steady steps and a one-time device check that masses match the pattern table. Any path that reads velm converts the data back first, which adds state-tracking complexity, an extra conversion kernel, and a host sync on the first check.

```diff
diff --git a/include/drude_tgnh.h b/include/drude_tgnh.h
--- a/include/drude_tgnh.h
+++ b/include/drude_tgnh.h
@@ -114,6 +114,7 @@
 tgnh_status tgnh_flush(tgnh_handle h, void* stream);
 tgnh_status tgnh_note_replayed_steps(tgnh_handle h, int nsteps);
 tgnh_status tgnh_get_pending_state(tgnh_handle h, uint32_t* bits);
+tgnh_status tgnh_get_velocity_planes(tgnh_handle h, int32_t out[4]);
 tgnh_status tgnh_set_time(tgnh_handle h, double time, int64_t step_count);
 tgnh_status tgnh_state_changed(tgnh_handle h);
 
diff --git a/openmm_drudenose_amd/_lib.py b/openmm_drudenose_amd/_lib.py
--- a/openmm_drudenose_amd/_lib.py
+++ b/openmm_drudenose_amd/_lib.py
@@ -102,6 +102,7 @@
     "tgnh_rccl_shutdown": (C.c_int, [C.c_void_p]),
     "tgnh_exchange_wait_stats": (C.c_int, [C.c_void_p, C.c_void_p, c_f64p, c_f64p, C.POINTER(C.c_int64)]),
     "tgnh_get_pending_state": (C.c_int, [C.c_void_p, C.POINTER(C.c_uint32)]),
+    "tgnh_get_velocity_planes": (C.c_int, [C.c_void_p, C.POINTER(C.c_int32)]),
     "tgnh_set_resident_share": (C.c_int, [C.c_void_p, C.c_int]),
     "tgnh_get_resident_work_groups": (C.c_int, [C.c_void_p, C.POINTER(C.c_int)]),
     "tgnh_get_resident_kernel": (C.c_int, [C.c_void_p, C.POINTER(C.c_int)]),
diff --git a/openmm_drudenose_amd/build.py b/openmm_drudenose_amd/build.py
--- a/openmm_drudenose_amd/build.py
+++ b/openmm_drudenose_amd/build.py
@@ -9,7 +9,7 @@
            "tgnh_frames.cpp", "tgnh_minimize.cpp", "tgnh_constraints.cpp", "tgnh_virtual_sites.cpp",
            "tgnh_kernels.hip", "tgnh_gather.hip", "tgnh_harness.hip", "tgnh_velinit.hip", "tgnh_drude_stats.hip", "tgnh_cm_motion.hip",
            "tgnh_rescale.hip", "tgnh_scale_positions.hip", "tgnh_wrap.hip", "tgnh_minimize.hip", "tgnh_constraints.hip",
-           "tgnh_virtual_sites.hip"]
+           "tgnh_virtual_sites.hip", "tgnh_vplanes.hip"]
 HEADERS = sorted(n for n in os.listdir(CSRC) if n.endswith(".h")) + [os.path.join("..", "..", "include", "drude_tgnh.h")]
 ARCH = "gfx950"
 
diff --git a/openmm_drudenose_amd/csrc/tgnh_constraints.cpp b/openmm_drudenose_amd/csrc/tgnh_constraints.cpp
--- a/openmm_drudenose_amd/csrc/tgnh_constraints.cpp
+++ b/openmm_drudenose_amd/csrc/tgnh_constraints.cpp
@@ -127,6 +127,7 @@
     h->owed.ke_carry = false;
     if (h->cons.count == 0) return TGNH_OK;
     HIP_OK(hipSetDevice(h->device));
+    rc = velm_current(h, (hipStream_t)stream); if (rc) return rc;
     HIP_OK(launch_constrain_velocities(h->d.precision, constraint_args(h, tol), (hipStream_t)stream));
     return TGNH_OK;
 }
diff --git a/openmm_drudenose_amd/csrc/tgnh_context.h b/openmm_drudenose_amd/csrc/tgnh_context.h
--- a/openmm_drudenose_amd/csrc/tgnh_context.h
+++ b/openmm_drudenose_amd/csrc/tgnh_context.h
@@ -64,6 +64,8 @@
         std::vector<uint32_t> wmeta;
         std::vector<uint32_t> tile_pat, wtile_pat;
         std::vector<uint32_t> pattern, wpattern;
+        std::vector<double> wpat_mass;
+        bool wpat_all_uniform = false;
         int num_wtiles = 0;
         tgnh::DeviceBuf<uint32_t> d_meta, d_wmeta, d_tile_pat, d_pattern, d_wpattern;
         tgnh::DeviceBuf<int> d_tile_start, d_tile_res;
@@ -184,6 +186,16 @@
         int wresident_per_cu = 0, wresident_grid = 0;
         int resident_per_cu = 0;
     } cfg;
+    struct VelPlanes {
+        tgnh::DeviceBytes d_planes;
+        tgnh::DeviceBytes d_invm;
+        tgnh::DeviceBuf<uint32_t> d_mismatch;
+        int verdict = 0;
+        int streak = 0;
+        bool pinned = false;
+        hipStream_t stream = nullptr;
+        bool usable() const { return d_planes.get() != nullptr && verdict >= 0 && !pinned; }
+    } vp;
     struct Owed {
         bool end_pending = false;
         bool scale_pending = false;
@@ -194,6 +206,7 @@
         bool xwait_pending = false;
         bool stage_pending = false;
         bool ke_carry = false;
+        bool planes_live = false;
         bool chain_pending_twice = false;
         bool carry_pending = false;
         bool tail_summed = false;
@@ -202,7 +215,7 @@
         enum : uint32_t { BIT_SWEEP_REVERSE = 1u << 8 };
         uint32_t bits() const {
             return end_pending | scale_pending << 1 | kick_pending << 2 | first_half_done << 3 | chain_pending << 4 | sum_pending << 5 |
-                   xwait_pending << 6 | stage_pending << 7 | ke_carry << 9;
+                   xwait_pending << 6 | stage_pending << 7 | ke_carry << 9 | planes_live << 10;
         }
         void chain_owed(bool twice) { chain_pending = true; chain_pending_twice = twice; }
         void chain_ran() { chain_pending = sum_pending = xwait_pending = carry_pending = false; }
diff --git a/openmm_drudenose_amd/csrc/tgnh_harness.hip b/openmm_drudenose_amd/csrc/tgnh_harness.hip
--- a/openmm_drudenose_amd/csrc/tgnh_harness.hip
+++ b/openmm_drudenose_amd/csrc/tgnh_harness.hip
@@ -453,6 +453,8 @@
 #define H_FAIL(code, msg) do { tgnh_set_error(msg); return code; } while (0)
 #define H_HIP(expr) do { hipError_t e_ = (expr); if (e_ != hipSuccess) { tgnh_set_error(std::string(#expr) + ": " + hipGetErrorString(e_)); return TGNH_ERR_HIP; } } while (0)
 
+tgnh_status velm_current(tgnh_handle h, hipStream_t s) __attribute__((visibility("hidden")));
+
 static tgnh_status harness_ready(tgnh_handle h) {
     if (!h) H_FAIL(TGNH_ERR_ARG, "null handle");
     if (h->host_only) H_FAIL(TGNH_ERR_STATE, "host-only handle (device -1): no GPU work can be launched on it");
@@ -497,6 +499,7 @@
     h->owed.ke_carry = false;
     if (h->harness.num_clusters == 0) return TGNH_OK;
     H_HIP(hipSetDevice(h->device));
+    rc = velm_current(h, (hipStream_t)stream); if (rc) return rc;
     H_HIP(launch_shake<true>(h->d.precision, cluster_args(h, tol), (hipStream_t)stream));
     return TGNH_OK;
 }
@@ -568,6 +571,7 @@
     h->owed.ke_carry = false;
     H_HIP(hipSetDevice(h->device));
     hipStream_t s = (hipStream_t)stream;
+    rc = velm_current(h, s); if (rc) return rc;
     auto fn = with_precision(h->d.precision, [](auto P) { return &cmm_kernel<decltype(P)::value>; });
     if (!fn) H_FAIL(TGNH_ERR_ARG, "unknown precision");
     TGNH_LAUNCH(fn, dim3(1), dim3(BLOCK), 0, s, h->bound.velm, h->d.num_particles);
diff --git a/openmm_drudenose_amd/csrc/tgnh_host.h b/openmm_drudenose_amd/csrc/tgnh_host.h
--- a/openmm_drudenose_amd/csrc/tgnh_host.h
+++ b/openmm_drudenose_amd/csrc/tgnh_host.h
@@ -11,6 +11,7 @@
 #include "tgnh_minimize.h"
 #include "tgnh_rescale.h"
 #include "tgnh_scale_positions.h"
+#include "tgnh_vplanes.h"
 
 using namespace tgnh;
 
@@ -51,6 +52,7 @@
 tgnh_status materialize_chain(tgnh_handle h, hipStream_t s);
 tgnh_status settle_kick(tgnh_handle h, hipStream_t s);
 tgnh_status settle_end(tgnh_handle h, hipStream_t s);
+tgnh_status velm_current(tgnh_handle h, hipStream_t s);
 tgnh_status flush_impl(tgnh_handle h, hipStream_t s);
 tgnh_status ke_query_launches(tgnh_handle h, hipStream_t s);
 tgnh_status cm_removal_due(tgnh_handle h, hipStream_t s);
diff --git a/openmm_drudenose_amd/csrc/tgnh_internal.h b/openmm_drudenose_amd/csrc/tgnh_internal.h
--- a/openmm_drudenose_amd/csrc/tgnh_internal.h
+++ b/openmm_drudenose_amd/csrc/tgnh_internal.h
@@ -160,6 +160,8 @@
     const double* st_in;
     double* st_out;
     ChainArgs chain;
+    void* vplanes;
+    const void* wpat_invm;
 };
 
 struct BigComArgs {
@@ -239,7 +241,7 @@
 int step_blocks_per_cu(int precision, int gb, int kind, size_t lds);
 int step_kind_ops2(int kind);
 hipError_t launch_wstep(int precision, int gb, bool multi, const TileArgs& a, int grid, hipStream_t s);
-int wstep_blocks_per_cu(int precision, int gb, bool multi);
+int wstep_blocks_per_cu(int precision, int gb, bool multi, bool planes = false);
 hipError_t launch_wke(int precision, int ops, int gb, const TileArgs& a, int grid, hipStream_t s);
 int wke_blocks_per_cu(int precision, int ops, int gb);
 hipError_t launch_chain(const ChainArgs& a, hipStream_t s);
diff --git a/openmm_drudenose_amd/csrc/tgnh_lifecycle.cpp b/openmm_drudenose_amd/csrc/tgnh_lifecycle.cpp
--- a/openmm_drudenose_amd/csrc/tgnh_lifecycle.cpp
+++ b/openmm_drudenose_amd/csrc/tgnh_lifecycle.cpp
@@ -151,6 +151,22 @@
                   &c->cfg.wresident_per_cu);
 }
 
+static tgnh_status allocate_velocity_planes(tgnh_context* c) {
+    if (const char* e = getenv("TGNH_VELOCITY_PLANES")) if (e[0] == '0') return TGNH_OK;
+    if (!(c->d.flags & TGNH_FLAG_DEFER_SCALE) || c->cfg.wresident_per_cu <= 0 || !c->topo.wpat_all_uniform) return TGNH_OK;
+    if (c->d.precision == TGNH_PREC_SINGLE) return TGNH_OK;
+    if (wstep_blocks_per_cu(c->d.precision, c->cfg.gb, c->thermo.L.C > 1, true) < c->cfg.wresident_per_cu) return TGNH_OK;
+    const bool single = c->d.precision == TGNH_PREC_SINGLE;
+    const size_t word = single ? sizeof(float) : sizeof(double), n = c->topo.wpat_mass.size();
+    std::vector<double> inv(n);
+    for (size_t k = 0; k < n; k++) inv[k] = c->topo.wpat_mass[k] == 0.0 ? 0.0 : 1.0 / c->topo.wpat_mass[k];
+    std::vector<float> inv_f(inv.begin(), inv.end());
+    HIP_OK(c->vp.d_invm.upload(reinterpret_cast<const unsigned char*>(single ? (const void*)inv_f.data() : (const void*)inv.data()), n * word));
+    HIP_OK(c->vp.d_mismatch.alloc(1, true));
+    HIP_OK(c->vp.d_planes.alloc(3 * (size_t)c->d.padded_num_particles * word, true));
+    return TGNH_OK;
+}
+
 extern "C" tgnh_status tgnh_create(const tgnh_desc* d, tgnh_handle* out) {
     if (!d || !out) return fail(TGNH_ERR_ARG, "null argument");
     bool long_chain = false;
@@ -187,6 +203,7 @@
     if (!host_only) {
         rc = allocate(c); if (rc) return rc;
         rc = resident_census(c); if (rc) return rc;
+        rc = allocate_velocity_planes(c); if (rc) return rc;
     }
     rc = finalize_thermostat(c); if (rc) return rc;
     *out = owner.release();
@@ -228,6 +245,10 @@
         }
     }
     h->owed.ke_carry = false;
+    if (velm != h->bound.velm) {
+        tgnh_status rc = velm_current(h, h->vp.stream); if (rc) return rc;
+        h->vp.verdict = 0; h->vp.pinned = false; h->vp.streak = 0;
+    }
     if (posq != h->bound.posq || posq_correction != h->bound.posq_corr) h->snap.valid = false;
     h->bound.posq = posq; h->bound.posq_corr = posq_correction; h->bound.velm = velm; h->bound.force = force; h->bound.pos_delta = pos_delta;
     return TGNH_OK;
diff --git a/openmm_drudenose_amd/csrc/tgnh_queries.cpp b/openmm_drudenose_amd/csrc/tgnh_queries.cpp
--- a/openmm_drudenose_amd/csrc/tgnh_queries.cpp
+++ b/openmm_drudenose_amd/csrc/tgnh_queries.cpp
@@ -257,7 +257,7 @@
         case KID_KE: b = N * V; break;
         case KID_FORCE: b = N * (X + F); break;
         case KID_STEP:
-            b = (h->d.flags & TGNH_FLAG_DEFER_SCALE) ? N * (3 * V + 2 * F + 2 * X) : N * (6 * V + 3 * F + 2 * X) / 2; break;
+            b = (h->d.flags & TGNH_FLAG_DEFER_SCALE) ? N * (3 * (h->owed.planes_live ? 0.75 * V : V) + 2 * F + 2 * X) : N * (6 * V + 3 * F + 2 * X) / 2; break;
         default: b = 0;
     }
     *bytes = b;
diff --git a/openmm_drudenose_amd/csrc/tgnh_step.cpp b/openmm_drudenose_amd/csrc/tgnh_step.cpp
--- a/openmm_drudenose_amd/csrc/tgnh_step.cpp
+++ b/openmm_drudenose_amd/csrc/tgnh_step.cpp
@@ -344,14 +344,57 @@
     return TGNH_OK;
 }
 
+constexpr int PLANES_AFTER_STEPS = 8;
+
+static tgnh_status leave_planes(tgnh_handle h, hipStream_t s) {
+    if (!h->owed.planes_live) return TGNH_OK;
+    HIP_OK(launch_planes_to_velm(h->d.precision, h->vp.d_planes, h->bound.velm, h->d.num_particles, h->d.padded_num_particles, s));
+    h->owed.planes_live = false;
+    return TGNH_OK;
+}
+
+static tgnh_status enter_planes(tgnh_handle h, hipStream_t s) {
+    tgnh_context::VelPlanes& vp = h->vp;
+    if (h->owed.planes_live || !vp.usable()) return TGNH_OK;
+    if (stream_capturing(s)) { vp.pinned = true; return TGNH_OK; }
+    if (vp.streak < PLANES_AFTER_STEPS) return TGNH_OK;
+    const bool check = vp.verdict == 0;
+    if (check) HIP_OK(hipMemsetAsync(vp.d_mismatch, 0, sizeof(uint32_t), s));
+    HIP_OK(launch_velm_to_planes(h->d.precision, h->bound.velm, vp.d_planes, h->topo.d_wave_tile, h->topo.num_wtiles, vp.d_invm,
+                                 h->d.padded_num_particles, check ? vp.d_mismatch.get() : nullptr, s));
+    if (check) {
+        uint32_t differs = 1;
+        HIP_OK(hipMemcpyAsync(&differs, vp.d_mismatch, sizeof(uint32_t), hipMemcpyDeviceToHost, s));
+        HIP_OK(hipStreamSynchronize(s));
+        vp.verdict = differs ? -1 : 1;
+        if (differs) return TGNH_OK;
+    }
+    h->owed.planes_live = true;
+    return TGNH_OK;
+}
+
+tgnh_status velm_current(tgnh_handle h, hipStream_t s) {
+    return h->owed.planes_live && !h->owed.end_pending ? settle_end(h, s) : TGNH_OK;
+}
+
+extern "C" tgnh_status tgnh_get_velocity_planes(tgnh_handle h, int32_t out[4]) {
+    CHECK_H(h);
+    if (!out) return fail(TGNH_ERR_ARG, "null out");
+    out[0] = h->owed.planes_live ? 1 : 0; out[1] = h->vp.usable() ? 1 : 0; out[2] = h->vp.streak; out[3] = PLANES_AFTER_STEPS;
+    return TGNH_OK;
+}
+
 static tgnh_status run_resident(tgnh_handle h, hipStream_t s, int kind) {
     if (h->owed.stage_pending) { tgnh_status rc = commit_stage(h, s); if (rc) return rc; }
+    const bool wstep = resident_kernel(h, kind) == 2;
+    if (wstep && kind == 0) { tgnh_status rc = enter_planes(h, s); if (rc) return rc; }
+    else if (h->owed.planes_live) return fail(TGNH_ERR_STATE, "internal: a launch that reads velm while the velocities live in the planes");
     TileArgs a = tile_args(h, nullptr);
+    if (h->owed.planes_live) { a.vplanes = h->vp.d_planes; a.wpat_invm = h->vp.d_invm; h->vp.stream = s; }
     const int ops2 = step_kind_ops2(kind);
     if ((ops2 & OP_POSDELTA) && !h->bound.pos_delta) return fail(TGNH_ERR_STATE, "posDelta buffer not bound");
     const bool hw = a.hardwall != 0 && (ops2 & (OP_DRIFT | OP_MOVE));
     const size_t lds = tile_lds_bytes(h->d.precision, ops2, hw, a.use_com != 0);
-    const bool wstep = resident_kernel(h, kind) == 2;
     int& grid = h->cfg.resident_grid[kind][hw ? 1 : 0];
     if (grid == 0 && !wstep) {
         int per_cu = std::min(h->cfg.resident_per_cu, step_blocks_per_cu(h->d.precision, h->cfg.gb, kind, lds));
@@ -380,6 +423,7 @@
         else HIP_OK(launch_step(h->d.precision, h->cfg.gb, kind, a, g, lds, s));
     }
     h->owed.resident_settled();
+    if (wstep && kind == 0 && h->vp.usable()) h->vp.streak = std::min(h->vp.streak + 1, 1 << 30);
     return TGNH_OK;
 }
 
@@ -433,10 +477,8 @@
     rc = cm_removal_due(h, s); if (rc) return rc;
     rc = rescale_due(h, s); if (rc) return rc;
     start_of_step(h);
-    if (h->owed.end_pending) {
-        if (resident_now(h)) return run_resident(h, s, 0);
-        rc = settle_end(h, s); if (rc) return rc;
-    }
+    if (h->owed.end_pending && resident_now(h)) return run_resident(h, s, 0);
+    rc = settle_end(h, s); if (rc) return rc;
     if (!(h->d.flags & TGNH_FLAG_DEFER_SCALE) && resident_now(h) && !h->owed.ke_carry)
         return run_resident(h, s, 1);
     rc = first_half(h, s); if (rc) return rc;
@@ -450,6 +492,7 @@
     const bool defer = (h->d.flags & TGNH_FLAG_DEFER_SCALE) != 0;
     h->owed.ke_carry = false;
     if (h->owed.scale_pending || h->owed.kick_pending || h->owed.end_pending) { rc = flush_impl(h, s); if (rc) return rc; }
+    if (!(defer && kick_ops && resident_now(h))) { rc = velm_current(h, s); if (rc) return rc; }
     if (!defer && resident_now(h)) {
         rc = run_resident(h, s, kick_ops ? 2 : 4); if (rc) return rc;
         h->owed.ke_carry = ke_carries(h);
@@ -476,13 +519,15 @@
 }
 
 tgnh_status settle_kick(tgnh_handle h, hipStream_t s) {
-    return (h->owed.kick_pending || h->owed.end_pending) ? flush_impl(h, s) : TGNH_OK;
+    return (h->owed.kick_pending || h->owed.end_pending || h->owed.planes_live) ? flush_impl(h, s) : TGNH_OK;
 }
 
 tgnh_status settle_end(tgnh_handle h, hipStream_t s) {
+    if (h->owed.planes_live || h->owed.end_pending) h->vp.streak = 0;
+    tgnh_status rc = leave_planes(h, s); if (rc) return rc;
     if (!h->owed.end_pending) return TGNH_OK;
     h->owed.end_pending = false;
-    tgnh_status rc = run_tile(h, OP_KICK | OP_KE | OP_NOSTORE, KID_KICK_KE, s); if (rc) return rc;
+    rc = run_tile(h, OP_KICK | OP_KE | OP_NOSTORE, KID_KICK_KE, s); if (rc) return rc;
     rc = run_chain(h, s, true); if (rc) return rc;
     h->owed.end_half_deferred(true);
     return TGNH_OK;
@@ -538,7 +583,7 @@
 
 extern "C" tgnh_status tgnh_flush(tgnh_handle h, void* stream) {
     CHECK_H(h);
-    if (!h->owed.scale_pending && !h->owed.kick_pending && !h->owed.end_pending) return TGNH_OK;
+    if (!h->owed.scale_pending && !h->owed.kick_pending && !h->owed.end_pending && !h->owed.planes_live) return TGNH_OK;
     tgnh_status rc = entry(h, true); if (rc) return rc;
     return flush_impl(h, (hipStream_t)stream);
 }
@@ -571,5 +616,7 @@
     tgnh_status rc = deferred_guard(h, "tgnh_state_changed");
     if (rc) return rc;
     h->owed.ke_carry = false;
-    return TGNH_OK;
-}
+    if (h->owed.planes_live) { HIP_OK(hipSetDevice(h->device)); rc = settle_end(h, h->vp.stream); if (rc) return rc; }
+    if (h->vp.verdict > 0) h->vp.verdict = 0;
+    return TGNH_OK;
+}
diff --git a/openmm_drudenose_amd/csrc/tgnh_topology.cpp b/openmm_drudenose_amd/csrc/tgnh_topology.cpp
--- a/openmm_drudenose_amd/csrc/tgnh_topology.cpp
+++ b/openmm_drudenose_amd/csrc/tgnh_topology.cpp
@@ -260,14 +260,17 @@
     {
         std::map<std::vector<uint32_t>, uint32_t> ids, wids;
         auto intern = [&](std::map<std::vector<uint32_t>, uint32_t>& m, std::vector<uint32_t>& store, const uint32_t* w, int P,
-                          uint32_t limit, uint32_t* id) {
+                          uint32_t limit, uint32_t* id, const double* mass = nullptr, bool known_only = false) {
             std::vector<uint32_t> key(w, w + P);
+            if (mass) { key.resize(3 * (size_t)P); std::memcpy(key.data() + P, mass, sizeof(double) * P); }
             auto it = m.find(key);
             if (it == m.end()) {
-                if (m.size() >= limit) return false;
+                if (known_only || m.size() >= limit) return false;
                 it = m.emplace(key, (uint32_t)m.size()).first;
-                key.resize(PATTERN_WORDS, 0u);
-                store.insert(store.end(), key.begin(), key.end());
+                std::vector<uint32_t> words(w, w + P);
+                words.resize(PATTERN_WORDS, 0u);
+                store.insert(store.end(), words.begin(), words.end());
+                if (mass) { c->topo.wpat_mass.insert(c->topo.wpat_mass.end(), mass, mass + P); c->topo.wpat_mass.resize(store.size(), 0.0); }
             }
             *id = it->second;
             return true;
@@ -288,18 +291,23 @@
                 break;
             }
         }
-        c->topo.wtile_pat.assign(std::max(c->topo.num_wtiles, 1), 0u); c->topo.wpattern.clear();
+        c->topo.wtile_pat.assign(std::max(c->topo.num_wtiles, 1), 0u); c->topo.wpattern.clear(); c->topo.wpat_mass.clear();
+        c->topo.wpat_all_uniform = c->topo.num_wtiles > 0;
         for (int t = 0; t < c->topo.num_wtiles; t++) {
             const int ws = c->topo.wave_tile[t].x, n = c->topo.wave_tile[t + 1].x - ws;
-            for (int P = 1; P <= PATTERN_WORDS && P < n; P++) {
+            for (int P = 1; P <= PATTERN_WORDS && P <= n; P++) {
                 bool same = true;
                 for (int k = 0; k < n && same; k++) same = c->topo.wmeta[ws + k] == c->topo.wmeta[ws + k % P];
                 if (!same) continue;
                 uint32_t id;
-                if (intern(wids, c->topo.wpattern, c->topo.wmeta.data() + ws, P, 1u << 16, &id))
+                if (intern(wids, c->topo.wpattern, c->topo.wmeta.data() + ws, P, 1u << 16, &id, c->topo.mass.data() + ws, P == n)) {
                     c->topo.wtile_pat[t] = (uint32_t)P | (id << 8);
+                    for (int k = 0; k < n; k++)
+                        if (std::memcmp(&c->topo.mass[ws + k], &c->topo.wpat_mass[(size_t)id * PATTERN_WORDS + k % P], sizeof(double))) c->topo.wpat_all_uniform = false;
+                }
                 break;
             }
+            if (!c->topo.wtile_pat[t]) c->topo.wpat_all_uniform = false;
         }
         if (c->topo.pattern.empty()) c->topo.pattern.assign(PATTERN_WORDS, 0u);
         if (c->topo.wpattern.empty()) c->topo.wpattern.assign(PATTERN_WORDS, 0u);
diff --git a/openmm_drudenose_amd/csrc/tgnh_vplanes.h b/openmm_drudenose_amd/csrc/tgnh_vplanes.h
--- /dev/null
+++ b/openmm_drudenose_amd/csrc/tgnh_vplanes.h
@@ -0,0 +1,14 @@
+#ifndef TGNH_VPLANES_H_
+#define TGNH_VPLANES_H_
+
+#include "tgnh_internal.h"
+
+namespace tgnh {
+
+hipError_t launch_velm_to_planes(int precision, const void* velm, void* planes, const int2* wave_tile, int num_wtiles,
+                                 const void* wpat_invm, int padded, uint32_t* mismatch, hipStream_t s);
+hipError_t launch_planes_to_velm(int precision, const void* planes, void* velm, int n, int padded, hipStream_t s);
+
+}
+
+#endif
diff --git a/openmm_drudenose_amd/csrc/tgnh_vplanes.hip b/openmm_drudenose_amd/csrc/tgnh_vplanes.hip
--- /dev/null
+++ b/openmm_drudenose_amd/csrc/tgnh_vplanes.hip
@@ -0,0 +1,61 @@
+#include "tgnh_vplanes.h"
+#include "tgnh_device_math.h"
+
+namespace tgnh {
+
+__device__ __forceinline__ bool same_bits(const float a, const float b) { return __float_as_uint(a) == __float_as_uint(b); }
+__device__ __forceinline__ bool same_bits(const double a, const double b) { return __double_as_longlong(a) == __double_as_longlong(b); }
+
+template <int PREC>
+__global__ __launch_bounds__(BLOCK) void velm_to_planes_kernel(const void* __restrict__ velm_, void* __restrict__ planes_, const int2* __restrict__ wave_tile,
+                                                               const int num_wtiles, const void* __restrict__ invm_, const int padded,
+                                                               uint32_t* __restrict__ mismatch) {
+    typedef typename Prec<PREC>::mixed mixed;
+    typedef typename Prec<PREC>::mixed4 mixed4;
+    const int lane = (int)threadIdx.x & 63;
+    const int t = (int)blockIdx.x * (BLOCK / 64) + ((int)threadIdx.x >> 6);
+    if (t >= num_wtiles) return;
+    const int ws = wave_tile[t].x, n = wave_tile[t + 1].x - ws;
+    if (lane >= n) return;
+    const int idx = ws + lane;
+    const mixed4 v = reinterpret_cast<const mixed4*>(velm_)[idx];
+    mixed* __restrict__ planes = reinterpret_cast<mixed*>(planes_);
+    planes[idx] = v.x; planes[idx + padded] = v.y; planes[idx + 2 * padded] = v.z;
+    if (mismatch) {
+        const uint32_t p = (uint32_t)wave_tile[t].y >> 8;
+        const int period = (int)(p & 255u);
+        bool same = false;
+        if (period) same = same_bits(reinterpret_cast<const mixed*>(invm_)[(p >> 8) * PATTERN_WORDS + (uint32_t)(lane % period)], v.w);
+        if (!same) atomicOr(mismatch, 1u);
+    }
+}
+
+template <int PREC>
+__global__ __launch_bounds__(BLOCK) void planes_to_velm_kernel(const void* __restrict__ planes_, void* __restrict__ velm_, const int n, const int padded) {
+    typedef typename Prec<PREC>::mixed mixed;
+    typedef typename Prec<PREC>::mixed4 mixed4;
+    const mixed* __restrict__ planes = reinterpret_cast<const mixed*>(planes_);
+    mixed4* __restrict__ velm = reinterpret_cast<mixed4*>(velm_);
+    const long long i = (long long)blockIdx.x * BLOCK + threadIdx.x;
+    if (i >= n) return;
+    mixed4 v = velm[i];
+    v.x = planes[i]; v.y = planes[i + padded]; v.z = planes[i + 2ll * padded];
+    velm[i] = v;
+}
+
+hipError_t launch_velm_to_planes(int precision, const void* velm, void* planes, const int2* wave_tile, int num_wtiles,
+                                 const void* wpat_invm, int padded, uint32_t* mismatch, hipStream_t s) {
+    if (!velm || !planes || !wave_tile || !wpat_invm || num_wtiles < 1 || padded < 1) return hipErrorInvalidValue;
+    const int grid = (num_wtiles + BLOCK / 64 - 1) / (BLOCK / 64);
+    TGNH_LAUNCH_PREC(velm_to_planes_kernel, precision, dim3(grid), dim3(BLOCK), 0, s, velm, planes, wave_tile, num_wtiles, wpat_invm, padded, mismatch);
+    return hipGetLastError();
+}
+
+hipError_t launch_planes_to_velm(int precision, const void* planes, void* velm, int n, int padded, hipStream_t s) {
+    if (!velm || !planes || n < 1 || padded < n) return hipErrorInvalidValue;
+    const int grid = (n + BLOCK - 1) / BLOCK;
+    TGNH_LAUNCH_PREC(planes_to_velm_kernel, precision, dim3(grid), dim3(BLOCK), 0, s, planes, velm, n, padded);
+    return hipGetLastError();
+}
+
+}
diff --git a/openmm_drudenose_amd/csrc/tgnh_wave_device.h b/openmm_drudenose_amd/csrc/tgnh_wave_device.h
--- a/openmm_drudenose_amd/csrc/tgnh_wave_device.h
+++ b/openmm_drudenose_amd/csrc/tgnh_wave_device.h
@@ -6,16 +6,20 @@
 
 struct PatternWord {
     uint32_t pat = 0u, word = 0u;
-    __device__ __forceinline__ bool of(const TileArgs& a, const uint32_t p, const int lane) {
+    template <typename Also>
+    __device__ __forceinline__ bool of(const TileArgs& a, const uint32_t p, const int lane, Also&& also) {
         if ((p & 255u) == 0u) return false;
         if (p != pat) {
             const int period = (int)(p & 255u);
             const int q = (int)(((float)lane + 0.5f) * __builtin_amdgcn_rcpf((float)period));
-            word = a.wpattern[(p >> 8) * PATTERN_WORDS + (uint32_t)(lane - q * period)];
+            const uint32_t at = (p >> 8) * PATTERN_WORDS + (uint32_t)(lane - q * period);
+            word = a.wpattern[at];
+            also(at);
             pat = p;
         }
         return true;
     }
+    __device__ __forceinline__ bool of(const TileArgs& a, const uint32_t p, const int lane) { return of(a, p, lane, [](uint32_t) {}); }
 };
 
 template <int PREC> struct WaveIn {
@@ -57,7 +61,7 @@
 
 struct WaveBounds { int ws, y, n; };
 
-template <int PREC, int GB> struct WaveStep {
+template <int PREC, int GB, bool PLANES = false> struct WaveStep {
     typedef typename Prec<PREC>::real real;
     typedef typename Prec<PREC>::mixed mixed;
     typedef typename Prec<PREC>::real4 real4;
@@ -67,6 +71,8 @@
     const double* s_scale;
     mixed *ix, *iy, *iz, *im, *jx, *jy, *jz;
     mixed4* __restrict__ velm; real4* __restrict__ posq; float4* __restrict__ pcorr;
+    mixed* __restrict__ vpl;
+    mixed pinvm;
     int lane, G, nw;
     bool use_com, hardwall;
     mixed dt, fscale;
@@ -75,7 +81,7 @@
         : a(a_), e(e_), s_scale(s_scale_), ix(img), iy(img + WAVE_SLOTS), iz(img + 2 * WAVE_SLOTS), im(img + 3 * WAVE_SLOTS),
           jx(img + 4 * WAVE_SLOTS), jy(img + 5 * WAVE_SLOTS), jz(img + 6 * WAVE_SLOTS),
           velm(reinterpret_cast<mixed4*>(a_.velm)), posq(reinterpret_cast<real4*>(a_.posq)), pcorr(reinterpret_cast<float4*>(a_.posq_corr)),
-          lane(lane_), G(a_.num_groups), nw(a_.num_wtiles), use_com(a_.use_com != 0), hardwall(a_.hardwall != 0),
+          vpl(reinterpret_cast<mixed*>(a_.vplanes)), pinvm((mixed)0), lane(lane_), G(a_.num_groups), nw(a_.num_wtiles), use_com(a_.use_com != 0), hardwall(a_.hardwall != 0),
           dt((mixed)a_.dt), fscale((mixed)(0.5 * a_.dt / 4294967296.0)) {}
     __device__ __forceinline__ static void wfence() {
         __builtin_amdgcn_fence(__ATOMIC_RELEASE, "wavefront");
@@ -88,12 +94,15 @@
     }
     __device__ __forceinline__ void load_vf(const WaveBounds& b, WStepIn<PREC>& in) {
         const int idx = b.ws + lane;
-        const bool patterned = pw.of(a, (uint32_t)b.y >> 8, lane);
+        const bool patterned = pw.of(a, (uint32_t)b.y >> 8, lane, [&](const uint32_t at) {
+            if (PLANES) pinvm = reinterpret_cast<const mixed*>(a.wpat_invm)[at];
+        });
         mixed4 v = mk4((mixed)0, (mixed)0, (mixed)0, (mixed)0);
         uint32_t meta = 64u << 10;
         long long fx = 0, fy = 0, fz = 0;
         if (lane < b.n) {
-            v = reinterpret_cast<const mixed4*>(a.velm)[idx];
+            if (PLANES) v = mk4(vpl[idx], vpl[idx + a.padded], vpl[idx + 2 * a.padded], pinvm);
+            else v = reinterpret_cast<const mixed4*>(a.velm)[idx];
             if (!patterned) meta = a.wmeta[idx];
             fx = a.force[idx]; fy = a.force[idx + a.padded]; fz = a.force[idx + 2 * a.padded];
         }
@@ -240,7 +249,8 @@
         wfence();
         if (lane < bd.n) {
             const int idx = bd.ws + lane;
-            velm[idx] = v;
+            if (PLANES) { vpl[idx] = v.x; vpl[idx + a.padded] = v.y; vpl[idx + 2 * a.padded] = v.z; }
+            else velm[idx] = v;
             store_position<PREC>(posq, pcorr, idx, px, py, pz, pq);
         }
     }
diff --git a/openmm_drudenose_amd/csrc/tgnh_wave_kernels.h b/openmm_drudenose_amd/csrc/tgnh_wave_kernels.h
--- a/openmm_drudenose_amd/csrc/tgnh_wave_kernels.h
+++ b/openmm_drudenose_amd/csrc/tgnh_wave_kernels.h
@@ -151,8 +151,8 @@
 }
 
 
-template <int PREC, int GB, bool MULTI = false>
-__global__ __launch_bounds__(WBLOCK) void wstep_kernel(const TileArgs a) {
+template <int PREC, int GB, bool MULTI, bool PLANES>
+__device__ __forceinline__ void wstep_body(const TileArgs& a) {
     typedef typename Prec<PREC>::mixed mixed;
     static_assert(GB > 0, "register bins only");
     __shared__ double s_scale[MAX_GROUPS + 2];
@@ -171,14 +171,14 @@
     TileEnv<PREC, GB> e;
     e.tid = tid; e.G = G; e.smem = nullptr; e.wbins0 = nullptr; e.s_scale = s_scale;
     e.clear_ke();
-    WaveStep<PREC, GB> ws(a, &e, s_scale, &s_img[wv][0][0], lane);
+    WaveStep<PREC, GB, PLANES> ws(a, &e, s_scale, &s_img[wv][0][0], lane);
     typedef WaveBounds Bounds;
     auto bounds = [&](const int ww, Bounds& b) { ws.bounds(ww, b); };
     auto load_vf = [&](const Bounds& b, WStepIn<PREC>& in) { ws.load_vf(b, in); };
     auto load_x = [&](const Bounds& b, WStepIn<PREC>& in) { ws.load_x(b, in); };
     auto prepare = [&](WStepIn<PREC>& t, const Bounds& bd, const bool ke) { ws.template prepare<true>(t, bd, ke); };
     auto finish = [&](WStepIn<PREC>& t, const Bounds& bd) { ws.finish(t, bd); };
-    auto wfence = [] { WaveStep<PREC, GB>::wfence(); };
+    auto wfence = [] { WaveStep<PREC, GB, PLANES>::wfence(); };
 
     unsigned gen0 = 0;
     unsigned long long seq0 = 0;
@@ -245,6 +245,11 @@
     TRACE(15);
 }
 
+template <int PREC, int GB, bool MULTI = false>
+__global__ __launch_bounds__(WBLOCK) void wstep_kernel(const TileArgs a) { wstep_body<PREC, GB, MULTI, false>(a); }
+template <int PREC, int GB, bool MULTI = false>
+__global__ __launch_bounds__(WBLOCK) void wstep_planes_kernel(const TileArgs a) { wstep_body<PREC, GB, MULTI, true>(a); }
+
 template <int PREC, int OPS> static tile_fn_t wke_fn_gb(int gb) {
     if (gb <= 1) return wke_kernel<PREC, OPS, 1>;
     if (gb <= 4) return wke_kernel<PREC, OPS, 4>;
@@ -270,22 +275,28 @@
 }
 int wke_blocks_per_cu(int precision, int ops, int gb) { return blocks_per_cu(wke_fn(precision, ops, gb), TBLOCK, 0); }
 
-template <int PREC, bool MULTI> static tile_fn_t wstep_fn_gb(int gb) {
+template <int PREC, bool MULTI> static tile_fn_t wstep_fn_gb(int gb, bool planes) {
+    if (planes && PREC == TGNH_PREC_SINGLE) return nullptr;
+    constexpr int PLANES_PREC = PREC == TGNH_PREC_SINGLE ? TGNH_PREC_MIXED : PREC;
+    if (planes) return gb <= 1 ? wstep_planes_kernel<PLANES_PREC, 1, MULTI>
+                     : gb <= 4 ? wstep_planes_kernel<PLANES_PREC, 4, MULTI>
+                               : wstep_planes_kernel<PLANES_PREC, 8, MULTI>;
     return gb <= 1 ? wstep_kernel<PREC, 1, MULTI> : gb <= 4 ? wstep_kernel<PREC, 4, MULTI> : wstep_kernel<PREC, 8, MULTI>;
 }
-static tile_fn_t wstep_fn(int precision, int gb, bool multi) {
+static tile_fn_t wstep_fn(int precision, int gb, bool multi, bool planes) {
     if (gb == 0) return nullptr;
     return with_precision(precision, [&](auto P) -> tile_fn_t {
-        return multi ? wstep_fn_gb<decltype(P)::value, true>(gb) : wstep_fn_gb<decltype(P)::value, false>(gb);
+        return multi ? wstep_fn_gb<decltype(P)::value, true>(gb, planes) : wstep_fn_gb<decltype(P)::value, false>(gb, planes);
     });
 }
 hipError_t launch_wstep(int precision, int gb, bool multi, const TileArgs& a, int grid, hipStream_t s) {
-    tile_fn_t fn = wstep_fn(precision, gb, multi);
+    if (a.vplanes && !a.wpat_invm) return hipErrorInvalidValue;
+    tile_fn_t fn = wstep_fn(precision, gb, multi, a.vplanes != nullptr);
     if (!fn) return hipErrorInvalidValue;
     TGNH_LAUNCH(fn, dim3(grid), dim3(WBLOCK), 0, s, a);
     return hipGetLastError();
 }
-int wstep_blocks_per_cu(int precision, int gb, bool multi) { return blocks_per_cu(wstep_fn(precision, gb, multi), WBLOCK, 0); }
+int wstep_blocks_per_cu(int precision, int gb, bool multi, bool planes) { return blocks_per_cu(wstep_fn(precision, gb, multi, planes), WBLOCK, 0); }
 
 }
 #endif
diff --git a/openmm_drudenose_amd/drudetgnhplugin.py b/openmm_drudenose_amd/drudetgnhplugin.py
--- a/openmm_drudenose_amd/drudetgnhplugin.py
+++ b/openmm_drudenose_amd/drudetgnhplugin.py
@@ -994,9 +994,9 @@
                     _check(self.lib.tgnh_run_harness(self.h, self._x0_arg(), self.k_drude, self.k_tether, int(steps), self._stream()))
             return g
         for _ in range(4):
-            owed_before = self.pending_state() & 0x2ff
+            owed_before = self.pending_state() & 0x6ff
             first = record()
-            if self.pending_state() & 0x2ff == owed_before:
+            if self.pending_state() & 0x6ff == owed_before:
                 break
             first.replay()
             torch.cuda.synchronize(self.dev)
@@ -1005,14 +1005,19 @@
             raise TgnhError(_lib.ERR_STATE, "capture_steps: the handle does not reach a steady state of its step sequence")
         clock = self.time()
         graphs = [first, record()]
-        if self.pending_state() & 0x2ff != owed_before:
+        if self.pending_state() & 0x6ff != owed_before:
             raise TgnhError(_lib.ERR_STATE, "capture_steps: the step sequence is not periodic")
         self.set_time(*clock)
         self._captured_not_run = int(steps)
         turn = [0]
         baths = self._bath_epoch
 
+        planes = owed_before & 0x400
+
         def replay():
+            if (self.pending_state() ^ planes) & 0x400:
+                raise TgnhError(_lib.ERR_STATE, "capture_steps: the velocities no longer live where these steps were recorded "
+                                "(a flush or a query moved them between the library's planes and velm): capture them again")
             if self._bath_epoch != baths:
                 raise TgnhError(_lib.ERR_STATE, "capture_steps: the temperatures were changed after these steps were recorded "
                                 "(their launches hold the old kT): capture them again")
@@ -1032,6 +1037,11 @@
         _check(self.lib.tgnh_get_pending_state(self.h, C.byref(bits)))
         return bits.value
 
+    def velocity_planes(self):
+        out = (C.c_int32 * 4)()
+        _check(self.lib.tgnh_get_velocity_planes(self.h, out))
+        return bool(out[0]), bool(out[1]), int(out[2]), int(out[3])
+
     def status_flags(self):
         flags = C.c_uint32()
         self.lib.tgnh_get_status_flags(self.h, self._stream(), C.byref(flags))
```

Measured after the change: 4544 steps/s (median of 6 runs). 9.3% higher.
